# manuelruder/fast-artistic-videos

Hardware: AMD Instinct MI355X
Metric: stylized frames/sec @1280x720, per-frame hot path (mask + warp + assembly + net + deprocess + PNG encode on the GPU) with inputs resident in HBM; file->PNG rate of the product CLI (BASELINE.json's end-to-end) in `end_to_end_fps` / `e2e`, PSNR vs CPU ref in `parity` (higher is better)
Workload: dtype f32

## Files before the change

### fast-artistic-videos_amd/csrc/fav_internal.h

```cpp
#pragma once
#include <hip/hip_runtime.h>
#include <cstdarg>
#include <cstdint>
#include <cstdio>
#include <exception>
#include <new>
#include <string>
#include <vector>

#include "../../include/fav.h"

#include <cstdlib>
inline const char* diag_env(const char* name)
{
#ifdef FAV_DIAG
    return getenv(name);
#else
    (void)name;
    return nullptr;
#endif
}

namespace fav {

// ... 28 lines not shown
        ::fav::set_error(where_ ": unexpected exception"); return FAV_EFORMAT;                                            \
    }

int ensure_device();

struct TraceRange {
    explicit TraceRange(const char* name);
    ~TraceRange();
    static bool enabled();
    bool on;
};

enum LayerType { L_PAD, L_CONV, L_IN, L_RELU, L_RES, L_UP, L_TANH, L_MUL, L_IDENTITY, L_BN };

struct Layer {
    LayerType type = L_IDENTITY;
    int pl = 0, pr = 0, pt = 0, pb = 0, pad_mode = 0;
    int cin = 0, cout = 0, k = 0, stride = 1, pad = 0;
    int transposed = 0, adj = 0;
    std::vector<float> w, b;
    std::vector<float> gamma, beta, mean, var;
    float eps = 1e-5f;
    int scale = 1;
    float mul = 1.f;
    int shave = 0;
    std::vector<Layer> block;
};

int t7_parse_model(const char* path, std::vector<Layer>& out);
int blob_pack(const std::vector<Layer>& layers, std::vector<uint8_t>& blob);
int blob_unpack(const void* blob, size_t bytes, std::vector<Layer>& out);
std::string describe_layers(const std::vector<Layer>& layers, int indent = 0);

struct Affine {
    const float* scale1 = nullptr; const float* shift1 = nullptr; int relu1 = 0;
    const float* scale2 = nullptr; const float* shift2 = nullptr; int relu2 = 0;
    int stages = 0;
    const long long* acc1 = nullptr; long long* acc1_zero = nullptr;
    const float* gamma1 = nullptr; const float* beta1 = nullptr; float eps1 = 0.f; int count1 = 0;
};
constexpr int STAT_COPIES = 8;
inline size_t stat_acc_words(int C) { return (size_t)STAT_COPIES * C * 4; }
constexpr long long STAT_NONFINITE = 1ll << 53;
__host__ __device__ inline bool stat_acc_poisoned(long long hi_sum, long long hi_squares)
{
    return hi_sum >= STAT_NONFINITE / 2 || hi_sum <= -(STAT_NONFINITE / 2) || hi_squares >= STAT_NONFINITE / 2 || hi_squares <= -(STAT_NONFINITE / 2);
}

struct ConvLaunch {
    const float* in = nullptr;
    int IH = 0, IW = 0;
    int IWp = 0;
    int ups = 0;
    int stuff = 0;
    int CIN = 0;
    Affine pre;
    const float* wgt = nullptr;
    const unsigned short* wgt16 = nullptr;
    const float* bias = nullptr;
    int COUT = 0, COUTp = 0;
    int KH = 0, KW = 0, stride = 1, pad = 0;
    int Kpad = 0;
    int OH = 0, OW = 0;
    float* out = nullptr;
    float* partials = nullptr;
    int final_mode = 0;
    float tanh_mul = 1.f;
    float* out_planar = nullptr;
    float* out_raw_nchw = nullptr;
    float* sk_ws = nullptr; unsigned* sk_flags = nullptr; unsigned sk_epoch = 0;
    unsigned* sk_err = nullptr;
    int reserve_cus = 0;
    int no_sk = 0;
    const float* join_skip = nullptr; float* join_out = nullptr; int OWp = 0;
    long long* stat_acc = nullptr;
    float* ks_ws = nullptr; int* ks_cnt = nullptr;
};
inline size_t conv3_wino4_ksplit_bytes() { return (size_t)256 * 2 * 256 * 128 * sizeof(float); }
size_t conv_streamk_workspace_bytes();
int conv_streamk_grid();
constexpr int CONV_BM = 128;
inline int conv_mblocks(int OH, int OW) { return (OH * OW + CONV_BM - 1) / CONV_BM; }
int launch_conv(const ConvLaunch& p, hipStream_t st);
bool conv_c8_eligible(int cin_pitch, int coutp, int k, int stride, int stages, int ups);
int conv_c8_tiles(int OH, int OW);
int launch_conv_c8(const ConvLaunch& p, int* counts, hipStream_t st);
bool conv_c8d_eligible(int cin_pitch, int cin_real, int coutp, int k, int stride, int stages, int ups);
void conv_c8d_pack(const float* w, int cin, int cout, std::vector<float>& out);
int launch_conv_c8d(const ConvLaunch& p, int cin_real, const float* wc8d, int* counts, hipStream_t st);
bool conv3_halo_eligible(int cin_pitch, int coutp, int k, int stride);
int conv3_halo_tiles(int OH, int OW, bool edge_b);
int launch_conv3_halo(const ConvLaunch& p, int* counts, hipStream_t st);
bool conv3s2_eligible(int cin_pitch, int coutp, int k, int stride, int stages, int ups);
int conv3s2_tiles(int OH, int OW);
int launch_conv3s2(const ConvLaunch& p, int* counts, hipStream_t st);
bool conv_fold_eligible(int cin_pitch, int cout, int k, int stride);
bool conv_fold_launchable(int cin_pitch, int k, int pad, int ups, int IH, int IW);
int launch_conv_fold(const ConvLaunch& p, const float* wfold, hipStream_t st);
int conv_first_tiles(int OH, int OW);
int launch_conv_first(const ConvLaunch& p, int cin_real, const float* wpk, int* counts, hipStream_t st);
bool conv_first2d_eligible(int cin_pitch, int cin_real, int coutp, int k, int stride, int stages, int ups);
int conv_first2d_tiles(int OH, int OW);
int launch_conv_first2d(const ConvLaunch& p, int cin_real, const float* wpk, int* counts, hipStream_t st);
bool conv3_wino_eligible(int cin_pitch, int cout, int coutp, int k, int stride, int pad, int stages, int ups);
int conv3_wino_tiles(int OH, int OW);
int launch_conv3_wino(const ConvLaunch& p, const float* wpk, int* counts, hipStream_t st);
bool conv3_wino4_eligible(int cin_pitch, int cout, int coutp, int k, int stride, int pad, int stages, int ups);
int conv3_wino4_tiles(int OH, int OW);
int launch_conv3_wino4(const ConvLaunch& p, const float* wpk, int* counts, hipStream_t st);
bool conv3_up2_eligible(int cin_pitch, int cout, int coutp, int k, int stride, int pad, int stages, int ups);
int conv3_up2_tiles(int OH, int OW);
int launch_conv3_up2(const ConvLaunch& p, const float* wpk, int* counts, hipStream_t st);
bool conv3s2w_eligible(int cin_pitch, int cout, int coutp, int k, int stride, int pad, int stages, int ups);
int conv3s2w_tiles(int OH, int OW, int coutp);
int launch_conv3s2w(const ConvLaunch& p, const float* wpk, int* counts, hipStream_t st);
enum ConvKernel { CK_GENERIC, CK_FOLD, CK_C8, CK_C8D, CK_FIRST1D, CK_FIRST2D, CK_S2W, CK_UP2, CK_WINO, CK_WINO4, CK_HALO3, CK_S2HALO };
constexpr int CONV_KERNELS = CK_S2HALO + 1;
int launch_in_finalize(const float* partials, const int* counts, int mblocks, int M, int block_pixels, int C, int Cpitch,
                       const float* gamma, const float* beta, float eps,
                       float* scale, float* shift, hipStream_t st);
int launch_stats(const float* x, int M, int C, const Affine& t, float* partials, hipStream_t st);
int launch_pad_nhwc(const float* in, int Hp, int Wp, int in_pitch, int C, int ups, float* out, int pl, int pr, int pt, int pb, int mode, hipStream_t st);
int launch_res_add(const float* y, const float* scale, const float* shift,
                   const float* skip, int SH, int SW, int shave, const Affine& skip_t,
                   int C, float* z, float* partials, int* counts, hipStream_t st, int skip_pitch = 0, const Affine* branch_acc = nullptr);
inline int res_add_stat_blocks(int OH, int OW) { return OH * ((OW + 127) / 128); }
int launch_nchw_to_nhwc_pad(const float* in, int C, int H, int W, int pad, int Cp, float* out, hipStream_t st);
int launch_nhwc_to_nchw(const float* in, int M, int C, const Affine& t, float* out, hipStream_t st);

#ifdef __HIPCC__
__device__ __forceinline__ float fill_uniform(unsigned seed, unsigned index, unsigned c, unsigned y, unsigned x)
{
    unsigned k = seed * 0x9E3779B1u + index * 0x85EBCA77u + c * 0xC2B2AE3Du + y * 0x27D4EB2Fu + x * 0x165667B1u;
    k ^= k >> 15; k *= 0x2C1B3C6Du;
    k ^= k >> 12; k *= 0x297A2D39u;
    k ^= k >> 15;
    return (float)(k >> 8) * (1.0f / 16777216.0f);
}
#endif

int launch_warp(const float* img, const float* flow, float* out, int B, int C, int H, int W, int Ho, int Wo,
                int border, hipStream_t st);
int launch_min_filter_f32(const float* cert, float* out, int H, int W, int r, hipStream_t st);
int launch_assemble(const float* frame, const float* warped, const float* cert, float* in7, int H, int W,
                    hipStream_t st);
int launch_cert_prepare(const uint8_t* mask, const float* backward_flo, int invert, int fix_occ, int border,
                        int r, float* cert_tmp, float* cert, int H, int W, hipStream_t st);
int launch_prep_input(const uint8_t* frame_hwc, const float* prev_rgb, int Hs, int Ws, const float* backward_flo,
                      const float* cert, int border, int H, int W, int pad, float* in8, hipStream_t st,
                      int fill_random = 0, unsigned seed = 0, unsigned index = 0, int* q0_out = nullptr);
int launch_quantize_rgb8(const float* rgb_planar, uint8_t* out_hwc, int H, int W, hipStream_t st);
constexpr int PNG_NSYM = 277;
constexpr int PNG_NTABLES = 12;
constexpr int PNG_HDR_WORDS = 40;
struct PngTable {
    uint32_t sym[PNG_NSYM];
    uint32_t hdr[PNG_HDR_WORDS];
    uint32_t hdr_bits, btype, dist_len, dist_code;
// ... 50 lines not shown
```

### fast-artistic-videos_amd/csrc/kernels_elem.hip

```cpp
#include <algorithm>

#include "fav_internal.h"
#include "conv_device.h"

namespace fav {

namespace {

__global__ __launch_bounds__(256) void in_finalize_kernel(const float2* partials, const int* counts, int mblocks, int M, int bp,
                                                          int Cpitch, const float* gamma, const float* beta,
                                                          float eps, float* scale, float* shift)
{
    __shared__ double sh[8];
    const int c = blockIdx.x, t = threadIdx.x;
    double s1 = 0, s2 = 0;
    float gq = 1.f, bq = 0.f;
    if (t == 0) { gq = gamma ? gamma[c] : 1.f; bq = beta ? beta[c] : 0.f; }
    for (int b0 = t; b0 < mblocks; b0 += 1024) {
        float2 pr[4]; int nb[4];
#pragma unroll
        for (int k = 0; k < 4; ++k) {
            const int b = b0 + 256 * k, bc = min(b, mblocks - 1);
            pr[k] = partials[(size_t)bc * Cpitch + c];
            nb[k] = b < mblocks ? (counts ? counts[bc] : min(bp, M - bc * bp)) : 0;
        }
#pragma unroll
        for (int k = 0; k < 4; ++k) {
            const double n = (double)nb[k], mu = (double)pr[k].x;
            s1 += n * mu;
            s2 += (nb[k] ? (double)pr[k].y : 0.0) + n * mu * mu;
        }
    }
    for (int o = 32; o > 0; o >>= 1) { s1 += __shfl_xor(s1, o); s2 += __shfl_xor(s2, o); }
    if ((t & 63) == 0) { sh[2 * (t >> 6)] = s1; sh[2 * (t >> 6) + 1] = s2; }
    __syncthreads();
    if (t == 0) {
        const double a = ((sh[0] + sh[2]) + sh[4]) + sh[6], q = ((sh[1] + sh[3]) + sh[5]) + sh[7];
        const double mean = a / (double)M;
        double var = q / (double)M - mean * mean;
        var = var > 0.0 ? var : 0.0;
        const double g = (double)gq, bt = (double)bq;
        const double sc = g / sqrt(var + (double)eps);
        scale[c] = (float)sc;
        shift[c] = (float)(bt - mean * sc);
    }
}

__device__ __forceinline__ float4 apply_affine_g(float4 v, const Affine& a, int c)
{
    if (a.stages >= 1) {
        v = affine4(v, a.scale1 + c, a.shift1 + c, a.relu1);
        if (a.stages >= 2) v = affine4(v, a.scale2 + c, a.shift2 + c, a.relu2);
    }
    return v;
}

template <int NPT>
__global__ __launch_bounds__(256) void stats_kernel(const float* x, int M, int C, const Affine a, float2* partials)
{
    __shared__ float red[1024];
    __shared__ float mean_s[1024];
    const int t = threadIdx.x;
    const int groups = C >> 2;
    const int nl = 256 / groups;
    const int g = t % groups, pl = t / groups;
    const int m0 = blockIdx.x * 128;
    const int cnt = min(128, M - m0);
    const bool active = pl < nl;
    float4 s = make_float4(0, 0, 0, 0);
    float4 keep[NPT > 0 ? NPT : 1];
    if (NPT > 0) {
#pragma unroll
        for (int i = 0; i < NPT; ++i) {
            const int pix = pl + i * nl;
            float4 v = make_float4(0, 0, 0, 0);
            if (pix < cnt) { v = *reinterpret_cast<const float4*>(x + (size_t)(m0 + pix) * C + 4 * g); v = apply_affine_g(v, a, 4 * g); }
            keep[i] = v;
        }
#pragma unroll
        for (int i = 0; i < NPT; ++i) { s.x += keep[i].x; s.y += keep[i].y; s.z += keep[i].z; s.w += keep[i].w; }
    } else if (active)
        for (int pix = pl; pix < cnt; pix += nl) {
            float4 v = *reinterpret_cast<const float4*>(x + (size_t)(m0 + pix) * C + 4 * g);
            v = apply_affine_g(v, a, 4 * g);
            s.x += v.x; s.y += v.y; s.z += v.z; s.w += v.w;
        }
    if (active) *reinterpret_cast<float4*>(red + pl * C + 4 * g) = s;
    __syncthreads();
    for (int c = t; c < C; c += 256) {
        float r = 0;
        for (int i = 0; i < nl; ++i) r += red[i * C + c];
        mean_s[c] = r / (float)cnt;
    }
    __syncthreads();
    float4 q = make_float4(0, 0, 0, 0);
    if (active) {
        const float4 mu = *reinterpret_cast<const float4*>(mean_s + 4 * g);
        if (NPT > 0) {
#pragma unroll
            for (int i = 0; i < NPT; ++i) {
                const float4 v = keep[i];
                const float dx = v.x - mu.x, dy = v.y - mu.y, dz = v.z - mu.z, dw = v.w - mu.w;
                if (pl + i * nl < cnt) { q.x = fmaf(dx, dx, q.x); q.y = fmaf(dy, dy, q.y); q.z = fmaf(dz, dz, q.z); q.w = fmaf(dw, dw, q.w); }
            }
        } else
            for (int pix = pl; pix < cnt; pix += nl) {
                float4 v = *reinterpret_cast<const float4*>(x + (size_t)(m0 + pix) * C + 4 * g);
                v = apply_affine_g(v, a, 4 * g);
                const float dx = v.x - mu.x, dy = v.y - mu.y, dz = v.z - mu.z, dw = v.w - mu.w;
                q.x = fmaf(dx, dx, q.x); q.y = fmaf(dy, dy, q.y); q.z = fmaf(dz, dz, q.z); q.w = fmaf(dw, dw, q.w);
            }
        *reinterpret_cast<float4*>(red + pl * C + 4 * g) = q;
    }
    __syncthreads();
    for (int c = t; c < C; c += 256) {
        float r = 0;
        for (int i = 0; i < nl; ++i) r += red[i * C + c];
        partials[(size_t)blockIdx.x * C + c] = make_float2(mean_s[c], r);
    }
}

template <bool ACC>
__global__ __launch_bounds__(256) void res_add_kernel(const float* y, const float* scale, const float* shift,
                                                      const float* skip, int SW, int shave, const Affine sa,
                                                      int OH, int OW, int C, float* z, const Affine br)
{
    __shared__ float ss[ACC ? 2048 : 4];
    if (ACC) {
        for (int i = threadIdx.x; i < C; i += 256) {
            long long w0 = 0, w1 = 0, w2 = 0, w3 = 0;
#pragma unroll
            for (int cp = 0; cp < STAT_COPIES; ++cp) {
                const longlong2* a = reinterpret_cast<const longlong2*>(br.acc1 + ((size_t)cp * C + i) * 4);
                const longlong2 lo = a[0], hi = a[1];
                w0 += lo.x; w1 += lo.y; w2 += hi.x; w3 += hi.y;
            }
            const double s1 = ((double)w1 * 4294967296.0 + (double)w0) * (1.0 / 1099511627776.0);
            const double s2 = ((double)w3 * 4294967296.0 + (double)w2) * (1.0 / 1099511627776.0);
            const double mean = s1 / (double)br.count1;
            double var = s2 / (double)br.count1 - mean * mean;
            var = var > 0.0 ? var : 0.0;
            const double sc = stat_acc_poisoned(w1, w3) ? (double)NAN : (double)br.gamma1[i] / sqrt(var + (double)br.eps1);
            ss[i] = (float)sc; ss[C + i] = (float)((double)br.beta1[i] - mean * sc);
            if (blockIdx.x == 0) {
#pragma unroll
                for (int cp = 0; cp < STAT_COPIES; ++cp) {
                    longlong2* zz = reinterpret_cast<longlong2*>(br.acc1_zero + ((size_t)cp * C + i) * 4);
                    zz[0] = longlong2{0, 0}; zz[1] = longlong2{0, 0};
                }
            }
        }
        __syncthreads();
        scale = ss; shift = ss + C;
    }
    const int groups = C >> 2;
    const size_t total = (size_t)OH * OW * groups;
    for (size_t idx = (size_t)blockIdx.x * 256 + threadIdx.x; idx < total; idx += (size_t)gridDim.x * 256) {
        const int g = (int)(idx % groups);
        const size_t pix = idx / groups;
        const int oy = (int)(pix / OW), ox = (int)(pix - (size_t)oy * OW);
        float4 v = *reinterpret_cast<const float4*>(y + pix * C + 4 * g);
        v = affine4(v, scale + 4 * g, shift + 4 * g, 0);
        float4 k = *reinterpret_cast<const float4*>(skip + ((size_t)(oy + shave) * SW + ox + shave) * C + 4 * g);
        k = apply_affine_g(k, sa, 4 * g);
        v.x += k.x; v.y += k.y; v.z += k.z; v.w += k.w;
        *reinterpret_cast<float4*>(z + pix * C + 4 * g) = v;
    }
}

template <int NPT>
__global__ __launch_bounds__(256) void res_add_stats_kernel(const float* y, const float* scale, const float* shift,
                                                            const float* skip, int SW, int shave, const Affine sa,
                                                            int OW, int C, float* z, float2* partials, int* counts)
{
    __shared__ float red[1024];
    __shared__ float mean_s[1024];
    const int t = threadIdx.x;
    const int groups = C >> 2, nl = 256 / groups;
    const int g = t % groups, pl = t / groups;
    const int segs = (OW + 127) / 128;
    const int oy = blockIdx.x / segs, x0 = (blockIdx.x - oy * segs) * 128;
    const int cnt = min(128, OW - x0);
    const bool active = pl < nl;
    const float* yr = y + ((size_t)oy * OW + x0) * C + 4 * g;
    const float* kr = skip + ((size_t)(oy + shave) * SW + x0 + shave) * C + 4 * g;
    float* zr = z + ((size_t)oy * OW + x0) * C + 4 * g;
    float4 sm = make_float4(0, 0, 0, 0);
    float4 keep[NPT > 0 ? NPT : 1];
    if (NPT > 0) {
        float4 kk[NPT > 0 ? NPT : 1];
#pragma unroll
        for (int i = 0; i < NPT; ++i) {
            const int px = pl + i * nl;
            keep[i] = make_float4(0, 0, 0, 0); kk[i] = make_float4(0, 0, 0, 0);
            if (px < cnt) { keep[i] = *reinterpret_cast<const float4*>(yr + (size_t)px * C); kk[i] = *reinterpret_cast<const float4*>(kr + (size_t)px * C); }
        }
#pragma unroll
        for (int i = 0; i < NPT; ++i) {
            const int px = pl + i * nl;
            float4 v = affine4(keep[i], scale + 4 * g, shift + 4 * g, 0);
            const float4 k = apply_affine_g(kk[i], sa, 4 * g);
            v.x += k.x; v.y += k.y; v.z += k.z; v.w += k.w;
            if (px < cnt) { *reinterpret_cast<float4*>(zr + (size_t)px * C) = v; sm.x += v.x; sm.y += v.y; sm.z += v.z; sm.w += v.w; }
            keep[i] = v;
        }
    } else if (active)
        for (int px = pl; px < cnt; px += nl) {
            float4 v = *reinterpret_cast<const float4*>(yr + (size_t)px * C);
            v = affine4(v, scale + 4 * g, shift + 4 * g, 0);
            float4 k = *reinterpret_cast<const float4*>(kr + (size_t)px * C);
            k = apply_affine_g(k, sa, 4 * g);
            v.x += k.x; v.y += k.y; v.z += k.z; v.w += k.w;
            *reinterpret_cast<float4*>(zr + (size_t)px * C) = v;
            sm.x += v.x; sm.y += v.y; sm.z += v.z; sm.w += v.w;
        }
    if (active) *reinterpret_cast<float4*>(red + pl * C + 4 * g) = sm;
    __syncthreads();
    for (int c = t; c < C; c += 256) {
        float r = 0;
        for (int i = 0; i < nl; ++i) r += red[i * C + c];
        mean_s[c] = r / (float)cnt;
    }
    __syncthreads();
    float4 q = make_float4(0, 0, 0, 0);
    if (active) {
        const float4 mu = *reinterpret_cast<const float4*>(mean_s + 4 * g);
        if (NPT > 0) {
#pragma unroll
            for (int i = 0; i < NPT; ++i) {
                const float4 v = keep[i];
                const float dx = v.x - mu.x, dy = v.y - mu.y, dz = v.z - mu.z, dw = v.w - mu.w;
                if (pl + i * nl < cnt) { q.x = fmaf(dx, dx, q.x); q.y = fmaf(dy, dy, q.y); q.z = fmaf(dz, dz, q.z); q.w = fmaf(dw, dw, q.w); }
            }
        } else
        for (int px = pl; px < cnt; px += nl) {
            const float4 v = *reinterpret_cast<const float4*>(zr + (size_t)px * C);
            const float dx = v.x - mu.x, dy = v.y - mu.y, dz = v.z - mu.z, dw = v.w - mu.w;
            q.x = fmaf(dx, dx, q.x); q.y = fmaf(dy, dy, q.y); q.z = fmaf(dz, dz, q.z); q.w = fmaf(dw, dw, q.w);
        }
        *reinterpret_cast<float4*>(red + pl * C + 4 * g) = q;
    }
    __syncthreads();
    for (int c = t; c < C; c += 256) {
        float r = 0;
        for (int i = 0; i < nl; ++i) r += red[i * C + c];
        partials[(size_t)blockIdx.x * C + c] = make_float2(mean_s[c], r);
    }
    if (t == 0) counts[blockIdx.x] = cnt;
}

__device__ __forceinline__ int reflect(int i, int n)
{
    if (i < 0) i = -i;
    if (i >= n) i = 2 * (n - 1) - i;
    return i;
}

__global__ __launch_bounds__(256) void nchw_to_nhwc_pad_kernel(const float* in, int C, int H, int W, int pad, int Cp,
                                                               float* out)
{
    const int Hp = H + 2 * pad, Wp = W + 2 * pad;
    const size_t total = (size_t)Hp * Wp * Cp;
    for (size_t idx = (size_t)blockIdx.x * 256 + threadIdx.x; idx < total; idx += (size_t)gridDim.x * 256) {
        const int c = (int)(idx % Cp);
        const size_t pix = idx / Cp;
        const int y = (int)(pix / Wp), x = (int)(pix - (size_t)y * Wp);
        float v = 0.f;
        if (c < C) v = in[((size_t)c * H + reflect(y - pad, H)) * W + reflect(x - pad, W)];
        out[idx] = v;
    }
}

__global__ __launch_bounds__(256) void nhwc_to_nchw_kernel(const float* in, int M, int C, const Affine a, float* out)
{
    const size_t total = (size_t)M * C;
    for (size_t idx = (size_t)blockIdx.x * 256 + threadIdx.x; idx < total; idx += (size_t)gridDim.x * 256) {
        const int c = (int)(idx / M);
        const size_t m = idx - (size_t)c * M;
        float v = in[m * C + c];
        if (a.stages >= 1) {
            v = fmaf(v, a.scale1[c], a.shift1[c]); if (a.relu1) v = fmaxf(v, 0.f);
            if (a.stages >= 2) { v = fmaf(v, a.scale2[c], a.shift2[c]); if (a.relu2) v = fmaxf(v, 0.f); }
        }
        out[idx] = v;
    }
}

inline int grid_for(size_t total) { size_t b = (total + 255) / 256; return (int)(b > 8192 ? 8192 : (b ? b : 1)); }

}

int launch_in_finalize(const float* partials, const int* counts, int mblocks, int M, int block_pixels, int C, int Cpitch,
                       const float* gamma, const float* beta, float eps, float* scale, float* shift, hipStream_t st)
{
    hipLaunchKernelGGL(in_finalize_kernel, dim3(C), dim3(256), 0, st, reinterpret_cast<const float2*>(partials), counts,
                       mblocks, M, block_pixels, Cpitch, gamma, beta, eps, scale, shift);
    FAV_LAUNCH_CHECK("in_finalize_kernel");
    return FAV_OK;
}

int launch_stats(const float* x, int M, int C, const Affine& t, float* partials, hipStream_t st)
{
    FAV_REQUIRE(C % 4 == 0 && C <= 1024 && 256 % (C / 4) == 0, "stats: unsupported channel count %d", C);
    const dim3 grid((M + 127) / 128);
    float2* pp = reinterpret_cast<float2*>(partials);
    if (C == 64) hipLaunchKernelGGL(stats_kernel<8>, grid, dim3(256), 0, st, x, M, C, t, pp);
    else if (C == 128) hipLaunchKernelGGL(stats_kernel<16>, grid, dim3(256), 0, st, x, M, C, t, pp);
    else hipLaunchKernelGGL(stats_kernel<0>, grid, dim3(256), 0, st, x, M, C, t, pp);
    FAV_LAUNCH_CHECK("stats_kernel");
    return FAV_OK;
}

int launch_res_add(const float* y, const float* scale, const float* shift, const float* skip, int SH, int SW,
                   int shave, const Affine& skip_t, int C, float* z, float* partials, int* counts, hipStream_t st, int skip_pitch, const Affine* branch_acc)
{
    const int OH = SH - 2 * shave, OW = SW - 2 * shave;
    if (skip_pitch > 0) SW = skip_pitch;
    FAV_REQUIRE(C % 4 == 0 && C <= 1024 && 256 % (C / 4) == 0 && OH > 0 && OW > 0, "res_add: bad shape (C=%d)", C);
    FAV_REQUIRE(!(partials && branch_acc && branch_acc->acc1), "res_add: the statistics-taking join does not take an accumulator-form InstanceNorm");
    if (partials) {
        const dim3 grid(res_add_stat_blocks(OH, OW));
        float2* pp = reinterpret_cast<float2*>(partials);
        if (C == 128) hipLaunchKernelGGL(res_add_stats_kernel<16>, grid, dim3(256), 0, st, y, scale, shift, skip, SW, shave, skip_t, OW, C, z, pp, counts);
        else if (C == 64) hipLaunchKernelGGL(res_add_stats_kernel<8>, grid, dim3(256), 0, st, y, scale, shift, skip, SW, shave, skip_t, OW, C, z, pp, counts);
        else hipLaunchKernelGGL(res_add_stats_kernel<0>, grid, dim3(256), 0, st, y, scale, shift, skip, SW, shave, skip_t, OW, C, z, pp, counts);
    }
    else if (branch_acc != nullptr && branch_acc->acc1 != nullptr)
        hipLaunchKernelGGL(res_add_kernel<true>, dim3(std::min(1024, grid_for((size_t)OH * OW * (C / 4)))), dim3(256), 0, st, y, scale, shift, skip, SW, shave, skip_t,
                           OH, OW, C, z, *branch_acc);
    else
        hipLaunchKernelGGL(res_add_kernel<false>, dim3(grid_for((size_t)OH * OW * (C / 4))), dim3(256), 0, st, y, scale, shift, skip, SW, shave, skip_t,
                           OH, OW, C, z, Affine());
    FAV_LAUNCH_CHECK("res_add_kernel");
    return FAV_OK;
}

int launch_nchw_to_nhwc_pad(const float* in, int C, int H, int W, int pad, int Cp, float* out, hipStream_t st)
{
    FAV_REQUIRE(pad < H && pad < W, "reflection pad %d must be smaller than the image (%dx%d)", pad, W, H);
    hipLaunchKernelGGL(nchw_to_nhwc_pad_kernel, dim3(grid_for((size_t)(H + 2 * pad) * (W + 2 * pad) * Cp)), dim3(256), 0,
                       st, in, C, H, W, pad, Cp, out);
    FAV_LAUNCH_CHECK("nchw_to_nhwc_pad_kernel");
    return FAV_OK;
}

int launch_nhwc_to_nchw(const float* in, int M, int C, const Affine& t, float* out, hipStream_t st)
{
    hipLaunchKernelGGL(nhwc_to_nchw_kernel, dim3(grid_for((size_t)M * C)), dim3(256), 0, st, in, M, C, t, out);
    FAV_LAUNCH_CHECK("nhwc_to_nchw_kernel");
    return FAV_OK;
}

}
```

### fast-artistic-videos_amd/csrc/kernels_first.hip

```cpp
#include <algorithm>
#include <cstdlib>
#include <vector>

#include "fav_internal.h"
#include "conv_device.h"
#include "launch_common.h"
#include "first_pack.h"
#include "first2d_pack.h"

namespace fav {

namespace {

constexpr int F_TH = 8, F_TW = 64;
constexpr int F_HR = F_TH + 8, F_HC = F_TW + 8;
constexpr int F_HALF = F_HC / 2;
constexpr int F_RP = F_HC;
constexpr int F_CPL = F_HR * F_RP;
constexpr int F_HP = F_HR * F_HC;
constexpr int F_NH = (F_HP + 511) / 512;

struct FirstArgs {
    const float* in; const float* wpk; const float* bias;
    float* out; float2* partials; int* counts;
    int IH, IW, IWp, COUT, pad, OH, OW, tiles_x, tiles_y;
    int COUTP, groups;
    long long* dbg = nullptr;
};

__device__ __forceinline__ float2 merge_rows(const float2* st, const int* wn, int c, int* n_out)
{
    int n = 0; float s = 0.f;
    for (int w = 0; w < 8; ++w) { n += wn[w]; s += (float)wn[w] * st[w * 32 + c].x; }
    const float mean = n ? s / (float)n : 0.f;
    float m2 = 0.f;
    for (int w = 0; w < 8; ++w) { const float d = st[w * 32 + c].x - mean; m2 += st[w * 32 + c].y + (float)wn[w] * d * d; }
    *n_out = n;
    return make_float2(mean, m2);
}

constexpr int f_off(int e) { return (e & 1) * F_HALF + (e >> 1); }

template <int CR>
__global__ __launch_bounds__(512, 2) void conv_first_kernel(const FirstArgs p)
{
    constexpr int NCC = (CR / 2) * 27, NJ = NCC + 14, LAST = CR - 1;
    extern __shared__ __attribute__((aligned(16))) float smem[];
    float* const Ws = smem;
    float* const Hs = Ws + 4 * NJ * 64;
    float* const red = Hs + CR * F_CPL;
    const int t = threadIdx.x, lane = t & 63, wave = t >> 6;

    for (int e = t; e < 4 * NJ * 16; e += 512) *reinterpret_cast<v4f*>(Ws + e * 4) = *reinterpret_cast<const v4f*>(p.wpk + e * 4);

    const int ntiles = p.tiles_x * p.tiles_y;
    float4 hlo[F_NH], hhi[F_NH];
#define FL_LOAD_HALO(tile_)                                                                         \
// ... 206 lines not shown
        _Pragma("unroll") for (int i = 0; i < G_NH; ++i) {                                          \
            float* d_ = Hs + min(t + 512 * i, G_HP - 1);                                            \
            const float c_[8] = {hlo[i].x, hlo[i].y, hlo[i].z, hlo[i].w, hhi[i].x, hhi[i].y, hhi[i].z, hhi[i].w}; \
            _Pragma("unroll") for (int c = 0; c < CR; ++c) d_[c * G_CPL] = c_[c];                   \
        }                                                                                           \
    }

    int tile = WIDE ? blockIdx.x / p.groups : blockIdx.x;
    G_LOAD_HALO(tile);
    G_STORE_HALO();

    const int txl = lane & 15, g = lane >> 4;
    int qoff[NQ];
#pragma unroll
    for (int q = 0; q < NQ; ++q) {
        const int idx = 4 * q + g;
        const int c = idx / 9, a = (idx - 9 * c) / 3, b = idx - 9 * c - 3 * a;
        qoff[q] = idx < 9 * CR ? c * G_CPL + 3 * a * G_HC + 3 * b : 0;
    }
    const float* const a_lane = Hs + 2 * wave * G_HC + 2 * txl;
    const float* const b_lo = Ws + lane;
    int hi_words = 8 * NQ * 128;
    asm volatile("" : "+v"(hi_words));
    const float* const b_hi = b_lo + hi_words;
    __syncthreads();

#ifdef FAV_DIAG
    long long dt_[5] = {0, 0, 0, 0, 0}, tq_ = 0; int ntl_ = 0;
#define G_DBG(i_) { if (p.dbg && t == 0) { const long long n_ = wall_clock64(); dt_[i_] += n_ - tq_; tq_ = n_; } }
    if (p.dbg && t == 0) tq_ = wall_clock64();
#else
#define G_DBG(i_)
#endif
    for (; tile < ntiles; tile += tstep) {
        const int nxt = tile + tstep;
        G_LOAD_HALO(nxt);
        G_DBG(0);
        v4f acc[16][2];
#pragma unroll
        for (int ps = 0; ps < 16; ++ps)
#pragma unroll
            for (int nt = 0; nt < 2; ++nt) acc[ps][nt] = v4f{0.f, 0.f, 0.f, 0.f};

        float R[2][16], B[2][8];
#define G_READ_R(set_, q_)                                                                          \
        { const float* rb_ = a_lane + qoff[q_];                                                     \
          _Pragma("unroll") for (int r = 0; r < 4; ++r) _Pragma("unroll") for (int d = 0; d < 4; ++d) R[set_][4 * r + d] = rb_[r * G_HC + d]; }
#define G_READ_B(set_, q_, i_)                                                                      \
        { _Pragma("unroll") for (int j = 0; j < 4; ++j) _Pragma("unroll") for (int nt = 0; nt < 2; ++nt) \
              B[set_][2 * j + nt] = ((i_) < 2 ? b_lo : b_hi)[(((4 * ((i_) & 1) + j) * NQ + (q_)) * 2 + nt) * 64]; }
#define G_FENCE() __builtin_amdgcn_sched_barrier(0)
        G_READ_R(0, 0);
        G_READ_B(0, 0, 0);
#pragma unroll
        for (int q = 0; q < NQ; ++q) {
            if (q + 1 < NQ) { G_READ_R((q + 1) & 1, q + 1); }
#pragma unroll
            for (int i = 0; i < 4; ++i) {
                float L[4], V[4];
                const float* Rq = R[q & 1];
#pragma unroll
                for (int d = 0; d < 4; ++d)
                    L[d] = i == 0 ? Rq[d] - Rq[8 + d] : i == 1 ? Rq[4 + d] + Rq[8 + d] : i == 2 ? Rq[8 + d] - Rq[4 + d] : Rq[4 + d] - Rq[12 + d];
                V[0] = L[0] - L[2]; V[1] = L[1] + L[2]; V[2] = L[2] - L[1]; V[3] = L[1] - L[3];
                const int nset = (4 * q + i + 1) & 1;
                if (i < 3) { G_READ_B(nset, q, i + 1); } else if (q + 1 < NQ) { G_READ_B(nset, q + 1, 0); }
// ... 83 lines not shown
            const int nw = nrows * ncols;
#pragma unroll
            for (int nt = 0; nt < 2; ++nt) {
                float s = sm[nt];
                s += __shfl_xor(s, 16); s += __shfl_xor(s, 32);
                const float mu = nw ? s / (float)nw : 0.f;
                float qv = 0.f;
                if (inside) {
#pragma unroll
                    for (int r = 0; r < 4; ++r)
#pragma unroll
                        for (int a = 0; a < 2; ++a)
#pragma unroll
                            for (int b = 0; b < 2; ++b) { const float d = y[nt][r][a][b] - mu; qv = fmaf(d, d, qv); }
                } else {
#pragma unroll
                    for (int r = 0; r < 4; ++r)
#pragma unroll
                        for (int a = 0; a < 2; ++a)
#pragma unroll
                            for (int b = 0; b < 2; ++b) {
                                const int oy = oy0 + a, ox = ox0 + 2 * (4 * g + r) + b;
                                const float d = y[nt][r][a][b] - mu;
                                if (oy < p.OH && ox < p.OW) qv = fmaf(d, d, qv);
                            }
                }
                qv += __shfl_xor(qv, 16); qv += __shfl_xor(qv, 32);
                if (lane < 16) st[wave * 32 + nt * 16 + lane] = make_float2(mu, qv);
            }
            if (lane == 0) wn[wave] = nw;
            __syncthreads();
            if (t < 32) {
                int n;
                p.partials[(size_t)tile * PITCH + grp * 32 + t] = merge_rows(st, wn, t, &n);
                if (t == 0 && grp == 0) p.counts[tile] = n;
            }
        }
        __syncthreads();
        G_DBG(4);
#ifdef FAV_DIAG
        ++ntl_;
#endif
    }
#ifdef FAV_DIAG
    if (p.dbg && t == 0) { for (int i = 0; i < 5; ++i) p.dbg[blockIdx.x * 8 + i] = dt_[i]; p.dbg[blockIdx.x * 8 + 5] = ntl_; }
#endif
#undef G_DBG
#undef G_LOAD_HALO
#undef G_STORE_HALO
}

template <int CR, bool WIDE = false>
int launch_first2d_t(const FirstArgs& a, int reserve_cus, hipStream_t st)
{
    const size_t lds = (size_t)(16 * conv_first2d_quads(CR) * 128 + CR * G_CPL + 8 * 64 + 8) * sizeof(float);
    static PerDevice cache; int cus;
    FAV_HIP(launch_cus(cache, &cus, conv_first2d_kernel<CR, WIDE>));
    const int tiles = a.tiles_x * a.tiles_y;
    const int ngrp = WIDE ? a.groups : 1;
    int grid = persistent_slots(cus, reserve_cus);
    grid = std::min(grid, tiles * ngrp);
    if (WIDE) grid = std::max(ngrp, grid / ngrp * ngrp);
#ifdef FAV_DIAG
    static int dbg_n = diag_env("FAV_FIRST_DBG") ? atoi(diag_env("FAV_FIRST_DBG")) : 0;
    static long long* dbuf = nullptr;
    const bool dbg = dbg_n > 0 && --dbg_n == 0;
    FirstArgs ad = a;
    if (dbg) { FAV_HIP(hipMalloc(reinterpret_cast<void**>(&dbuf), 1024 * 8 * 8)); FAV_HIP(hipMemsetAsync(dbuf, 0, 1024 * 8 * 8, st)); ad.dbg = dbuf; }
    hipLaunchKernelGGL((conv_first2d_kernel<CR, WIDE>), dim3(grid), dim3(512), lds, st, ad);
    FAV_LAUNCH_CHECK("conv_first2d_kernel");
    if (dbg) {
        std::vector<long long> hb((size_t)1024 * 8);
        FAV_HIP(hipStreamSynchronize(st)); FAV_HIP(hipMemcpy(hb.data(), dbuf, hb.size() * 8, hipMemcpyDeviceToHost));
        double sum[5] = {0, 0, 0, 0, 0}, nt = 0;
        for (int b = 0; b < grid; ++b) { for (int i = 0; i < 5; ++i) sum[i] += hb[b * 8 + i] * 0.01; nt += hb[b * 8 + 5]; }
        fprintf(stderr, "FIRSTDBG grid=%d tiles=%.0f  per tile (us): halo request %.2f  quads %.2f  barrier + halo to LDS %.2f  transform + stores %.2f  statistics %.2f\n",
                grid, nt, sum[0] / nt, sum[1] / nt, sum[2] / nt, sum[3] / nt, sum[4] / nt);
    }
    return FAV_OK;
#else
    hipLaunchKernelGGL((conv_first2d_kernel<CR, WIDE>), dim3(grid), dim3(512), lds, st, a);
    FAV_LAUNCH_CHECK("conv_first2d_kernel");
    return FAV_OK;
#endif
}

}

int conv_first_tiles(int OH, int OW) { return ((OH + F_TH - 1) / F_TH) * ((OW + F_TW - 1) / F_TW); }

int launch_conv_first(const ConvLaunch& c, int cin_real, const float* wpk, int* counts, hipStream_t st)
{
    FAV_REQUIRE(c.CIN == 8 && (cin_real == 7 || cin_real == 3) && c.COUTp == 32 && c.KH == 9 && c.KW == 9 && c.stride == 1 && c.pre.stages == 0 &&
                c.ups == 0 && !c.final_mode && wpk, "first-layer conv (F(2,3) along x): not eligible");
    FAV_REQUIRE((long long)c.IH * c.IWp * 8 < (1ll << 31), "first-layer conv: bad shape");
    FirstArgs a;
    a.in = c.in; a.wpk = wpk; a.bias = c.bias; a.out = c.out; a.partials = reinterpret_cast<float2*>(c.partials); a.counts = counts;
    a.IH = c.IH; a.IW = c.IW; a.IWp = c.IWp; a.COUT = c.COUT; a.pad = c.pad; a.OH = c.OH; a.OW = c.OW;
    a.tiles_x = (c.OW + F_TW - 1) / F_TW; a.tiles_y = (c.OH + F_TH - 1) / F_TH;
    return cin_real == 7 ? launch_first_t<7>(a, c.reserve_cus, st) : launch_first_t<3>(a, c.reserve_cus, st);
}

bool conv_first2d_eligible(int cin_pitch, int cin_real, int coutp, int k, int stride, int stages, int ups)
{
    return cin_pitch == 8 && (cin_real == 7 || cin_real == 3) && k == 9 && stride == 1 && stages == 0 && ups == 0 && coutp % 32 == 0 && coutp >= 32 && coutp <= 256;
}
int conv_first2d_tiles(int OH, int OW) { return ((OH + G_TH - 1) / G_TH) * ((OW + G_TW - 1) / G_TW); }

int launch_conv_first2d(const ConvLaunch& c, int cin_real, const float* wpk, int* counts, hipStream_t st)
{
    FAV_REQUIRE(conv_first2d_eligible(c.CIN, cin_real, c.COUTp, c.KH, c.stride, c.pre.stages, c.ups) && c.KW == 9 && !c.final_mode && wpk,
                "first-layer conv (F(2x2,3x3) over the nine 3x3 blocks): not eligible");
    FAV_REQUIRE((long long)c.IH * c.IWp * 32 < (1ll << 31) - 512, "first-layer conv: input too large for 32-bit byte offsets");
    FirstArgs a;
    a.in = c.in; a.wpk = wpk; a.bias = c.bias; a.out = c.out; a.partials = reinterpret_cast<float2*>(c.partials); a.counts = counts;
    a.IH = c.IH; a.IW = c.IW; a.IWp = c.IWp; a.COUT = c.COUT; a.pad = c.pad; a.OH = c.OH; a.OW = c.OW;
    a.tiles_x = (c.OW + G_TW - 1) / G_TW; a.tiles_y = (c.OH + G_TH - 1) / G_TH;
    a.COUTP = c.COUTp; a.groups = c.COUTp / 32; a.dbg = nullptr;
    if (a.groups > 1) return cin_real == 7 ? launch_first2d_t<7, true>(a, c.reserve_cus, st) : launch_first2d_t<3, true>(a, c.reserve_cus, st);
    return cin_real == 7 ? launch_first2d_t<7>(a, c.reserve_cus, st) : launch_first2d_t<3>(a, c.reserve_cus, st);
}

}
```

### fast-artistic-videos_amd/csrc/kernels_fold.hip

```cpp
#include <algorithm>
#include <cstdlib>
#include <vector>

#include "fav_internal.h"
#include "conv_device.h"
#include "launch_common.h"

namespace fav {

namespace {

constexpr int FOLD_R = 16;
constexpr int FOLD_M = 128;

struct FoldArgs {
    const float* in; const float* wfold; const float* bias;
    const float* scale1; const float* shift1; const float* scale2; const float* shift2;
    float* out_planar; float* out_raw;
    int IH, IW, IWp, ups, COUT, KH, KW, pad, OH, OW;
    int stages, relu1, relu2;
    float tanh_mul;
    int tiles_x, tiles_y;
    long long* dbg;
};

template <int CIN>
__global__ __launch_bounds__(512, 2) void conv_rowfold_kernel(const FoldArgs p)
{
    constexpr int NT = 512;
    constexpr int RW = FOLD_R / 2;
    constexpr int S = CIN + 4;
    constexpr int NV = CIN / 16;
    constexpr int KK = CIN / 8;
    extern __shared__ __attribute__((aligned(16))) float smem[];
    float* Bs = smem;
    float* aff = Bs + p.KH * 32 * S;
    float* As = aff + 4 * CIN;

    const int t = threadIdx.x, lane = t & 63, wave = t >> 6;
    const int wcol = wave & 3, wrow = wave >> 2;
    const int XO = FOLD_M - (p.KW - 1);

    for (int i = t; i < CIN; i += NT) {
        aff[i] = p.stages >= 1 ? p.scale1[i] : 1.f; aff[CIN + i] = p.stages >= 1 ? p.shift1[i] : 0.f;
        aff[2 * CIN + i] = p.stages >= 2 ? p.scale2[i] : 1.f; aff[3 * CIN + i] = p.stages >= 2 ? p.shift2[i] : 0.f;
    }
    const float lo1 = (p.stages >= 1 && p.relu1) ? 0.f : -INFINITY;
    const float lo2 = (p.stages >= 2 && p.relu2) ? 0.f : -INFINITY;
    for (int e = t; e < p.KH * 32 * (CIN / 4); e += NT) {
        const int row = e / (CIN / 4), c4 = e - row * (CIN / 4);
        *reinterpret_cast<v4f*>(Bs + row * S + c4 * 4) = *reinterpret_cast<const v4f*>(p.wfold + (size_t)row * CIN + c4 * 4);
    }
    const int xl = t >> 2, ch0 = (t & 3) * (CIN / 4);
// ... 106 lines not shown
            __syncthreads();
        }
    }
}

constexpr int FOLD2_M = 64;

template <int CIN, int NH = 1>
__global__ __launch_bounds__(512, 2) void conv_rowfold_up2_kernel(const FoldArgs p)
{
    constexpr int NT = 512;
    constexpr int CT = CIN * NH;
    constexpr int RW = FOLD_R / 4;
    constexpr int S = CIN + 4;
    constexpr int NV = CIN / 32;
    constexpr int KK = CIN / 8;
    extern __shared__ __attribute__((aligned(16))) float smem[];
    float* Bs = smem;
    float* aff = Bs + (p.KH + 1) * 32 * S;
    float* As = aff + 4 * CIN;

    const int t = threadIdx.x, lane = t & 63, wave = t >> 6;
    const int wcol = wave & 1, wrow = wave >> 1;
    const int XO = 2 * FOLD2_M - (p.KW - 1);
    const int PH = p.IH >> 1, PW = p.IW >> 1;

    const float lo1 = (p.stages >= 1 && p.relu1) ? 0.f : -INFINITY;
    const float lo2 = (p.stages >= 2 && p.relu2) ? 0.f : -INFINITY;
    const float* wm = p.wfold + (size_t)p.KH * 32 * CT;
#define FOLD_RESIDENT(hoff_)                                                                        \
    {                                                                                               \
        for (int i = t; i < CIN; i += NT) {                                                         \
            aff[i] = p.stages >= 1 ? p.scale1[(hoff_) + i] : 1.f; aff[CIN + i] = p.stages >= 1 ? p.shift1[(hoff_) + i] : 0.f; \
            aff[2 * CIN + i] = p.stages >= 2 ? p.scale2[(hoff_) + i] : 1.f; aff[3 * CIN + i] = p.stages >= 2 ? p.shift2[(hoff_) + i] : 0.f; \
        }                                                                                           \
        for (int e = t; e < (p.KH + 1) * 32 * (CIN / 4); e += NT) {                                 \
            const int row = e / (CIN / 4), c4 = e - row * (CIN / 4);                                \
            *reinterpret_cast<v4f*>(Bs + row * S + c4 * 4) = *reinterpret_cast<const v4f*>(wm + (size_t)row * CT + (hoff_) + c4 * 4); \
        }                                                                                           \
    }
    if (NH == 1) FOLD_RESIDENT(0);
    const int xl = t >> 3, ch0 = (t & 7) * (CIN / 8);
    const int frag = (lane & 31) * S + (lane >> 5) * 4;
    const int col = lane & 31, rbase = 4 * (lane >> 5);
    float4 ra[NV];

    for (int tile = blockIdx.x; tile < p.tiles_x * p.tiles_y; tile += gridDim.x) {
        const int by = tile / p.tiles_x, bx = tile - by * p.tiles_x;
        const int ox0 = bx * XO, oy0 = by * FOLD_R;
        const int pxs = (ox0 - p.pad) >> 1;
        const int iy_lo = max(0, oy0 - p.pad), iy_hi = min(p.IH - 1, oy0 + FOLD_R - 1 + p.KH - 1 - p.pad);
        const int pr_lo = iy_lo >> 1, pr_hi = min(iy_hi >> 1, PH - 1);
        const int pc = pxs + xl;
        const bool colv = pc >= 0 && pc < PW;
        const float colm = colv ? 1.f : 0.f;
        const int coloff = colv ? pc * CT + ch0 : 0;
        int hoff = 0;

#define FOLD_LOAD(pr_)                                                                              \
        {                                                                                           \
            const float* src_ = p.in + (size_t)(pr_) * p.IWp * CT + coloff + hoff;                  \
            _Pragma("unroll") for (int i = 0; i < NV; ++i) ra[i] = *reinterpret_cast<const float4*>(src_ + 4 * i); \
        }
#define FOLD_STORE(buf_)                                                                            \
        {                                                                                           \
            float* dst_ = As + (buf_) * FOLD2_M * S + xl * S + ch0;                                 \
            _Pragma("unroll") for (int i = 0; i < NV; ++i) {                                        \
// ... 145 lines not shown
        for (int b = 0; b < 512; ++b) { n += hb[b * 8]; a0 += hb[b * 8 + 1]; a1 += hb[b * 8 + 2]; a2 += hb[b * 8 + 3]; rows += hb[b * 8 + 4]; }
        if (n > 0) fprintf(stderr, "FOLDDBG tiles=%.0f  per tile: first row %.2f  loop %.2f (%.1f staged rows)  epilogue %.2f us\n", n, a0 / n * 0.01, a1 / n * 0.01, rows / n, a2 / n * 0.01);
    }
    return FAV_OK;
}

template <int CIN>
int launch_fold_t(FoldArgs a, int reserve_cus, hipStream_t st)
{
    const int S = CIN + 4;
    const size_t wbytes = (size_t)(a.KH * 32 * S + 4 * CIN) * sizeof(float);
    size_t stage = (size_t)(2 * FOLD_M * S) * sizeof(float);
    const size_t epi = (size_t)4 * FOLD_M * 33 * sizeof(float);
    if (epi > stage) stage = epi;
    const size_t lds = wbytes + stage;
    if (lds > 160 * 1024) { set_error("row-folded conv: %zu bytes of LDS needed", lds); return FAV_EUNSUPPORTED; }
    static PerDevice cache; int cus;
    FAV_HIP(launch_cus(cache, &cus, conv_rowfold_kernel<CIN>));
    const int XO = FOLD_M - (a.KW - 1);
    a.tiles_x = (a.OW + XO - 1) / XO; a.tiles_y = (a.OH + FOLD_R - 1) / FOLD_R;
    const int tiles = a.tiles_x * a.tiles_y;
    const int nres = persistent_slots(cus, reserve_cus);
    hipLaunchKernelGGL((conv_rowfold_kernel<CIN>), dim3(tiles < nres ? tiles : nres), dim3(512), lds, st, a);
    FAV_LAUNCH_CHECK("conv_rowfold_kernel");
    return FAV_OK;
}

}

bool conv_fold_eligible(int cin_pitch, int cout, int k, int stride)
{
    return stride == 1 && cout * k <= 32 && k <= 9 && (cin_pitch == 16 || cin_pitch == 32 || cin_pitch == 64 || cin_pitch == 128 || cin_pitch == 256);
}
bool conv_fold_launchable(int cin_pitch, int k, int pad, int ups, int IH, int IW)
{
    static const bool no_up2 = diag_env("FAV_NO_FOLD_UP2") != nullptr;
    if (cin_pitch <= 64) return true;
    return ups == 1 && !no_up2 && (pad & 1) == 0 && (k & 1) == 1 && (IH & 1) == 0 && (IW & 1) == 0 && k + 1 <= 10;
}

int launch_conv_fold(const ConvLaunch& c, const float* wfold, hipStream_t st)
{
    FAV_REQUIRE(conv_fold_eligible(c.CIN, c.COUT, c.KW, c.stride) && c.KH == c.KW && c.final_mode, "row-folded conv: not eligible");
    FoldArgs a;
    a.dbg = nullptr;
    a.in = c.in; a.wfold = wfold; a.bias = c.bias;
    a.scale1 = c.pre.scale1; a.shift1 = c.pre.shift1; a.scale2 = c.pre.scale2; a.shift2 = c.pre.shift2;
    a.stages = c.pre.stages; a.relu1 = c.pre.relu1; a.relu2 = c.pre.relu2;
    a.out_planar = c.out_planar; a.out_raw = c.out_raw_nchw;
    a.IH = c.IH; a.IW = c.IW; a.IWp = c.IWp; a.ups = c.ups; a.COUT = c.COUT; a.KH = c.KH; a.KW = c.KW; a.pad = c.pad;
    a.OH = c.OH; a.OW = c.OW; a.tanh_mul = c.tanh_mul;
    static const bool no_up2 = diag_env("FAV_NO_FOLD_UP2") != nullptr;
    if (c.ups == 1 && !no_up2 && (c.pad & 1) == 0 && (c.KW & 1) == 1 && (c.IH & 1) == 0 && (c.IW & 1) == 0 && c.KH + 1 <= 10) {
        if (c.CIN == 256) return launch_fold_up2_t<64, 4>(a, c.reserve_cus, st);
        if (c.CIN == 128) return launch_fold_up2_t<64, 2>(a, c.reserve_cus, st);
        if (c.CIN == 64) return launch_fold_up2_t<64>(a, c.reserve_cus, st);
        if (c.CIN == 32) return launch_fold_up2_t<32>(a, c.reserve_cus, st);
    }
    FAV_REQUIRE(c.CIN <= 64, "row-folded conv: %d input channels are supported on a x2-upsampled input only", c.CIN);
    if (c.CIN == 64) return launch_fold_t<64>(a, c.reserve_cus, st);
    if (c.CIN == 32) return launch_fold_t<32>(a, c.reserve_cus, st);
    return launch_fold_t<16>(a, c.reserve_cus, st);
}

}
```

### fast-artistic-videos_amd/csrc/kernels_s2.hip

```cpp
#include <algorithm>
#include <cstdlib>

#include "fav_internal.h"
#include "conv_device.h"
#include "launch_common.h"
#include "s2_pack.h"

namespace fav {

namespace {

constexpr int SW_P = 20;
constexpr int SW_EW = 33, SW_OW = 32;

struct S2wArgs {
    const float* in; const float* wpk; const float* bias; const float* scale1; const float* shift1;
    float* out; float2* partials; int* counts;
    int IH, IW, IWp, CIN, OH, OW, pad, tiles_x, tiles_y, stages, relu1;
    int COUTP, groups;
};

template <int NTC, int TR> struct SwGeo {
    static constexpr int NW = NTC * TR;
    static constexpr int NTH = 64 * NW;
    static constexpr int HR = 2 * TR + 1;
    static constexpr int EP = HR * SW_EW;
    static constexpr int HP = EP + HR * SW_OW;
    static constexpr int PS = NTH / 4;
    static constexpr int NPC = (HP + PS - 1) / PS;
    static constexpr int HB = NPC * PS * SW_P;
};

template <int NTC, int TR, bool WIDE = false>
__global__ __launch_bounds__(64 * NTC * TR, NTC * TR / 4) void conv3s2w_kernel(const S2wArgs p)
{
    using G = SwGeo<NTC, TR>;
    static_assert(G::NW % 4 == 0 && G::NW >= 8 && G::NW <= 16, "whole waves per SIMD");
    constexpr int COUT = NTC * 32;
    constexpr int EP = G::EP, HP = G::HP, NPC = G::NPC, HB = G::HB, PS = G::PS, NTH = G::NTH;
    extern __shared__ __attribute__((aligned(16))) float smem[];
    float* const Hs = smem;
    float* const aff = smem + 2 * HB;
    float2* const stt = reinterpret_cast<float2*>(aff + 2 * p.CIN);
    int* const wn = reinterpret_cast<int*>(stt + TR * COUT);

    const int t = threadIdx.x, lane = t & 63;
    const int wave = __builtin_amdgcn_readfirstlane(t >> 6);
    const int nt = wave % NTC, row = wave / NTC;
    const int m = lane & 31, h = lane >> 5;
    const int CIN = p.CIN, nch = CIN >> 4;
    const int lb = xcd_linear_block();
    const int ngrp = WIDE ? p.groups : 1, grp = WIDE ? lb % p.groups : 0;
    const int PITCH = WIDE ? p.COUTP : COUT;
    const __amdgpu_buffer_rsrc_t wrs = __builtin_amdgcn_make_buffer_rsrc(const_cast<float*>(p.wpk) + (size_t)grp * (nch * 18 * NTC * 256), 0, nch * 18 * NTC * 1024, 0x00020000);
    const __amdgpu_buffer_rsrc_t irs = __builtin_amdgcn_make_buffer_rsrc(const_cast<float*>(p.in), 0, p.IH * p.IWp * CIN * 4, 0x00020000);
    const int wlo = lane * 16, wnt = nt * 1024;

    const float* const aE = Hs + ((2 * row) * SW_EW + m) * SW_P + 4 * h;
    const float* const aO = Hs + (EP + (2 * row) * SW_OW + m) * SW_P + 4 * h;
#define SW_AOFF(T_) (((T_) % 3 == 1) ? ((T_) / 3) * SW_OW * SW_P : (((T_) / 3) * SW_EW + ((T_) % 3 == 2 ? 1 : 0)) * SW_P)
#define SW_ABASE(T_) (((T_) % 3 == 1) ? aO : aE)

    const int c4 = t & 3, p0 = t >> 2;
    float* const hst = Hs + p0 * SW_P + c4 * 4;
    int hyx[NPC], hbase[NPC];
#pragma unroll
    for (int i = 0; i < NPC; ++i) {
        const int pe = p0 + PS * i;
        int hy = 0x7000, hx = 0;
        if (pe < EP) { hy = pe / SW_EW; hx = 2 * (pe - hy * SW_EW); }
        else if (pe < HP) { const int q = pe - EP; hy = q / SW_OW; hx = 2 * (q - hy * SW_OW) + 1; }
        hyx[i] = hy << 16 | hx;
        hbase[i] = ((pe < HP ? (hy * p.IWp + hx) * p.CIN : 0) + c4 * 4) * 4;
    }
    for (int i = t; i < CIN; i += NTH) { aff[i] = p.stages >= 1 ? p.scale1[i] : 1.f; aff[CIN + i] = p.stages >= 1 ? p.shift1[i] : 0.f; }
    const float lo1 = (p.stages >= 1 && p.relu1) ? 0.f : -INFINITY;
    const float* const affr = aff + c4 * 4;

    const int ntiles = p.tiles_x * p.tiles_y * ngrp;
    int tile = lb;
    if (tile >= ntiles) return;

    int ho[NPC]; float hm[NPC];
    v4f hq[NPC];
    bool hmask = false;
#define SW_TILE_SETUP(tile_)                                                                        \
    {   const int pt_ = WIDE ? (tile_) / ngrp : (tile_);                                            \
        const int ty_ = pt_ / p.tiles_x, tx_ = pt_ - ty_ * p.tiles_x;                               \
        const int iy0_ = 2 * ty_ * TR - p.pad, ix0_ = 2 * tx_ * 32 - p.pad;                         \
        hmask = iy0_ < 0 || ix0_ < 0 || iy0_ + 2 * TR >= p.IH || ix0_ + 64 >= p.IW;                  \
        if (!hmask) {                                                                               \
            const int org_ = (iy0_ * p.IWp + ix0_) * CIN * 4;                                       \
            _Pragma("unroll") for (int i = 0; i < NPC; ++i) ho[i] = hbase[i] + org_;                \
        } else {                                                                                    \
            _Pragma("unroll") for (int i = 0; i < NPC; ++i) {                                       \
                const int iy = iy0_ + (hyx[i] >> 16), ix = ix0_ + (hyx[i] & 0xffff);                \
                const bool v = ((unsigned)iy < (unsigned)p.IH) & ((unsigned)ix < (unsigned)p.IW);   \
                ho[i] = ((v ? (iy * p.IWp + ix) * CIN : 0) + c4 * 4) * 4;                           \
                hm[i] = v ? 1.f : 0.f;                                                              \
            } } }
#define SW_LOAD_H(chunk_)                                                                           \
    { _Pragma("unroll") for (int i = 0; i < NPC; ++i) hq[i] = __builtin_bit_cast(v4f, __builtin_amdgcn_raw_buffer_load_b128(irs, ho[i], (chunk_) * 64, 0)); }
#define SW_COMMIT(chunk_, par_)                                                                     \
    {   const v4f sc_ = *reinterpret_cast<const v4f*>(affr + (chunk_) * 16), sh_ = *reinterpret_cast<const v4f*>(affr + CIN + (chunk_) * 16); \
        _Pragma("unroll") for (int i = 0; i < NPC; ++i) {                                           \
            hq[i].x = fmaxf(fmaf(hq[i].x, sc_.x, sh_.x), lo1); hq[i].y = fmaxf(fmaf(hq[i].y, sc_.y, sh_.y), lo1); \
            hq[i].z = fmaxf(fmaf(hq[i].z, sc_.z, sh_.z), lo1); hq[i].w = fmaxf(fmaf(hq[i].w, sc_.w, sh_.w), lo1); } \
        if (hmask) { _Pragma("unroll") for (int i = 0; i < NPC; ++i) hq[i] *= hm[i]; }               \
// ... 47 lines not shown
            if (last && ntile < ntiles) SW_TILE_SETUP(ntile);
            const int so1 = ((chunk * 2 + 1) * 9) * NTC * 1024 + wnt, so0 = ((nchunk * 2) * 9) * NTC * 1024 + wnt;
#pragma unroll
            for (int tp = 0; tp < 9; ++tp) {
                fb[1][tp] = __builtin_bit_cast(v4f, __builtin_amdgcn_raw_buffer_load_b128(wrs, wlo, so1 + tp * NTC * 1024, 0));
                if (tp < NPC) hq[tp] = __builtin_bit_cast(v4f, __builtin_amdgcn_raw_buffer_load_b128(irs, ho[tp], nchunk * 64, 0));
                if (tp + 2 < 9) { SW_READ_A_DYN((tp + 2) % 3, tp + 2, 0, par); } else { SW_READ_A_DYN((tp + 2) % 3, tp + 2 - 9, 1, par); }
                SW_FENCE(); SW_MFMA4(fa[tp % 3], fb[0][tp]); SW_FENCE();
            }
#pragma unroll
            for (int tp = 0; tp < 7; ++tp) {
                fb[0][tp] = __builtin_bit_cast(v4f, __builtin_amdgcn_raw_buffer_load_b128(wrs, wlo, so0 + tp * NTC * 1024, 0));
                if (tp + 2 < 9) { SW_READ_A_DYN((tp + 2) % 3, tp + 2, 1, par); }
                SW_FENCE(); SW_MFMA4(fa[tp % 3], fb[1][tp]); SW_FENCE();
                if (tp == 2) { __builtin_amdgcn_sched_barrier(0); SW_COMMIT(nchunk, par ^ 1); __builtin_amdgcn_sched_barrier(0); }
            }
            asm volatile("s_waitcnt lgkmcnt(0)" ::: "memory");
            __syncthreads();
            __builtin_amdgcn_sched_barrier(0);
            {
                const v4f a7_ = fa[7 % 3], a8_ = fa[8 % 3];
                fb[0][7] = __builtin_bit_cast(v4f, __builtin_amdgcn_raw_buffer_load_b128(wrs, wlo, so0 + 7 * NTC * 1024, 0));
                fb[0][8] = __builtin_bit_cast(v4f, __builtin_amdgcn_raw_buffer_load_b128(wrs, wlo, so0 + 8 * NTC * 1024, 0));
                SW_READ_A_DYN(0, 0, 0, par ^ 1); SW_READ_A_DYN(1, 1, 0, par ^ 1);
                SW_FENCE(); SW_MFMA4(a7_, fb[1][7]); SW_MFMA4(a8_, fb[1][8]); SW_FENCE();
            }
            if (pend >= 0) {
                if (t < COUT) {
                    int cnt = 0; float s1 = 0.f;
                    for (int w = 0; w < TR; ++w) { cnt += wn[w]; s1 += (float)wn[w] * stt[w * COUT + t].x; }
                    const float mean = cnt ? s1 / (float)cnt : 0.f;
                    float m2 = 0.f;
                    for (int w = 0; w < TR; ++w) { const float d = stt[w * COUT + t].x - mean; m2 += stt[w * COUT + t].y + (float)wn[w] * d * d; }
                    p.partials[(size_t)pend * PITCH + grp * COUT + t] = make_float2(mean, m2);
                    if (t == 0 && grp == 0) p.counts[pend] = cnt;
                }
                pend = -1;
            }
            par ^= 1;
        }
        {
            const int oy = oy0 + row;
            float sm = 0.f; int nv = 0;
            float* const ob = p.out + ((size_t)oy * p.OW + ox0 + 4 * h) * PITCH + grp * COUT + co;
            const bool full = oy0 + TR <= p.OH && ox0 + 32 <= p.OW;
            if (full) {
#pragma unroll
                for (int r = 0; r < 16; ++r) {
                    const float v = acc[r] + bv;
                    acc[r] = v;
                    ob[(size_t)((r & 3) + 8 * (r >> 2)) * PITCH] = v;
                    sm += v;
                }
                nv = 16;
            } else {
#pragma unroll
                for (int r = 0; r < 16; ++r) {
                    const int mi = (r & 3) + 8 * (r >> 2);
                    const float v = acc[r] + bv;
                    acc[r] = v;
                    if (oy < p.OH && ox0 + 4 * h + mi < p.OW) { ob[(size_t)mi * PITCH] = v; sm += v; ++nv; }
                }
            }
            if (p.partials != nullptr) {
                const int nw = nv + __shfl_xor(nv, 32);
                const float ssum = sm + __shfl_xor(sm, 32);
                const float mu = nw ? ssum / (float)nw : 0.f;
                float q = 0.f;
                if (full) {
#pragma unroll
                    for (int r = 0; r < 16; ++r) { const float d = acc[r] - mu; q = fmaf(d, d, q); }
                } else {
#pragma unroll
                    for (int r = 0; r < 16; ++r) {
                        const int mi = (r & 3) + 8 * (r >> 2);
                        const float d = acc[r] - mu;
                        if (oy < p.OH && ox0 + 4 * h + mi < p.OW) q = fmaf(d, d, q);
                    }
                }
                q += __shfl_xor(q, 32);
                if (lane < 32) stt[row * COUT + co] = make_float2(mu, q);
                if (lane == 0 && nt == 0) wn[row] = nw;
                pend = ptile;
            }
#pragma unroll
            for (int r = 0; r < 16; ++r) acc[r] = 0.f;
        }
        tile = ntile;
        if (tile >= ntiles) break;
        ptile = WIDE ? tile / ngrp : tile;
        oy0 = (ptile / p.tiles_x) * TR; ox0 = (ptile - (ptile / p.tiles_x) * p.tiles_x) * 32;
    }
    if (pend >= 0) {
        __syncthreads();
        if (t < COUT) {
            int cnt = 0; float s1 = 0.f;
            for (int w = 0; w < TR; ++w) { cnt += wn[w]; s1 += (float)wn[w] * stt[w * COUT + t].x; }
            const float mean = cnt ? s1 / (float)cnt : 0.f;
            float m2 = 0.f;
            for (int w = 0; w < TR; ++w) { const float d = stt[w * COUT + t].x - mean; m2 += stt[w * COUT + t].y + (float)wn[w] * d * d; }
            p.partials[(size_t)pend * PITCH + grp * COUT + t] = make_float2(mean, m2);
            if (t == 0 && grp == 0) p.counts[pend] = cnt;
        }
    }
#undef SW_AOFF
#undef SW_ABASE
#undef SW_TILE_SETUP
#undef SW_LOAD_H
#undef SW_COMMIT
#undef SW_LOAD_B
#undef SW_READ_A
#undef SW_GROUP
#undef SW_TAPS
#undef SW_MFMA4
#undef SW_FENCE
#undef SW_READ_A_DYN
}

template <int NTC, int TR, bool WIDE = false>
int launch_s2w_t(const S2wArgs& a, int reserve_cus, hipStream_t st)
{
    const auto kern = conv3s2w_kernel<NTC, TR, WIDE>;
    const size_t lds = (size_t)(2 * SwGeo<NTC, TR>::HB + 2 * a.CIN) * sizeof(float) + (size_t)TR * NTC * 32 * sizeof(float2) + 16 * sizeof(int);
    static PerDevice cache; int cus;
    FAV_HIP(launch_cus(cache, &cus, kern));
    const int ngrp = WIDE ? a.groups : 1;
    const int tiles = a.tiles_x * a.tiles_y * ngrp;
    const int slots = persistent_slots(cus, reserve_cus);
    static const bool tile_grid = diag_env("FAV_S2W_TILE_GRID") != nullptr;
    int grid = (tile_grid && reserve_cus > 0 && tiles > 4 * slots) ? tiles : std::min(tiles, slots);
    if (WIDE) grid = std::max(ngrp, grid / ngrp * ngrp);
    hipLaunchKernelGGL(kern, dim3(grid), dim3(SwGeo<NTC, TR>::NTH), lds, st, a);
    FAV_LAUNCH_CHECK("conv3s2w_kernel");
    return FAV_OK;
}

}

bool conv3s2w_eligible(int cin_pitch, int cout, int coutp, int k, int stride, int pad, int stages, int ups)
{
    return k == 3 && stride == 2 && pad <= 1 && ups == 0 && stages <= 1 && cin_pitch % 16 == 0 && cin_pitch >= 32 && cin_pitch <= 512 &&
           cout == coutp && (coutp == 64 || (coutp % 128 == 0 && coutp <= 1024));
}
static int s2w_rows(int coutp) { static const int r128 = diag_env("FAV_S2W_ROWS128") ? atoi(diag_env("FAV_S2W_ROWS128")) : 3; return coutp == 64 ? 4 : (r128 == 2 && coutp == 128 ? 2 : 3); }
int conv3s2w_tiles(int OH, int OW, int coutp) { const int tr = s2w_rows(coutp); return ((OH + tr - 1) / tr) * ((OW + 31) / 32); }

int launch_conv3s2w(const ConvLaunch& c, const float* wpk, int* counts, hipStream_t st)
{
    FAV_REQUIRE(conv3s2w_eligible(c.CIN, c.COUT, c.COUTp, c.KH, c.stride, c.pad, c.pre.stages, c.ups) && c.KH == c.KW && !c.final_mode && !c.stuff && wpk,
                "stride-2 conv: not eligible");
    FAV_REQUIRE((long long)(c.IH + 1) * c.IWp * c.CIN < (1ll << 29), "stride-2 conv: tensor too large for 32-bit byte offsets");
    S2wArgs a;
    a.in = c.in; a.wpk = wpk; a.bias = c.bias; a.scale1 = c.pre.scale1; a.shift1 = c.pre.shift1; a.stages = c.pre.stages; a.relu1 = c.pre.relu1;
    a.out = c.out; a.partials = reinterpret_cast<float2*>(c.partials); a.counts = counts;
    a.IH = c.IH; a.IW = c.IW; a.IWp = c.IWp; a.CIN = c.CIN; a.OH = c.OH; a.OW = c.OW; a.pad = c.pad;
    const int tr = s2w_rows(c.COUTp);
    a.tiles_x = (c.OW + 31) / 32; a.tiles_y = (c.OH + tr - 1) / tr;
    a.COUTP = c.COUTp; a.groups = c.COUTp > 128 ? c.COUTp / 128 : 1;
    FAV_REQUIRE((long long)(c.OH + 1) * c.OW * c.COUTp < (1ll << 31), "stride-2 conv: output too large");
    if (a.groups > 1) return launch_s2w_t<4, 3, true>(a, c.reserve_cus, st);
    return c.COUTp == 64 ? launch_s2w_t<2, 4>(a, c.reserve_cus, st) : tr == 2 ? launch_s2w_t<4, 2>(a, c.reserve_cus, st) : launch_s2w_t<4, 3>(a, c.reserve_cus, st);
}

}
```

### fast-artistic-videos_amd/csrc/kernels_up2.hip

```cpp
#include <algorithm>
#include <cstdlib>

#include "fav_internal.h"
#include "conv_device.h"
#include "launch_common.h"
#include "up2_pack.h"

namespace fav {

namespace {

constexpr int U2_HW = 34, U2_HP = 10 * 34;
constexpr int U2_HPP = 384;
constexpr int U2_HB = U2_HPP * LDSS;

struct Up2Args {
    const float* in; const float* wpk; const float* bias; const float* scale1; const float* shift1;
    float* out; float2* partials; int* counts;
    int PH, PW, IWp, CIN, tiles_x, tiles_y, relu1;
    int COUTP, groups;
};

template <bool AFF>
__global__ __launch_bounds__(512, 2) void conv3_up2_kernel(const Up2Args p)
{
    extern __shared__ __attribute__((aligned(16))) float smem[];
    float* const Hs = smem;
    float* const aff = smem + 2 * U2_HB;

    const int t = threadIdx.x, lane = t & 63;
    const int wave = __builtin_amdgcn_readfirstlane(t >> 6);
    const int py = wave >> 2, px = (wave >> 1) & 1, nt = wave & 1;
    const int CIN = p.CIN, nslices = CIN >> 5, nsteps = nslices * 16;
    const int m = lane & 31, h = lane >> 5;

    const __amdgpu_buffer_rsrc_t wrs = __builtin_amdgcn_make_buffer_rsrc(const_cast<float*>(p.wpk), 0, nsteps * 8192, 0x00020000);
    const __amdgpu_buffer_rsrc_t irs = __builtin_amdgcn_make_buffer_rsrc(const_cast<float*>(p.in), 0, p.PH * p.IWp * CIN * 4, 0x00020000);
    const int wlo = lane * 16, wso = wave * 1024;

    const float* const ab = Hs + ((py * U2_HW) + px + m) * LDSS + 4 * h;
    const int c4 = t & 7;
    float* const hst = Hs + (t >> 3) * LDSS + c4 * 4;

    if (AFF) { for (int i = t; i < CIN; i += 512) { aff[i] = p.scale1[i]; aff[CIN + i] = p.shift1[i]; } __syncthreads(); }
    const float lo1 = (AFF && p.relu1) ? 0.f : -INFINITY;
    const float* const affr = aff + c4 * 4;

    const int ntiles = p.tiles_x * p.tiles_y;
    for (int tile = blockIdx.x; tile < ntiles; tile += gridDim.x) {
        const int ty = tile / p.tiles_x, tx = tile - ty * p.tiles_x;
        const int sy0 = ty * 8, sx0 = tx * 32;
// ... 131 lines not shown
                if (t == 0) p.counts[tile] = cnt;
            }
            __syncthreads();
        }
    }
}

constexpr int UW_HW = 34, UW_HP = 6 * 34;
constexpr int UW_HPP = 288;
constexpr int UW_HB = UW_HPP * LDSS;
static_assert(2 * 288 * LDSS <= 8 * 64 * 2 * LDSS, "halo buffers inside the exchange area");
constexpr int UW_ZS = 8 * 64 * 2 * LDSS;

template <bool WIDE>
__global__ __launch_bounds__(768) void conv3_up2w_kernel(const Up2Args p)
{
    extern __shared__ __attribute__((aligned(16))) float smem[];
    float* const Hs = smem;
    float* const aff = smem + UW_ZS;
    const int t = threadIdx.x, lane = t & 63;
    const int wave = __builtin_amdgcn_readfirstlane(t >> 6);
    const int kind = wave >> 2, row = wave & 3;
    const int CIN = p.CIN, nslices = CIN >> 5, nkg = CIN >> 3;
    const int m = lane & 31, h = lane >> 5;
    const int ngrp = WIDE ? p.groups : 1, PITCH = WIDE ? p.COUTP : 64;
    const __amdgpu_buffer_rsrc_t wrs = __builtin_amdgcn_make_buffer_rsrc(const_cast<float*>(p.wpk), 0, nkg * 18 * 1024 * ngrp, 0x00020000);
    const __amdgpu_buffer_rsrc_t irs = __builtin_amdgcn_make_buffer_rsrc(const_cast<float*>(p.in), 0, p.PH * p.IWp * CIN * 4, 0x00020000);
    const int wlo = lane * 16, wso0 = kind * 3 * 2048;
    const float kap = kind == 1 ? 0.f : 1.f;
    const float* const ra = Hs + ((row + (kind == 0 ? 0 : 1)) * UW_HW + m) * LDSS + 4 * h;
    const float* const rb = Hs + ((row + (kind == 0 ? 1 : kind == 1 ? 1 : 2)) * UW_HW + m) * LDSS + 4 * h;
    const int c4 = t & 7;
    float* const hst = Hs + (t >> 3) * LDSS + c4 * 4;
    for (int i = t; i < CIN; i += 768) { aff[i] = p.scale1[i]; aff[CIN + i] = p.shift1[i]; }
    __syncthreads();
    const float lo1 = p.relu1 ? 0.f : -INFINITY;
    const float* const affr = aff + c4 * 4;

    const int ntiles = p.tiles_x * p.tiles_y * ngrp;
    for (int item = blockIdx.x; item < ntiles; item += gridDim.x) {
        const int tile = WIDE ? item / ngrp : item, grp = WIDE ? item - tile * ngrp : 0;
        const int wso = wso0 + grp * nkg * 18432;
        const int ty = tile / p.tiles_x, tx = tile - ty * p.tiles_x;
        const int sy0 = ty * 4, sx0 = tx * 32;
        int ho[3];
#pragma unroll
        for (int i = 0; i < 3; ++i) {
            const int pix = (t >> 3) + 96 * i, hy = (pix * 1928) >> 16, hx = pix - hy * UW_HW;
            const int sy = sy0 - 1 + hy, sx = sx0 - 1 + hx;
            const bool v = pix < UW_HP && (unsigned)sy < (unsigned)p.PH && (unsigned)sx < (unsigned)p.PW;
            ho[i] = v ? ((sy * p.IWp + sx) * CIN + c4 * 4) * 4 : -16;
        }
#define UW_XF(v_, i_, slice_)                                                                       \
        { const v4f sc_ = *reinterpret_cast<const v4f*>(affr + (slice_) * 32), sh_ = *reinterpret_cast<const v4f*>(affr + CIN + (slice_) * 32); \
          const float mk_ = ho[i_] >= 0 ? 1.f : 0.f;                                                \
          v_.x = fmaxf(fmaf(v_.x, sc_.x, sh_.x), lo1) * mk_; v_.y = fmaxf(fmaf(v_.y, sc_.y, sh_.y), lo1) * mk_; \
          v_.z = fmaxf(fmaf(v_.z, sc_.z, sh_.z), lo1) * mk_; v_.w = fmaxf(fmaf(v_.w, sc_.w, sh_.w), lo1) * mk_; }
#define UW_LOAD_B(jj_, kg_)                                                                         \
        { const int so_ = wso + (kg_) * 18432 + (jj_) * 2048;                                       \
          fb[jj_][0] = __builtin_bit_cast(v4f, __builtin_amdgcn_raw_buffer_load_b128(wrs, wlo, so_, 0)); \
          fb[jj_][1] = __builtin_bit_cast(v4f, __builtin_amdgcn_raw_buffer_load_b128(wrs, wlo + 1024, so_, 0)); }
#define UW_READ_R(par_, kg_)                                                                        \
        { _Pragma("unroll") for (int dx = 0; dx < 3; ++dx) {                                        \
              Ra[dx] = *reinterpret_cast<const v4f*>(ra + (par_) * UW_HB + dx * LDSS + (kg_) * 8);  \
              Rb[dx] = *reinterpret_cast<const v4f*>(rb + (par_) * UW_HB + dx * LDSS + (kg_) * 8); } }

        v4f fb[3][2], Ra[3], Rb[3], V[3];
// ... 104 lines not shown
                            if (nt == 0) nv += 4;
                        }
                    }
                }
            }
            if (p.partials != nullptr) {
                const int nw = nv + __shfl_xor(nv, 32);
#pragma unroll
                for (int nt = 0; nt < 2; ++nt) {
                    const float ssum = sm[nt] + __shfl_xor(sm[nt], 32);
                    const float mu = nw ? ssum / (float)nw : 0.f;
                    float q = 0.f;
#pragma unroll
                    for (int r = 0; r < 16; ++r) {
                        const int sx = sx0 + (r & 3) + 8 * (r >> 2) + 4 * h;
                        if (sy < p.PH && sx < p.PW) {
                            const float d0 = acc[0][nt][r] - mu, d1 = acc[1][nt][r] - mu, d2 = acc[2][nt][r] - mu, d3 = y3[nt][r] - mu;
                            q = fmaf(d0, d0, q); q = fmaf(d1, d1, q); q = fmaf(d2, d2, q); q = fmaf(d3, d3, q);
                        }
                    }
                    q += __shfl_xor(q, 32);
                    if (lane < 32) stt[row * 64 + nt * 32 + lane] = make_float2(mu, q);
                }
                if (lane == 0) wn[row] = nw;
            }
        }
        __syncthreads();
        if (p.partials != nullptr && t < 64) {
            int cnt = 0; float s1 = 0.f;
            for (int w = 0; w < 4; ++w) { cnt += wn[w]; s1 += (float)wn[w] * stt[w * 64 + t].x; }
            const float mean = cnt ? s1 / (float)cnt : 0.f;
            float m2 = 0.f;
            for (int w = 0; w < 4; ++w) { const float d = stt[w * 64 + t].x - mean; m2 += stt[w * 64 + t].y + (float)wn[w] * d * d; }
            p.partials[(size_t)tile * PITCH + grp * 64 + t] = make_float2(mean, m2);
            if (t == 0 && grp == 0) p.counts[tile] = cnt;
        }
        __syncthreads();
    }
}

}

static bool up2_winograd() { static const bool w = diag_env("FAV_UP2_PHASES") == nullptr; return w; }
bool conv3_up2_eligible(int cin_pitch, int cout, int coutp, int k, int stride, int pad, int stages, int ups)
{
    return k == 3 && stride == 1 && pad == 1 && ups == 1 && stages == 1 && cin_pitch % 32 == 0 && cin_pitch >= 32 && cin_pitch <= 256 &&
           cout == coutp && (cout == 64 || (up2_winograd() && cout % 64 == 0 && cout <= 512));
}
int conv3_up2_tiles(int OH, int OW) { return ((OH / 2 + (up2_winograd() ? 3 : 7)) / (up2_winograd() ? 4 : 8)) * ((OW / 2 + 31) / 32); }

int launch_conv3_up2(const ConvLaunch& c, const float* wpk, int* counts, hipStream_t st)
{
    FAV_REQUIRE(conv3_up2_eligible(c.CIN, c.COUT, c.COUTp, c.KH, c.stride, c.pad, c.pre.stages, c.ups) && c.KH == c.KW && !c.final_mode && !c.stuff && wpk,
                "upsampled 3x3 conv: not eligible");
    FAV_REQUIRE((c.IH & 1) == 0 && (c.IW & 1) == 0 && c.OH == c.IH && c.OW == c.IW, "upsampled 3x3 conv: bad geometry");
    FAV_REQUIRE((long long)(c.IH / 2 + 1) * c.IWp * c.CIN < (1ll << 29), "upsampled 3x3 conv: tensor too large for 32-bit byte offsets");
    Up2Args a;
    a.in = c.in; a.wpk = wpk; a.bias = c.bias; a.scale1 = c.pre.scale1; a.shift1 = c.pre.shift1; a.relu1 = c.pre.relu1; a.out = c.out; a.partials = reinterpret_cast<float2*>(c.partials); a.counts = counts;
    a.PH = c.IH / 2; a.PW = c.IW / 2; a.IWp = c.IWp; a.CIN = c.CIN;
    const bool wg = up2_winograd();
    a.tiles_x = (a.PW + 31) / 32; a.tiles_y = wg ? (a.PH + 3) / 4 : (a.PH + 7) / 8;
    const size_t lds = wg ? (size_t)(UW_ZS + 2 * c.CIN + 2 * 4 * 64 + 8) * sizeof(float)
                          : (size_t)(2 * U2_HB + 2 * c.CIN) * sizeof(float);
    static PerDevice cache; int cus;
    FAV_HIP(launch_cus(cache, &cus, conv3_up2_kernel<true>, conv3_up2w_kernel<false>, conv3_up2w_kernel<true>));
    a.COUTP = c.COUTp; a.groups = c.COUTp / 64;
    FAV_REQUIRE((long long)(c.OH + 1) * c.OW * c.COUTp < (1ll << 31), "upsampled 3x3 conv: output too large");
    const int tiles = a.tiles_x * a.tiles_y * a.groups;
    const int grid = std::min(tiles, persistent_slots(cus, c.reserve_cus));
    if (wg && a.groups > 1) { hipLaunchKernelGGL(conv3_up2w_kernel<true>, dim3(grid), dim3(768), lds, st, a); }
    else if (wg) { a.wpk = wpk + conv_up2_packed_floats(c.CIN); hipLaunchKernelGGL(conv3_up2w_kernel<false>, dim3(grid), dim3(768), lds, st, a); }
    else hipLaunchKernelGGL(conv3_up2_kernel<true>, dim3(grid), dim3(512), lds, st, a);
    FAV_LAUNCH_CHECK("conv3_up2_kernel");
    return FAV_OK;
}

}
```

### fast-artistic-videos_amd/csrc/kernels_wino4.hip

```cpp
#include <algorithm>
#include <cstdlib>
#include <type_traits>
#include <vector>

#include "fav_internal.h"
#include "wino4_pack.h"

namespace fav {

typedef float v4f __attribute__((ext_vector_type(4)));
typedef int v4i __attribute__((ext_vector_type(4)));

namespace {

constexpr int MAX_DEVICES = 64;
constexpr int W4_MEET_MAX = 256;
constexpr int W4_SHARES = 252;
inline int cur_dev() { int d = 0; (void)hipGetDevice(&d); return (d >= 0 && d < MAX_DEVICES) ? d : 0; }

constexpr int W4_VPOS = 256;
constexpr int W4_VBUF = 36 * W4_VPOS;
constexpr int W4_LLINE = 18 * 4;
constexpr int W4_LTY = 113 * 4;
constexpr int W4_LKQ = 464 * 4;
constexpr int W4_LBUF = 4 * W4_LKQ;
constexpr int W4_RBUF = 6 * 288 * 4;
constexpr int W4_SMEM = 2 * W4_VBUF + W4_LBUF + W4_RBUF;
static_assert((W4_LTY / 4) % 16 == 1 && (W4_LKQ / 4) % 16 == 0 && W4_LTY >= 6 * W4_LLINE && W4_LKQ >= 4 * W4_LTY, "pitches of L");

struct Wino4Args {
    const float* in; const float* wpk; const float* bias; const float* scale1; const float* shift1;
    float* out; float2* partials; int* counts;
    const float* skip; float* zout;
    int OWp;
    int IH, IW, IWp, CIN, OH, OW, units_x, units_y, relu1;
    int stream, shares; float* ks_ws; int* ks_cnt;
    long long* dbg;
    long long* stat_acc; const long long* acc1; long long* acc1_zero; const float* gamma1; const float* beta1; float eps1; int count1;
    int COUT, groups;
};

__device__ __forceinline__ void w4_store16_wt(void* ptr, v4f v)
{
    asm volatile("global_store_dwordx4 %0, %1, off sc1" ::"v"(ptr), "v"(v) : "memory");
}

typedef float v2f __attribute__((ext_vector_type(2)));
__device__ __forceinline__ v2f w4_fma(float a, v2f b, v2f c) { return __builtin_elementwise_fma(v2f{a, a}, b, c); }
__device__ __forceinline__ void w4_bt2(const v2f d[6], v2f v[6])
{
    const v2f e1 = w4_fma(-2.25f, d[2], d[4]), o1 = w4_fma(-1.6875f, d[1], 0.75f * d[3]);
    const v2f e2 = w4_fma(-0.5625f, d[2], d[4]), o2 = w4_fma(-0.84375f, d[1], 1.5f * d[3]);
    v[0] = w4_fma(1.265625f, d[0], w4_fma(-2.8125f, d[2], d[4]));
    v[1] = e1 + o1; v[2] = e1 - o1; v[3] = e2 + o2; v[4] = e2 - o2;
    v[5] = w4_fma(1.265625f, d[1], w4_fma(-2.8125f, d[3], d[5]));
}
__device__ __forceinline__ void w4_bt(const v4f d[6], v4f v[6])
{
    v2f dl[6], dh[6], vl[6], vh[6];
#pragma unroll
    for (int i = 0; i < 6; ++i) { dl[i] = d[i].xy; dh[i] = d[i].zw; }
    w4_bt2(dl, vl); w4_bt2(dh, vh);
#pragma unroll
    for (int i = 0; i < 6; ++i) v[i] = v4f{vl[i].x, vl[i].y, vh[i].x, vh[i].y};
}
__device__ __forceinline__ void w4_at(const v2f m[6], v2f y[4])
{
    const v2f s1 = m[1] + m[2], d1 = m[1] - m[2], s2 = m[3] + m[4], d2 = m[3] - m[4];
    y[0] = (m[0] + s1) + s2;
    y[1] = w4_fma(1.5f, d2, 0.75f * d1);
    y[2] = w4_fma(2.25f, s2, 0.5625f * s1);
    y[3] = w4_fma(3.375f, d2, w4_fma(0.421875f, d1, m[5]));
}

template <int MODE, int VAR = 0, bool WIDE = false>
__global__ __launch_bounds__(512) __attribute__((amdgpu_waves_per_eu(2, 2))) void conv3_wino4_kernel(const Wino4Args p)
{
    constexpr bool AFF = MODE != 0, JOIN = MODE == 2;
    constexpr bool PAIR = (VAR & 8) == 0 && MODE != 2;
    constexpr int NT = 512;
    extern __shared__ __attribute__((aligned(16))) float smem[];
    float* const Vs = smem;
    float* const Ls = smem + 2 * W4_VBUF;
    float* const Rs = Ls + W4_LBUF;
    float* const Ss = Rs + W4_RBUF;
    float* const aff = Ss + ((MODE == 2 || PAIR) ? W4_RBUF : 0);
    typedef __attribute__((address_space(3))) void* lds_ptr_t;

    const int t = threadIdx.x, lane = t & 63;
    const int wave = __builtin_amdgcn_readfirstlane(t >> 6);
    const int CIN = p.CIN, nslices = CIN >> 4;

    int dbi = 0;
#define DBG_T() { if (p.dbg && t == 0 && dbi < 21) p.dbg[blockIdx.x * 24 + dbi++] = wall_clock64(); }
    DBG_T();
    int lb;
    {
        const int nwg = gridDim.x, q = nwg >> 3, r = nwg & 7, xcd = blockIdx.x & 7, idx = blockIdx.x >> 3;
        lb = (xcd < r ? xcd * (q + 1) : r * (q + 1) + (xcd - r) * q) + idx;
    }
    if (MODE == 1 && p.acc1 != nullptr) {
        for (int i = t; i < CIN; i += NT) {
            long long w0 = 0, w1 = 0, w2 = 0, w3 = 0;
#pragma unroll
            for (int cp = 0; cp < STAT_COPIES; ++cp) {
                const longlong2* a = reinterpret_cast<const longlong2*>(p.acc1 + ((size_t)cp * CIN + i) * 4);
                const longlong2 lo = a[0], hi = a[1];
                w0 += lo.x; w1 += lo.y; w2 += hi.x; w3 += hi.y;
            }
            const double s1 = ((double)w1 * 4294967296.0 + (double)w0) * (1.0 / 1099511627776.0);
            const double s2 = ((double)w3 * 4294967296.0 + (double)w2) * (1.0 / 1099511627776.0);
            const double mean = s1 / (double)p.count1;
            double var = s2 / (double)p.count1 - mean * mean;
            var = var > 0.0 ? var : 0.0;
            const double sc = stat_acc_poisoned(w1, w3) ? (double)NAN : (double)p.gamma1[i] / sqrt(var + (double)p.eps1);
            aff[i] = (float)sc; aff[CIN + i] = (float)((double)p.beta1[i] - mean * sc);
            if (blockIdx.x == 0) {
#pragma unroll
                for (int cp = 0; cp < STAT_COPIES; ++cp) {
                    longlong2* z = reinterpret_cast<longlong2*>(p.acc1_zero + ((size_t)cp * CIN + i) * 4);
                    z[0] = longlong2{0, 0}; z[1] = longlong2{0, 0};
                }
            }
        }
    } else if (AFF) for (int i = t; i < CIN; i += NT) { aff[i] = p.scale1[i]; aff[CIN + i] = p.shift1[i]; }
    const float lo1 = (MODE == 1 && p.relu1) ? 0.f : -INFINITY;

    const bool has1 = t < 288;
    const int cq = (t >> 3) & 3;
    const int pix1 = min((t >> 5) * 8 + (t & 7), 71), ty1 = (pix1 * 3641) >> 16, x1 = pix1 - ty1 * 18;
    float* const l1 = Ls + cq * W4_LKQ + ty1 * W4_LTY + x1 * 4;
    const float* const affr = aff + cq * 4;
    const bool has2 = wave >= 2;
    const int i2 = max(wave - 2, 0);
    const int m2 = lane & 15, kq2 = lane >> 4;
    const float* const l2 = Ls + kq2 * W4_LKQ + (m2 >> 2) * W4_LTY + 4 * (m2 & 3) * 4 + i2 * W4_LLINE;
    float* const v2 = Vs + lane * 4 + 6 * i2 * W4_VPOS;
    const float* const aA = Vs + lane * 4;
    const int wlo = lane * 16, wso = wave * 1024;

    v4f fb[6];
    bool ring_primed = false;
    int ring_grp = 0;
    const int upix = p.units_x * p.units_y;
    if (AFF) __syncthreads();
    auto work = [&](const int ug, const int s0, const int s1, const int meet, const int part) {
        const int nsl = s1 - s0;
        const bool whole = meet < 0;
        if (s0 != 0) ring_primed = false;
        int u = ug, grp = 0;
        if (WIDE) {
            if (p.stream) { grp = ug / upix; u = ug - grp * upix; } else { u = ug / p.groups; grp = ug - u * p.groups; }
            if (grp != ring_grp) { ring_primed = false; ring_grp = grp; }
        }
        const int wgb = (p.CIN >> 4) * 36 * 8192;
        const __amdgpu_buffer_rsrc_t wrs = __builtin_amdgcn_make_buffer_rsrc(const_cast<float*>(p.wpk) + (WIDE ? (size_t)grp * (wgb >> 2) : 0), 0, wgb, 0x00020000);
        const __amdgpu_buffer_rsrc_t irs = __builtin_amdgcn_make_buffer_rsrc(const_cast<float*>(p.in), 0, p.IH * p.IWp * p.CIN * 4, 0x00020000);
// ... 256 lines not shown
        } else {
#pragma unroll
            for (int a = 0; a < 4; ++a) {
                const bool rv = oyb + a < p.OH;
                const int ro = rv ? ((oyb + a) * p.OWp + ox0) * cpb + cb * 4 : (int)0xFFFF0000;
#pragma unroll
                for (int c = 0; c < 16; ++c) {
                    if (c < ncols) {
                        const float v = y[a][c & 3][c >> 2];
                        __builtin_amdgcn_raw_buffer_store_b32(__builtin_bit_cast(int, v), ors, ro + c * cpb, 0, 0);
                        sm += rv ? v : 0.f;
                    }
                }
            }
            if (p.partials != nullptr) {
                sm += __shfl_xor(sm, 16); sm += __shfl_xor(sm, 32);
                mu = nv ? sm / (float)nv : 0.f;
#pragma unroll
                for (int a = 0; a < 4; ++a) {
                    const bool rv = oyb + a < p.OH;
#pragma unroll
                    for (int c = 0; c < 16; ++c) {
                        if (c < ncols) {
                            const float d = y[a][c & 3][c >> 2] - mu;
                            m2 = rv ? fmaf(d, d, m2) : m2;
                        }
                    }
                }
            }
        }
        if (p.partials != nullptr) {
            m2 += __shfl_xor(m2, 16); m2 += __shfl_xor(m2, 32);
            if (p.stat_acc != nullptr) {
                const double nd = (double)nv, mud = (double)mu;
                const double v = (g & 2) ? (double)m2 + nd * mud * mud : nd * mud;
                const double tt = v * 1099511627776.0;
                const double hi = floor(tt * (1.0 / 4294967296.0));
                const bool fin = fabs(tt) < 9.0e18;
                const long long word = !fin ? ((g & 1) ? STAT_NONFINITE : 0ll) : (g & 1) ? (long long)hi : (long long)(tt - hi * 4294967296.0);
                long long* const dst = p.stat_acc + ((size_t)(blockIdx.x & (STAT_COPIES - 1)) * (WIDE ? p.COUT : 128) + cb) * 4 + g;
                __hip_atomic_fetch_add(dst, word, __ATOMIC_RELAXED, __HIP_MEMORY_SCOPE_AGENT);
            } else if (g == 0) p.partials[(size_t)u * (WIDE ? p.COUT : 128) + cb] = make_float2(mu, m2);
        }
        if (p.partials != nullptr && p.stat_acc == nullptr && t == 0 && grp == 0) p.counts[u] = nv;
        DBG_T();
    };
    const int units = WIDE ? upix * p.groups : upix;
    if (!p.stream) {
        for (int u = lb; u < units; u += gridDim.x) work(u, 0, nslices, -1, 0);
    } else {
        const long long tot = (long long)units * nslices;
        for (int sh = lb; sh < p.shares; sh += gridDim.x) {
            int g = (int)(tot * sh / p.shares);
            const int g1 = (int)(tot * (sh + 1) / p.shares);
            while (g < g1) {
                const int u = g / nslices, s0 = g - u * nslices, s1 = min(nslices, s0 + (g1 - g));
                const bool whole = s0 == 0 && s1 == nslices;
                work(u, s0, s1, whole ? -1 : (s0 == 0 ? sh : sh - 1), s0 == 0 ? 0 : 1);
                g += s1 - s0;
            }
        }
    }
    if (p.dbg && t == 0) p.dbg[blockIdx.x * 24 + 23] = dbi;
#undef DBG_T
}

void wino4_debug_report(const long long* hbuf, int grid, int mode)
{
    long long t0 = hbuf[0];
    for (int b = 0; b < grid; ++b) t0 = std::min(t0, hbuf[b * 24]);
    double sum[4] = {0, 0, 0, 0}, tend = 0, ck = 0, wk = 0; int items = 0;
    for (int b = 0; b < grid; ++b) {
        const long long* r = &hbuf[b * 24]; const int n = (int)r[23];
        for (int i = 1; i + 4 < n + 1 && i + 4 <= 20; i += 5) {
// ... 51 lines not shown
    if (dbg) {
        std::vector<long long> hb((size_t)512 * 24);
        FAV_HIP(hipStreamSynchronize(st)); FAV_HIP(hipMemcpy(hb.data(), dbuf, hb.size() * 8, hipMemcpyDeviceToHost));
        wino4_debug_report(hb.data(), grid, MODE);
    }
    return FAV_OK;
}

}

bool conv3_wino4_eligible(int cin_pitch, int cout, int coutp, int k, int stride, int pad, int stages, int ups)
{
    return k == 3 && stride == 1 && pad == 0 && ups == 0 && stages <= 1 && cin_pitch % 16 == 0 && cin_pitch >= 16 && cin_pitch <= 512 &&
           cout == coutp && cout % 128 == 0 && cout >= 128 && cout <= 1024;
}
int conv3_wino4_tiles(int OH, int OW) { return ((OH + 15) / 16) * ((OW + 15) / 16); }

int launch_conv3_wino4(const ConvLaunch& c, const float* wpk, int* counts, hipStream_t st)
{
    FAV_REQUIRE(conv3_wino4_eligible(c.CIN, c.COUT, c.COUTp, c.KH, c.stride, c.pad, c.pre.stages, c.ups) && c.KH == c.KW && !c.final_mode && !c.stuff && wpk,
                "winograd F(4x4) conv: not eligible");
    FAV_REQUIRE((long long)(c.IH + 1) * c.IWp * c.CIN < (1ll << 29), "winograd F(4x4) conv: tensor too large for 32-bit byte offsets");
    FAV_REQUIRE(c.OH == c.IH - 2 && c.OW == c.IW - 2, "winograd F(4x4) conv: bad geometry");
    FAV_REQUIRE((long long)(c.OH + 1) * (c.OWp > 0 ? c.OWp : c.OW) * c.COUT < (1ll << 29), "winograd F(4x4) conv: output too large for 32-bit byte offsets");
    Wino4Args a;
    a.in = c.in; a.wpk = wpk; a.bias = c.bias; a.scale1 = c.pre.scale1; a.shift1 = c.pre.shift1; a.relu1 = c.pre.relu1;
    a.out = c.out; a.partials = reinterpret_cast<float2*>(c.partials); a.counts = counts;
    a.IH = c.IH; a.IW = c.IW; a.IWp = c.IWp; a.CIN = c.CIN; a.OH = c.OH; a.OW = c.OW;
    a.units_x = (c.OW + 15) / 16; a.units_y = (c.OH + 15) / 16;
    a.dbg = nullptr;
    a.skip = c.join_skip; a.zout = c.join_out; a.OWp = c.OWp > 0 ? c.OWp : c.OW;
    a.ks_ws = c.ks_ws; a.ks_cnt = c.ks_cnt; a.stream = 0; a.shares = 1;
    a.COUT = c.COUT; a.groups = c.COUT / 128;
    a.stat_acc = c.stat_acc; a.acc1 = c.pre.acc1; a.acc1_zero = c.pre.acc1_zero; a.gamma1 = c.pre.gamma1; a.beta1 = c.pre.beta1; a.eps1 = c.pre.eps1; a.count1 = c.pre.count1;
    if (c.stat_acc != nullptr && a.partials == nullptr) a.partials = reinterpret_cast<float2*>(c.stat_acc);
    FAV_REQUIRE(c.pre.acc1 == nullptr || (c.join_skip == nullptr && c.pre.stages == 1 && c.pre.count1 > 0), "winograd F(4x4) conv: accumulator-form InstanceNorm on an unsupported input");
    if (c.join_skip != nullptr) {
        FAV_REQUIRE(c.join_out != nullptr && c.pre.stages == 1 && c.pre.relu1 == 0, "winograd F(4x4) conv: a pending residual join needs its output tensor and exactly one pending normalisation");
        FAV_REQUIRE(a.groups == 1, "winograd F(4x4) conv: a pending residual join is formed by 128-filter layers only");
        return launch_wino4_t<2, false>(a, c.reserve_cus, st);
    }
    if (a.groups > 1) return c.pre.stages >= 1 ? launch_wino4_t<1, true>(a, c.reserve_cus, st) : launch_wino4_t<0, true>(a, c.reserve_cus, st);
    return c.pre.stages >= 1 ? launch_wino4_t<1, false>(a, c.reserve_cus, st) : launch_wino4_t<0, false>(a, c.reserve_cus, st);
}

}
```

### fast-artistic-videos_amd/csrc/net.cpp

```cpp
#include <algorithm>
#include <cmath>
#include <cstdlib>
#include <cstring>
#include <functional>
#include <memory>

#include <mutex>
#include <unistd.h>

#include "fav_internal.h"
#include "wino_pack.h"
#include "wino4_pack.h"
#include "up2_pack.h"
#include "s2_pack.h"
#include "first_pack.h"
#include "first2d_pack.h"

using namespace fav;

namespace {

struct DevBuf { void* p = nullptr; size_t bytes = 0; };
struct DevConvW {
    float* wgt = nullptr; float* bias = nullptr; unsigned short* wgt16 = nullptr;
    float* packed[CONV_KERNELS] = {};
    int cinp = 0, coutp = 0, kpad = 0;
};
struct DevIN { float* gamma = nullptr; float* beta = nullptr; float* scale = nullptr; float* shift = nullptr;
               long long* acc = nullptr; size_t acc_bytes = 0; };

struct Act {
    float* data = nullptr;
    int Hp = 0, Wp = 0;
    int C = 0;
    int ups = 0;
    Affine pre;
    float* partials = nullptr;
    int mblocks = 0, ppitch = 0;
    int* counts = nullptr;
    int pitch = 0;
    const float* join_skip = nullptr; float* join_out = nullptr;
    long long* acc = nullptr; long long* acc_other = nullptr;
    int H() const { return Hp << ups; }
    int W() const { return Wp << ups; }
    int P() const { return pitch ? pitch : Wp; }
};

int dev_upload(const std::vector<float>& h, size_t pad_to, float** out)
{
    const size_t n = std::max(pad_to, h.size());
    std::vector<float> tmp(n, 0.f);
    std::copy(h.begin(), h.end(), tmp.begin());
    FAV_HIP(hipMalloc(reinterpret_cast<void**>(out), (n ? n : 1) * sizeof(float)));
    if (n) FAV_HIP(hipMemcpy(*out, tmp.data(), n * sizeof(float), hipMemcpyHostToDevice));
    return FAV_OK;
}

void repack_weights(const Layer& L, int cinp, int coutp, int kpad, std::vector<float>& out)
{
    out.assign((size_t)coutp * kpad, 0.f);
    const int taps = L.k * L.k;
    for (int co = 0; co < L.cout; ++co)
// ... 58 lines not shown
    case CK_FOLD:    return {0, false, 1};
    case CK_C8:      return {conv_c8_tiles(OH, OW), true, 8};
    case CK_C8D:     return {conv_c8_tiles(OH, OW), true, 7};
    case CK_FIRST1D: return {conv_first_tiles(OH, OW), true, 6};
    case CK_FIRST2D: return {conv_first2d_tiles(OH, OW), true, 16};
    case CK_S2W:     return {conv3s2w_tiles(OH, OW, coutp), true, 700 + coutp};
    case CK_UP2:     return {conv3_up2_tiles(OH, OW), true, 500 + coutp};
    case CK_WINO:    return {conv3_wino_tiles(OH, OW), true, 400 + coutp + (join ? 1 : 0)};
    case CK_WINO4:   return {conv3_wino4_tiles(OH, OW), true, 600 + coutp + (join ? 1 : 0)};
    case CK_HALO3:   return {conv3_halo_tiles(OH, OW, precision == 0), true, 300 + coutp};
    case CK_S2HALO:  return {conv3s2_tiles(OH, OW), true, 200 + coutp};
    }
    return {0, false, 0};
}

int launch_selected(ConvKernel k, const ConvLaunch& cs, const ConvLaunch& cg, const DevConvW& d, int cin_real, int* counts, hipStream_t st)
{
    const float* w = d.packed[k];
    switch (k) {
    case CK_GENERIC: return launch_conv(cg, st);
    case CK_FOLD:    return launch_conv_fold(cs, w, st);
    case CK_C8:      return launch_conv_c8(cs, counts, st);
    case CK_C8D:     return launch_conv_c8d(cs, cin_real, w, counts, st);
    case CK_FIRST1D: return launch_conv_first(cs, cin_real, w, counts, st);
    case CK_FIRST2D: return launch_conv_first2d(cs, cin_real, w, counts, st);
    case CK_S2W:     return launch_conv3s2w(cs, w, counts, st);
    case CK_UP2:     return launch_conv3_up2(cs, w, counts, st);
    case CK_WINO:    return launch_conv3_wino(cs, w, counts, st);
    case CK_WINO4:   return launch_conv3_wino4(cs, w, counts, st);
    case CK_HALO3:   return launch_conv3_halo(cg, counts, st);
    case CK_S2HALO:  return launch_conv3s2(tuning().side_sk == 2 ? cs : cg, counts, st);
    }
    set_error("internal: unknown convolution kernel %d", (int)k); return FAV_EINVAL;
}

int append_stage(Affine& a, const float* scale, const float* shift, int relu)
{
    if (a.stages >= 2) { set_error("network: more than two stacked normalisations on one tensor are unsupported"); return FAV_EUNSUPPORTED; }
    if (a.stages == 0) { a.scale1 = scale; a.shift1 = shift; a.relu1 = relu; }
    else { a.scale2 = scale; a.shift2 = shift; a.relu2 = relu; }
    ++a.stages;
    return FAV_OK;
}

bool only_tail(const std::vector<Layer>& ls, size_t from, bool& has_tanh, float& mul);
int pow2_ceil(int c) { int p = 4; while (p < c) p <<= 1; return p; }

int pad_channel_counts(std::vector<Layer>& ls, int& chan, int& real, bool& seen_conv, bool top)
{
    for (size_t li = 0; li < ls.size(); ++li) {
        Layer& L = ls[li];
        if (L.type == L_CONV) {
            const bool first_input = !seen_conv && L.cin <= 8;
            seen_conv = true;
            const int cin_new = first_input ? L.cin : chan;
            bool has_tanh = false; float mul = 1.f;
            const bool is_final = top && L.cout == 3 && only_tail(ls, li + 1, has_tanh, mul) && has_tanh;
            const int cout_new = is_final ? L.cout : pow2_ceil(L.cout);
            if (!first_input && L.cin != real) { set_error("network: conv expects %d input channels, its producer has %d", L.cin, real); return FAV_EFORMAT; }
            const int cout_real = L.cout;
            if (cin_new != L.cin || cout_new != L.cout) {
                std::vector<float> w((size_t)cout_new * cin_new * L.k * L.k, 0.f);
                const size_t kk = (size_t)L.k * L.k;
                for (int co = 0; co < L.cout; ++co)
                    for (int ci = 0; ci < L.cin; ++ci) {
                        const float* src = L.transposed ? &L.w[((size_t)ci * L.cout + co) * kk] : &L.w[((size_t)co * L.cin + ci) * kk];
// ... 32 lines not shown
    return n;
}

bool only_tail(const std::vector<Layer>& ls, size_t from, bool& has_tanh, float& mul)
{
    has_tanh = false; mul = 1.f;
    for (size_t i = from; i < ls.size(); ++i) {
        if (ls[i].type == L_TANH) { if (has_tanh) return false; has_tanh = true; }
        else if (ls[i].type == L_MUL) { if (!has_tanh) return false; mul *= ls[i].mul; }
        else if (ls[i].type != L_IDENTITY) return false;
    }
    return true;
}

}

struct fav_net {
    int device = 0;
    std::vector<Layer> layers;
    std::vector<Layer> exec;
    int pad = 0;
    bool pad_folded = false;
    int in_channels = 0;
    long long params = 0;
    std::vector<DevConvW> convs;
    std::vector<DevIN> ins;
    float* ones = nullptr; float* zeros = nullptr;
    float* sk_ws = nullptr; unsigned* sk_flags = nullptr; unsigned sk_epoch = 0;
    float* ks_ws = nullptr; int* ks_cnt = nullptr;
    struct LazyOut { bool active = false; int pitch = 0, rows = 0, shave = 0, conv_index = -1; } lazy;
    unsigned* sk_err_host = nullptr; unsigned* sk_err_dev = nullptr;
    bool shared_device = false;
    int precision = 0;
    int acc_parity = 0;
    bool acc_dirty = false;
    bool branch_tail_acc_ok = false;
    int reserve_cus = 0;
    int curH = 0, curW = 0;
    std::vector<DevBuf> bufs;
    std::vector<void*> slabs; char* slab_cur = nullptr; size_t slab_left = 0;
    size_t cursor = 0, conv_cursor = 0, in_cursor = 0;
    hipStream_t st = nullptr;
    float* stage = nullptr; size_t stage_bytes = 0;
    bool profiling = false;
    struct ProfRec { hipEvent_t a, b; int conv; };
    std::vector<ProfRec> prof_pending;
    std::vector<double> prof_ms, prof_macs; std::vector<int> prof_n, prof_tile;

    ~fav_net()
    {
        (void)hipSetDevice(device);
        (void)hipFree(stage);
        for (auto& c : convs) { (void)hipFree(c.wgt); (void)hipFree(c.bias); (void)hipFree(c.wgt16); for (float* p : c.packed) (void)hipFree(p); }
        for (auto& i : ins) { (void)hipFree(i.gamma); (void)hipFree(i.beta); (void)hipFree(i.scale); (void)hipFree(i.shift); (void)hipFree(i.acc); }
        for (void* sp : slabs) (void)hipFree(sp);
        (void)hipFree(ones); (void)hipFree(zeros); (void)hipFree(sk_ws); (void)hipFree(sk_flags); (void)hipFree(ks_ws); (void)hipFree(ks_cnt); if (sk_err_host) (void)hipHostFree(sk_err_host);
    }
    int upload_layers(std::vector<Layer>& ls, int& chan_pitch, int& maxc);
    int upload();
    int alloc(size_t bytes, float** out);
    int timed_conv(const ConvLaunch& c, int conv_index, const Layer& L, ConvKernel kernel, int* counts);
    int run(std::vector<Layer>& ls, Act& cur, bool top, float* out_planar, float* out_raw);
    bool res_block_is_winograd(const Layer& R, size_t first_conv) const;
    bool acc_stats_ok(const std::vector<Layer>& ls, size_t li) const;
    int forward_padded(const float* in8, int H, int W, float* out_planar, float* out_raw, hipStream_t stream);
    int forward_padded_unordered(const float* in8, int H, int W, float* out_planar, float* out_raw, hipStream_t stream);
    void out_size(int H, int W, int* Ho, int* Wo) const;
};

int fav_net::upload_layers(std::vector<Layer>& ls, int& chan_pitch, int& maxc)
{
    for (Layer& L : ls) {
        if (L.type == L_CONV) {
            convs.emplace_back();
            DevConvW& d = convs.back();
            d.cinp = chan_pitch;
            if (L.cin > chan_pitch || (chan_pitch != 8 && L.cin != chan_pitch)) {
                set_error("network: conv expects %d input channels, producer has %d", L.cin, chan_pitch); return FAV_EFORMAT; }
            if (L.k < 1 || L.stride < 1 || L.pad < 0) { set_error("network: bad convolution geometry"); return FAV_EFORMAT; }
            if ((d.cinp & (d.cinp - 1)) != 0) {
                set_error("network: a convolution with %d input channels is unsupported (channel counts must be powers of two)", d.cinp);
                return FAV_EUNSUPPORTED; }
            d.coutp = (L.cout + 31) / 32 * 32;
            d.kpad = (L.k * L.k * d.cinp + 31) / 32 * 32;
            std::vector<float> w;
            repack_weights(L, d.cinp, d.coutp, d.kpad, w);
            int rc = dev_upload(w, 0, &d.wgt); if (rc) return rc;
            rc = dev_upload(L.b, (size_t)d.coutp, &d.bias); if (rc) return rc;
            if (!L.transposed && conv3_halo_eligible(d.cinp, d.coutp, L.k, L.stride)) {
                std::vector<unsigned short> w16(w.size());
                for (size_t i = 0; i < w.size(); ++i) { unsigned b; memcpy(&b, &w[i], 4); w16[i] = (unsigned short)((b + 0x7FFFu + ((b >> 16) & 1u)) >> 16); }
                FAV_HIP(hipMalloc(reinterpret_cast<void**>(&d.wgt16), w16.size() * 2));
                FAV_HIP(hipMemcpy(d.wgt16, w16.data(), w16.size() * 2, hipMemcpyHostToDevice));
            }
            if (L.transposed && (L.stride != 2 || L.adj != 1 || L.pad > L.k - 1)) {
                set_error("network: SpatialFullConvolution is supported for stride 2, adj 1 (models_video.lua:99-102), got s=%d adj=%d", L.stride, L.adj);
                return FAV_EUNSUPPORTED; }
// ... 115 lines not shown
    FAV_HIP(hipMemset(sk_flags, 0, conv_streamk_grid() * sizeof(unsigned)));
    FAV_HIP(hipMalloc(reinterpret_cast<void**>(&ks_ws), conv3_wino4_ksplit_bytes()));
    FAV_HIP(hipMalloc(reinterpret_cast<void**>(&ks_cnt), 256 * sizeof(int)));
    FAV_HIP(hipMemset(ks_cnt, 0, 256 * sizeof(int)));
    FAV_HIP(hipHostMalloc(reinterpret_cast<void**>(&sk_err_host), sizeof(unsigned), hipHostMallocMapped));
    *sk_err_host = 0;
    FAV_HIP(hipHostGetDevicePointer(reinterpret_cast<void**>(&sk_err_dev), sk_err_host, 0));
    return FAV_OK;
}

int fav_net::alloc(size_t bytes, float** out)
{
    bytes = (bytes + 255) / 256 * 256;
    if (cursor < bufs.size()) {
        if (bufs[cursor].bytes < bytes) { set_error("internal: activation arena mismatch"); return FAV_EINVAL; }
        *out = static_cast<float*>(bufs[cursor++].p);
        return FAV_OK;
    }
    if (slab_left < bytes) {
        const size_t sz = std::max(bytes, (size_t)256 << 20);
        void* sp = nullptr;
        FAV_HIP(hipMalloc(&sp, sz));
        slabs.push_back(sp); slab_cur = static_cast<char*>(sp); slab_left = sz;
    }
    DevBuf b; b.bytes = bytes; b.p = slab_cur;
    slab_cur += bytes; slab_left -= bytes;
    bufs.push_back(b); ++cursor;
    *out = static_cast<float*>(b.p);
    return FAV_OK;
}

int fav_net::timed_conv(const ConvLaunch& c, int conv_index, const Layer& L, ConvKernel kernel, int* counts)
{
    if (c.pre.acc1 != nullptr && kernel != CK_WINO4) { set_error("internal: accumulator-form InstanceNorm in front of a kernel that cannot take it"); return FAV_EINVAL; }
    ConvLaunch cs = c;
    cs.reserve_cus = reserve_cus;
    cs.no_sk = shared_device ? 1 : 0;
    cs.sk_ws = sk_ws; cs.sk_flags = sk_flags; cs.sk_epoch = ++sk_epoch;
    cs.sk_err = sk_err_dev;
    cs.ks_ws = ks_ws; cs.ks_cnt = ks_cnt;
    if (sk_epoch == 0xffffffffu) sk_epoch = 0;
    ConvLaunch cg = cs;
    if (reserve_cus > 0 && tuning().side_sk != 1) cg.no_sk = 1;
    auto go = [&]() { return launch_selected(kernel, cs, cg, convs[conv_index], L.cin, counts, st); };
    char tag[96] = "";
    if (TraceRange::enabled()) snprintf(tag, sizeof tag, "fav:conv%d k%d s%d %d->%d %dx%d", conv_index, L.k, L.stride, L.cin, L.cout, c.OW, c.OH);
    TraceRange tr(tag);
    if (!profiling) return go();
    ProfRec r; r.conv = conv_index;
    FAV_HIP(hipEventCreateWithFlags(&r.a, hipEventDisableSystemFence)); FAV_HIP(hipEventCreateWithFlags(&r.b, hipEventDisableSystemFence));
    FAV_HIP(hipEventRecord(r.a, st));
    int rc = go();
    FAV_HIP(hipEventRecord(r.b, st));
    prof_pending.push_back(r);
    if ((int)prof_ms.size() <= conv_index) { prof_ms.resize(conv_index + 1, 0.0); prof_macs.resize(conv_index + 1, 0.0); prof_n.resize(conv_index + 1, 0); prof_tile.resize(conv_index + 1, 0); }
    prof_macs[conv_index] = (double)c.OH * c.OW * L.cout * L.cin * L.k * L.k;
    prof_tile[conv_index] = conv_facts(kernel, c.OH, c.OW, c.COUTp, precision, c.join_skip != nullptr).id;
    return rc;
}

static int count_convs(const std::vector<Layer>& ls)
{
    int n = 0;
    for (const Layer& l : ls) { if (l.type == L_CONV) ++n; else if (l.type == L_RES) n += count_convs(l.block); }
    return n;
}

bool fav_net::acc_stats_ok(const std::vector<Layer>& ls, size_t li) const
{
    if (tuning().no_acc_stats) return false;
    if (li + 3 >= ls.size() || ls[li + 1].type != L_IN || ls[li + 2].type != L_RELU || ls[li + 3].type != L_CONV) return false;
    if (conv_cursor >= convs.size()) return false;
    const Layer& c2 = ls[li + 3]; const DevConvW& d2 = convs[conv_cursor];
    return select_conv(c2, d2, 1, 0, precision, false, 0, 0, tuning()) == CK_WINO4;
}

bool fav_net::res_block_is_winograd(const Layer& R, size_t first_conv) const
{
    const std::vector<Layer>& b = R.block;
    if (b.size() != 5 || b[0].type != L_CONV || b[1].type != L_IN || b[2].type != L_RELU || b[3].type != L_CONV || b[4].type != L_IN) return false;
    if (first_conv + 1 >= convs.size()) return false;
    for (int k = 0; k < 2; ++k) {
        const Layer& c = b[k ? 3 : 0]; const DevConvW& d = convs[first_conv + (size_t)k];
        const ConvKernel kernel = select_conv(c, d, 1, 0, precision, false, 0, 0, tuning());
        if ((kernel != CK_WINO && kernel != CK_WINO4) || d.packed[CK_WINO] == nullptr) return false;
    }
    return true;
}

int fav_net::run(std::vector<Layer>& ls, Act& cur, bool top, float* out_planar, float* out_raw)
{
    for (size_t li = 0; li < ls.size(); ++li) {
        Layer& L = ls[li];
        switch (L.type) {
        case L_PAD: {
            if (top && li == 0 && pad_folded) break;
            if (cur.data == nullptr || cur.join_skip != nullptr) { set_error("network: misplaced padding layer"); return FAV_EUNSUPPORTED; }
            if (L.pad_mode == 0 && (std::max(L.pl, L.pr) >= cur.W() || std::max(L.pt, L.pb) >= cur.H())) { set_error("network: reflection padding %d %d %d %d of a %dx%d tensor", L.pl, L.pr, L.pt, L.pb, cur.W(), cur.H()); return FAV_EINVAL; }
            Act nxt;
            nxt.Hp = cur.H() + L.pt + L.pb; nxt.Wp = cur.W() + L.pl + L.pr; nxt.C = cur.C; nxt.pre = cur.pre;
            if (nxt.pre.acc1 != nullptr) { set_error("internal: accumulator-form InstanceNorm in front of a padding layer"); return FAV_EINVAL; }
            int rc = alloc((size_t)nxt.Hp * nxt.Wp * nxt.C * sizeof(float), &nxt.data); if (rc) return rc;
            rc = launch_pad_nhwc(cur.data, cur.Hp, cur.Wp, cur.P(), cur.C, cur.ups, nxt.data, L.pl, L.pr, L.pt, L.pb, L.pad_mode, st); if (rc) return rc;
            cur = nxt;
            break;
        }
        case L_CONV: {
            const DevConvW& d = convs[conv_cursor++];
            if (cur.C != d.cinp) { set_error("internal: channel pitch mismatch (%d vs %d)", cur.C, d.cinp); return FAV_EINVAL; }
            ConvLaunch c;
            c.in = cur.data; c.IH = cur.H(); c.IW = cur.W(); c.IWp = cur.P(); c.ups = cur.ups; c.CIN = d.cinp;
            c.pre = cur.pre;
            c.wgt = d.wgt; c.bias = d.bias; c.COUT = L.cout; c.COUTp = d.coutp; c.KH = c.KW = L.k; c.stride = L.stride;
            c.pad = L.pad; c.Kpad = d.kpad;
            if (L.transposed) {
                if (cur.ups != 0) { set_error("network: SpatialFullConvolution directly after an upsampling is unsupported"); return FAV_EUNSUPPORTED; }
                c.ups = 1; c.stuff = 1; c.IH = 2 * cur.Hp; c.IW = 2 * cur.Wp; c.stride = 1; c.pad = L.k - 1 - L.pad;
                c.OH = c.IH + 2 * c.pad - L.k + 1; c.OW = c.IW + 2 * c.pad - L.k + 1;
            } else {
                c.OH = (c.IH + 2 * L.pad - L.k) / L.stride + 1;
                c.OW = (c.IW + 2 * L.pad - L.k) / L.stride + 1;
            }
            if (c.IH + 2 * c.pad < L.k || c.IW + 2 * c.pad < L.k) { set_error("network: input too small for the architecture"); return FAV_EINVAL; }
            bool has_tanh = false; float mul = 1.f;
            const bool is_final = top && only_tail(ls, li + 1, has_tanh, mul) && has_tanh && L.cout == 3;
            const ConvKernel kernel = select_conv(L, d, cur.pre.stages, cur.ups, precision, is_final, c.IH, c.IW, tuning());
            Act nxt;
            nxt.Hp = c.OH; nxt.Wp = c.OW; nxt.C = L.cout;
            if (is_final && L.transposed) { set_error("network: a transposed convolution as the last layer is unsupported"); return FAV_EUNSUPPORTED; }
            if (is_final) {
                c.final_mode = 1; c.tanh_mul = mul; c.out_planar = out_planar; c.out_raw_nchw = out_raw;
                int rc = timed_conv(c, (int)conv_cursor - 1, L, kernel, nullptr); if (rc) return rc;
                cur = nxt;
                return FAV_OK;
            }
            if (L.cout % 4 != 0) { set_error("network: %d output channels (must be a multiple of 4 except for the last layer)", L.cout); return FAV_EUNSUPPORTED; }
            const bool pitched_out = lazy.active && (int)conv_cursor - 1 == lazy.conv_index;
            int rc;
            if (pitched_out) {
                if (c.OH != lazy.rows - 2 * lazy.shave || c.OW > lazy.pitch - 2 * lazy.shave) { set_error("internal: pending residual join of mismatching shapes"); return FAV_EINVAL; }
                float* base = nullptr;
                rc = alloc((size_t)lazy.rows * lazy.pitch * L.cout * sizeof(float), &base); if (rc) return rc;
                nxt.data = base + ((size_t)lazy.shave * lazy.pitch + lazy.shave) * L.cout; nxt.pitch = lazy.pitch; c.OWp = lazy.pitch;
            } else { rc = alloc((size_t)c.OH * c.OW * L.cout * sizeof(float), &nxt.data); if (rc) return rc; }
            const bool want_stats = li + 1 < ls.size() && ls[li + 1].type == L_IN;
            const ConvFacts facts = conv_facts(kernel, c.OH, c.OW, d.coutp, precision, cur.join_skip != nullptr);
            nxt.mblocks = facts.tiles; nxt.ppitch = d.coutp;
            const bool acc = kernel == CK_WINO4 && want_stats && !pitched_out && cur.join_skip == nullptr &&
                             (acc_stats_ok(ls, li) || (branch_tail_acc_ok && !top && li + 2 == ls.size() && !tuning().no_acc_stats && precision == 0));
            if (acc) {
                DevIN& din = ins[in_cursor];
                nxt.acc = din.acc + (size_t)acc_parity * stat_acc_words(L.cout); nxt.acc_other = din.acc + (size_t)(acc_parity ^ 1) * stat_acc_words(L.cout);
                c.stat_acc = nxt.acc;
            }
            if (want_stats && !acc) { rc = alloc((size_t)nxt.mblocks * d.coutp * 2 * sizeof(float), &nxt.partials); if (rc) return rc; }
            if (want_stats && !acc && facts.counts) { float* cp = nullptr; rc = alloc((size_t)nxt.mblocks * sizeof(int), &cp); if (rc) return rc; nxt.counts = reinterpret_cast<int*>(cp); }
            c.out = nxt.data; c.partials = nxt.partials;
            if (cur.join_skip != nullptr || pitched_out) {
                if (kernel != CK_WINO && kernel != CK_WINO4) { set_error("internal: a pending residual join next to a convolution that is not the Winograd kernel's"); return FAV_EINVAL; }
                c.join_skip = cur.join_skip; c.join_out = cur.join_out;
            }
            if (kernel == CK_HALO3 && precision == 1) c.wgt16 = d.wgt16;
            int* counts = facts.counts ? (nxt.counts ? nxt.counts : reinterpret_cast<int*>(zeros)) : nullptr;
            rc = timed_conv(c, (int)conv_cursor - 1, L, kernel, counts); if (rc) return rc;
            cur = nxt;
            break;
        }
        case L_IN: {
            const DevIN& d = ins[in_cursor++];
            const int C = (int)L.gamma.size();
            const int M = cur.Hp * cur.Wp;
            if (cur.data == nullptr || C != cur.C) { set_error("network: misplaced InstanceNormalization"); return FAV_EUNSUPPORTED; }
            if (cur.acc != nullptr && cur.pre.stages == 0) {
                cur.pre = Affine();
                cur.pre.acc1 = cur.acc; cur.pre.acc1_zero = cur.acc_other; cur.pre.gamma1 = d.gamma; cur.pre.beta1 = d.beta; cur.pre.eps1 = L.eps; cur.pre.count1 = M;
                cur.pre.relu1 = 0; cur.pre.stages = 1;
            } else if (cur.partials != nullptr && cur.pre.stages == 0) {
                int rc = launch_in_finalize(cur.partials, cur.counts, cur.mblocks, M, CONV_BM, C, cur.ppitch, d.gamma, d.beta, L.eps,
                                            d.scale, d.shift, st);
                if (rc) return rc;
                rc = append_stage(cur.pre, d.scale, d.shift, 0); if (rc) return rc;
            } else {
                Affine normalised = cur.pre;
                int rc = append_stage(normalised, d.scale, d.shift, 0); if (rc) return rc;
                float* part = nullptr;
                const int mb = (M + 127) / 128;
                rc = alloc((size_t)mb * C * 2 * sizeof(float), &part); if (rc) return rc;
                rc = launch_stats(cur.data, M, C, cur.pre, part, st); if (rc) return rc;
                rc = launch_in_finalize(part, nullptr, mb, M, 128, C, C, d.gamma, d.beta, L.eps, d.scale, d.shift, st); if (rc) return rc;
                cur.pre = normalised;
            }
            cur.partials = nullptr; cur.counts = nullptr; cur.acc = nullptr; cur.acc_other = nullptr;
            break;
        }
        case L_BN: {
            const DevIN& d = ins[in_cursor++];
            if (cur.data == nullptr || (int)L.mean.size() != cur.C) { set_error("network: misplaced SpatialBatchNormalization"); return FAV_EUNSUPPORTED; }
            int rc = append_stage(cur.pre, d.scale, d.shift, 0); if (rc) return rc;
            cur.partials = nullptr; cur.counts = nullptr;
            break;
        }
        case L_RELU:
            if (cur.pre.stages == 0) (void)append_stage(cur.pre, ones, zeros, 1);
            else if (cur.pre.stages == 1) cur.pre.relu1 = 1;
            else cur.pre.relu2 = 1;
            cur.partials = nullptr;
            break;
        case L_UP:
            if (L.scale != 2 || cur.ups != 0) { set_error("network: only a single x2 nearest upsampling per convolution is supported"); return FAV_EUNSUPPORTED; }
            cur.ups = 1;
            break;
        case L_RES: {
            if (cur.ups != 0) { set_error("network: residual block directly after an upsampling is unsupported"); return FAV_EUNSUPPORTED; }
            Act skip = cur;
            Act br = cur;
            br.partials = nullptr;
            int rc;
            if (cur.join_skip != nullptr) {
                float* zb = nullptr;
                rc = alloc((size_t)cur.Hp * cur.P() * cur.C * sizeof(float), &zb); if (rc) return rc;
                br.join_out = zb;
                skip = Act(); skip.data = zb; skip.Hp = cur.Hp; skip.Wp = cur.Wp; skip.C = cur.C; skip.pitch = cur.P();
            }
            const int nconv = count_convs(L.block);
            const bool lazy_out = !tuning().no_lazy_join && (tuning().wino_f2 || tuning().lazy_join) && precision == 0 &&
                                  li + 1 < ls.size() && ls[li + 1].type == L_RES && skip.pre.stages == 0 && skip.ups == 0 &&
                                  res_block_is_winograd(L, conv_cursor) && res_block_is_winograd(ls[li + 1], conv_cursor + (size_t)nconv);
            if (lazy_out) { lazy.active = true; lazy.pitch = skip.P(); lazy.rows = skip.Hp; lazy.shave = L.shave; lazy.conv_index = (int)conv_cursor + nconv - 1; }
            size_t nx = li + 1;
            if (nx < ls.size() && ls[nx].type == L_UP && ls[nx].scale == 2) ++nx;
            const bool join_stats = nx < ls.size() && ls[nx].type == L_IN;
            branch_tail_acc_ok = !lazy_out && !join_stats;
            rc = run(L.block, br, false, nullptr, nullptr);
            lazy.active = false; branch_tail_acc_ok = false;
            if (rc) return rc;
            if (br.pre.stages != 1 || br.pre.relu1 || br.ups != 0) { set_error("network: residual branch must end in conv + InstanceNormalization"); return FAV_EUNSUPPORTED; }
            if (br.Hp != skip.Hp - 2 * L.shave || br.Wp != skip.Wp - 2 * L.shave || br.C != skip.C) {
                set_error("network: residual branch output %dx%d does not match the shaved skip %dx%d", br.Wp, br.Hp,
                          skip.Wp - 2 * L.shave, skip.Hp - 2 * L.shave);
                return FAV_EUNSUPPORTED; }
            if (lazy_out) {
                cur = br;
                cur.partials = nullptr; cur.counts = nullptr;
                cur.join_skip = skip.data + ((size_t)L.shave * skip.P() + L.shave) * skip.C; cur.join_out = nullptr;
                break;
            }
            Act z; z.Hp = br.Hp; z.Wp = br.Wp; z.C = br.C;
            rc = alloc((size_t)z.Hp * z.Wp * z.C * sizeof(float), &z.data); if (rc) return rc;
            if (join_stats) {
                z.mblocks = res_add_stat_blocks(z.Hp, z.Wp); z.ppitch = z.C;
                rc = alloc((size_t)z.mblocks * z.C * 2 * sizeof(float), &z.partials); if (rc) return rc;
                float* cp = nullptr; rc = alloc((size_t)z.mblocks * sizeof(int), &cp); if (rc) return rc; z.counts = reinterpret_cast<int*>(cp);
            }
            rc = launch_res_add(br.data, br.pre.scale1, br.pre.shift1, skip.data, skip.Hp, skip.Wp, L.shave, skip.pre, z.C,
                                z.data, z.partials, z.counts, st, skip.P(), &br.pre);
            if (rc) return rc;
            cur = z;
            break;
        }
        case L_TANH: case L_MUL:
            set_error("network: Tanh/MulConstant are only supported after the last convolution"); return FAV_EUNSUPPORTED;
        case L_IDENTITY: break;
        }
    }
    if (top) { set_error("network: the model does not end in a 3-channel convolution followed by Tanh"); return FAV_EUNSUPPORTED; }
    return FAV_OK;
}

void fav_net::out_size(int H, int W, int* Ho, int* Wo) const
{
    int h = H + 2 * pad, w = W + 2 * pad;
    std::function<void(const std::vector<Layer>&)> walk = [&](const std::vector<Layer>& ls) {
        for (const Layer& L : ls) {
            if (L.type == L_PAD) { if (&L == &layers[0] && pad_folded) continue; h += L.pt + L.pb; w += L.pl + L.pr; }
            else if (L.type == L_CONV && L.transposed) { h = (h - 1) * L.stride - 2 * L.pad + L.k + L.adj; w = (w - 1) * L.stride - 2 * L.pad + L.k + L.adj; }
            else if (L.type == L_CONV) { h = (h + 2 * L.pad - L.k) / L.stride + 1; w = (w + 2 * L.pad - L.k) / L.stride + 1; }
            else if (L.type == L_UP) { h *= L.scale; w *= L.scale; }
            else if (L.type == L_RES) walk(L.block);
        }
    };
    walk(layers);
    *Ho = h; *Wo = w;
}

namespace {
struct DeviceOrder { std::mutex mu; hipStream_t last = nullptr; bool valid = false; };
DeviceOrder& device_order(int device)
{
// ... 21 lines not shown
{
    FAV_HIP(hipSetDevice(device));
    DeviceOrder& ord = device_order(device);
    std::lock_guard<std::mutex> order_lock(ord.mu);
    if (ord.valid && ord.last != stream && hipStreamSynchronize(ord.last) != hipSuccess)
        (void)hipGetLastError();
    ord.valid = true; ord.last = stream;
    return forward_padded_unordered(in8, H, W, out_planar, out_raw, stream);
}

int fav_net::forward_padded_unordered(const float* in8, int H, int W, float* out_planar, float* out_raw, hipStream_t stream)
{
    if (sk_err_host && *reinterpret_cast<volatile unsigned*>(sk_err_host)) {
        *sk_err_host = 0;
        shared_device = true;
        set_error("a stream-K hand-off between convolution blocks timed out in an earlier launch of this network: its result was "
                  "wrong (two networks running concurrently on one device? see the concurrency note in fav.h)");
        return FAV_EHIP;
    }
    if (H != curH || W != curW) {
        if (!bufs.empty()) {
            FAV_HIP(hipDeviceSynchronize());
            for (void* sp : slabs) (void)hipFree(sp);
            slabs.clear(); slab_cur = nullptr; slab_left = 0;
            bufs.clear();
        }
        curH = H; curW = W;
    }
    st = stream; cursor = 0; conv_cursor = 0; in_cursor = 0;
    if (acc_dirty) {
        for (DevIN& i : ins) if (i.acc) FAV_HIP(hipMemsetAsync(i.acc, 0, i.acc_bytes, stream));
        acc_dirty = false;
    }
    if (precision == 0 && !tuning().no_acc_stats && !tuning().no_wino) acc_parity ^= 1;
    Act cur;
    cur.data = const_cast<float*>(in8); cur.Hp = H + 2 * pad; cur.Wp = W + 2 * pad; cur.C = 8;
    const int rc = run(exec, cur, true, out_planar, out_raw);
    if (rc) acc_dirty = true;
    return rc;
}

static int finish_create(fav_net* net, fav_net** out)
{
    int rc = net->upload();
    if (rc) { delete net; return rc; }
    *out = net;
    return FAV_OK;
}

extern "C" int fav_net_create(const char* t7_path_host, int device, fav_net** out)
{
    FAV_REQUIRE(t7_path_host && out, "fav_net_create: null argument");
    int rc = ensure_device(); if (rc) return rc;
    FAV_ABI_TRY
    std::unique_ptr<fav_net> net(new fav_net());
    net->device = device;
    rc = t7_parse_model(t7_path_host, net->layers);
    if (rc) return rc;
    return finish_create(net.release(), out);
    FAV_ABI_CATCH("fav_net_create")
}

extern "C" int fav_net_pack_host(const char* t7_path_host, void* blob_host, size_t capacity, size_t* bytes)
{
    FAV_REQUIRE(t7_path_host && bytes, "fav_net_pack_host: null argument");
    FAV_ABI_TRY
    std::vector<Layer> layers;
// ... 564 lines not shown
```

Baseline: 658.9.

## Extend fixed-point atomic InstanceNorm statistics to stats, res-add and first-layer kernels

Generalizes the accumulator-form InstanceNorm statistics (fixed-point atomics into striped copies) to the standalone stats kernel, the statistics-taking residual join, and the first-layer conv. Each block accumulates its tiles locally and flushes once with atomics, and consumers rebuild scale and shift from the accumulator in-kernel. This removes the separate in_finalize launches and the partials round-trips. It adds a grid-stride loop with a capped grid, per-block recomputation of the affine table, and wider overflow limits, which risk precision or parity edge cases.

Measured after the change: 660.1, median of 5. Within noise of the previous version (+0.2%).

```diff
diff --git a/fast-artistic-videos_amd/csrc/fav_internal.h b/fast-artistic-videos_amd/csrc/fav_internal.h
--- a/fast-artistic-videos_amd/csrc/fav_internal.h
+++ b/fast-artistic-videos_amd/csrc/fav_internal.h
@@ -84,16 +84,22 @@
 int blob_unpack(const void* blob, size_t bytes, std::vector<Layer>& out);
 std::string describe_layers(const std::vector<Layer>& layers, int indent = 0);
 
+struct StatAcc {
+    const long long* acc = nullptr; long long* zero = nullptr;
+    const float* gamma = nullptr; const float* beta = nullptr; float eps = 0.f; int count = 0;
+    float* scale_out = nullptr; float* shift_out = nullptr;
+};
 struct Affine {
     const float* scale1 = nullptr; const float* shift1 = nullptr; int relu1 = 0;
     const float* scale2 = nullptr; const float* shift2 = nullptr; int relu2 = 0;
     int stages = 0;
-    const long long* acc1 = nullptr; long long* acc1_zero = nullptr;
-    const float* gamma1 = nullptr; const float* beta1 = nullptr; float eps1 = 0.f; int count1 = 0;
+    StatAcc acc;
 };
 constexpr int STAT_COPIES = 8;
 inline size_t stat_acc_words(int C) { return (size_t)STAT_COPIES * C * 4; }
-constexpr long long STAT_NONFINITE = 1ll << 53;
+constexpr long long STAT_NONFINITE = 1ll << 61;
+constexpr double STAT_TILE_LIMIT = 0x1p76;
+constexpr long long STAT_RUN_LIMIT = 1ll << 50;
 __host__ __device__ inline bool stat_acc_poisoned(long long hi_sum, long long hi_squares)
 {
     return hi_sum >= STAT_NONFINITE / 2 || hi_sum <= -(STAT_NONFINITE / 2) || hi_squares >= STAT_NONFINITE / 2 || hi_squares <= -(STAT_NONFINITE / 2);
@@ -148,6 +154,7 @@
 int launch_conv3s2(const ConvLaunch& p, int* counts, hipStream_t st);
 bool conv_fold_eligible(int cin_pitch, int cout, int k, int stride);
 bool conv_fold_launchable(int cin_pitch, int k, int pad, int ups, int IH, int IW);
+bool conv_fold_takes_acc(int cin_pitch, int k, int pad, int ups, int IH, int IW);
 int launch_conv_fold(const ConvLaunch& p, const float* wfold, hipStream_t st);
 int conv_first_tiles(int OH, int OW);
 int launch_conv_first(const ConvLaunch& p, int cin_real, const float* wpk, int* counts, hipStream_t st);
@@ -162,6 +169,7 @@
 int launch_conv3_wino4(const ConvLaunch& p, const float* wpk, int* counts, hipStream_t st);
 bool conv3_up2_eligible(int cin_pitch, int cout, int coutp, int k, int stride, int pad, int stages, int ups);
 int conv3_up2_tiles(int OH, int OW);
+bool conv3_up2_takes_acc(int coutp);
 int launch_conv3_up2(const ConvLaunch& p, const float* wpk, int* counts, hipStream_t st);
 bool conv3s2w_eligible(int cin_pitch, int cout, int coutp, int k, int stride, int pad, int stages, int ups);
 int conv3s2w_tiles(int OH, int OW, int coutp);
@@ -171,11 +179,12 @@
 int launch_in_finalize(const float* partials, const int* counts, int mblocks, int M, int block_pixels, int C, int Cpitch,
                        const float* gamma, const float* beta, float eps,
                        float* scale, float* shift, hipStream_t st);
-int launch_stats(const float* x, int M, int C, const Affine& t, float* partials, hipStream_t st);
+int launch_stats(const float* x, int M, int C, const Affine& t, float* partials, hipStream_t st, long long* stat_acc = nullptr);
 int launch_pad_nhwc(const float* in, int Hp, int Wp, int in_pitch, int C, int ups, float* out, int pl, int pr, int pt, int pb, int mode, hipStream_t st);
 int launch_res_add(const float* y, const float* scale, const float* shift,
                    const float* skip, int SH, int SW, int shave, const Affine& skip_t,
-                   int C, float* z, float* partials, int* counts, hipStream_t st, int skip_pitch = 0, const Affine* branch_acc = nullptr);
+                   int C, float* z, float* partials, int* counts, hipStream_t st, int skip_pitch = 0, const Affine* branch_acc = nullptr,
+                   long long* stat_acc = nullptr);
 inline int res_add_stat_blocks(int OH, int OW) { return OH * ((OW + 127) / 128); }
 int launch_nchw_to_nhwc_pad(const float* in, int C, int H, int W, int pad, int Cp, float* out, hipStream_t st);
 int launch_nhwc_to_nchw(const float* in, int M, int C, const Affine& t, float* out, hipStream_t st);
diff --git a/fast-artistic-videos_amd/csrc/kernels_elem.hip b/fast-artistic-videos_amd/csrc/kernels_elem.hip
--- a/fast-artistic-videos_amd/csrc/kernels_elem.hip
+++ b/fast-artistic-videos_amd/csrc/kernels_elem.hip
@@ -2,6 +2,7 @@
 
 #include "fav_internal.h"
 #include "conv_device.h"
+#include "stat_acc.h"
 
 namespace fav {
 
@@ -56,17 +57,27 @@
 }
 
 template <int NPT>
-__global__ __launch_bounds__(256) void stats_kernel(const float* x, int M, int C, const Affine a, float2* partials)
+__global__ __launch_bounds__(256) void stats_kernel(const float* x, int M, int C, const Affine a_in, float2* partials, long long* stat_acc)
 {
     __shared__ float red[1024];
     __shared__ float mean_s[1024];
+    __shared__ float ss[2048];
     const int t = threadIdx.x;
+    Affine a = a_in;
+    if (a.acc.acc != nullptr) {
+        stat_acc_table<256>(a.acc, C, ss, ss + C);
+        __syncthreads();
+        if (a.stages >= 2) { a.scale2 = ss; a.shift2 = ss + C; } else { a.scale1 = ss; a.shift1 = ss + C; }
+    }
     const int groups = C >> 2;
     const int nl = 256 / groups;
     const int g = t % groups, pl = t / groups;
-    const int m0 = blockIdx.x * 128;
+    const bool active = pl < nl;
+    StatAccRun run;
+    const int nblk = (M + 127) / 128;
+    for (int blk = blockIdx.x; blk < nblk; blk += gridDim.x) {
+    const int m0 = blk * 128;
     const int cnt = min(128, M - m0);
-    const bool active = pl < nl;
     float4 s = make_float4(0, 0, 0, 0);
     float4 keep[NPT > 0 ? NPT : 1];
     if (NPT > 0) {
@@ -116,40 +127,22 @@
     for (int c = t; c < C; c += 256) {
         float r = 0;
         for (int i = 0; i < nl; ++i) r += red[i * C + c];
-        partials[(size_t)blockIdx.x * C + c] = make_float2(mean_s[c], r);
-    }
+        if (stat_acc != nullptr) run.add(cnt, mean_s[c], r);
+        else partials[(size_t)blk * C + c] = make_float2(mean_s[c], r);
+    }
+    __syncthreads();
+    }
+    if (stat_acc != nullptr && t < C) run.flush(stat_acc, C, t);
 }
 
 template <bool ACC>
 __global__ __launch_bounds__(256) void res_add_kernel(const float* y, const float* scale, const float* shift,
                                                       const float* skip, int SW, int shave, const Affine sa,
-                                                      int OH, int OW, int C, float* z, const Affine br)
+                                                      int OH, int OW, int C, float* z, const StatAcc br)
 {
     __shared__ float ss[ACC ? 2048 : 4];
     if (ACC) {
-        for (int i = threadIdx.x; i < C; i += 256) {
-            long long w0 = 0, w1 = 0, w2 = 0, w3 = 0;
-#pragma unroll
-            for (int cp = 0; cp < STAT_COPIES; ++cp) {
-                const longlong2* a = reinterpret_cast<const longlong2*>(br.acc1 + ((size_t)cp * C + i) * 4);
-                const longlong2 lo = a[0], hi = a[1];
-                w0 += lo.x; w1 += lo.y; w2 += hi.x; w3 += hi.y;
-            }
-            const double s1 = ((double)w1 * 4294967296.0 + (double)w0) * (1.0 / 1099511627776.0);
-            const double s2 = ((double)w3 * 4294967296.0 + (double)w2) * (1.0 / 1099511627776.0);
-            const double mean = s1 / (double)br.count1;
-            double var = s2 / (double)br.count1 - mean * mean;
-            var = var > 0.0 ? var : 0.0;
-            const double sc = stat_acc_poisoned(w1, w3) ? (double)NAN : (double)br.gamma1[i] / sqrt(var + (double)br.eps1);
-            ss[i] = (float)sc; ss[C + i] = (float)((double)br.beta1[i] - mean * sc);
-            if (blockIdx.x == 0) {
-#pragma unroll
-                for (int cp = 0; cp < STAT_COPIES; ++cp) {
-                    longlong2* zz = reinterpret_cast<longlong2*>(br.acc1_zero + ((size_t)cp * C + i) * 4);
-                    zz[0] = longlong2{0, 0}; zz[1] = longlong2{0, 0};
-                }
-            }
-        }
+        stat_acc_table<256>(br, C, ss, ss + C);
         __syncthreads();
         scale = ss; shift = ss + C;
     }
@@ -171,17 +164,25 @@
 template <int NPT>
 __global__ __launch_bounds__(256) void res_add_stats_kernel(const float* y, const float* scale, const float* shift,
                                                             const float* skip, int SW, int shave, const Affine sa,
-                                                            int OW, int C, float* z, float2* partials, int* counts)
+                                                            int OH, int OW, int C, float* z, float2* partials, int* counts, const StatAcc br, long long* stat_acc)
 {
     __shared__ float red[1024];
     __shared__ float mean_s[1024];
+    __shared__ float ss[2048];
     const int t = threadIdx.x;
+    if (br.acc != nullptr) {
+        stat_acc_table<256>(br, C, ss, ss + C);
+        __syncthreads();
+        scale = ss; shift = ss + C;
+    }
     const int groups = C >> 2, nl = 256 / groups;
     const int g = t % groups, pl = t / groups;
     const int segs = (OW + 127) / 128;
-    const int oy = blockIdx.x / segs, x0 = (blockIdx.x - oy * segs) * 128;
+    const bool active = pl < nl;
+    StatAccRun run;
+    for (int blk = blockIdx.x; blk < OH * segs; blk += gridDim.x) {
+    const int oy = blk / segs, x0 = (blk - oy * segs) * 128;
     const int cnt = min(128, OW - x0);
-    const bool active = pl < nl;
     const float* yr = y + ((size_t)oy * OW + x0) * C + 4 * g;
     const float* kr = skip + ((size_t)(oy + shave) * SW + x0 + shave) * C + 4 * g;
     float* zr = z + ((size_t)oy * OW + x0) * C + 4 * g;
@@ -244,9 +245,13 @@
     for (int c = t; c < C; c += 256) {
         float r = 0;
         for (int i = 0; i < nl; ++i) r += red[i * C + c];
-        partials[(size_t)blockIdx.x * C + c] = make_float2(mean_s[c], r);
-    }
-    if (t == 0) counts[blockIdx.x] = cnt;
+        if (stat_acc != nullptr) run.add(cnt, mean_s[c], r);
+        else partials[(size_t)blk * C + c] = make_float2(mean_s[c], r);
+    }
+    if (t == 0 && stat_acc == nullptr) counts[blk] = cnt;
+    __syncthreads();
+    }
+    if (stat_acc != nullptr && t < C) run.flush(stat_acc, C, t);
 }
 
 __device__ __forceinline__ int reflect(int i, int n)
@@ -299,38 +304,49 @@
     return FAV_OK;
 }
 
-int launch_stats(const float* x, int M, int C, const Affine& t, float* partials, hipStream_t st)
+inline int capped_grid(int nblk) { const int rounds = (nblk + 1023) / 1024; return rounds ? (nblk + rounds - 1) / rounds : 1; }
+
+int launch_stats(const float* x, int M, int C, const Affine& t, float* partials, hipStream_t st, long long* stat_acc)
 {
     FAV_REQUIRE(C % 4 == 0 && C <= 1024 && 256 % (C / 4) == 0, "stats: unsupported channel count %d", C);
-    const dim3 grid((M + 127) / 128);
+    FAV_REQUIRE(stat_acc == nullptr || C <= 256, "stats: accumulator-form statistics take at most 256 channels (%d)", C);
+    FAV_REQUIRE(t.acc.acc == nullptr || (t.stages >= 1 && t.acc.count > 0), "stats: accumulator-form InstanceNorm without a stage");
+    const int nblk = (M + 127) / 128;
+    const dim3 grid(stat_acc != nullptr || t.acc.acc != nullptr ? capped_grid(nblk) : nblk);
     float2* pp = reinterpret_cast<float2*>(partials);
-    if (C == 64) hipLaunchKernelGGL(stats_kernel<8>, grid, dim3(256), 0, st, x, M, C, t, pp);
-    else if (C == 128) hipLaunchKernelGGL(stats_kernel<16>, grid, dim3(256), 0, st, x, M, C, t, pp);
-    else hipLaunchKernelGGL(stats_kernel<0>, grid, dim3(256), 0, st, x, M, C, t, pp);
+    if (C == 64) hipLaunchKernelGGL(stats_kernel<8>, grid, dim3(256), 0, st, x, M, C, t, pp, stat_acc);
+    else if (C == 128) hipLaunchKernelGGL(stats_kernel<16>, grid, dim3(256), 0, st, x, M, C, t, pp, stat_acc);
+    else hipLaunchKernelGGL(stats_kernel<0>, grid, dim3(256), 0, st, x, M, C, t, pp, stat_acc);
     FAV_LAUNCH_CHECK("stats_kernel");
     return FAV_OK;
 }
 
 int launch_res_add(const float* y, const float* scale, const float* shift, const float* skip, int SH, int SW,
-                   int shave, const Affine& skip_t, int C, float* z, float* partials, int* counts, hipStream_t st, int skip_pitch, const Affine* branch_acc)
+                   int shave, const Affine& skip_t, int C, float* z, float* partials, int* counts, hipStream_t st, int skip_pitch, const Affine* branch_acc,
+                   long long* stat_acc)
 {
     const int OH = SH - 2 * shave, OW = SW - 2 * shave;
     if (skip_pitch > 0) SW = skip_pitch;
     FAV_REQUIRE(C % 4 == 0 && C <= 1024 && 256 % (C / 4) == 0 && OH > 0 && OW > 0, "res_add: bad shape (C=%d)", C);
-    FAV_REQUIRE(!(partials && branch_acc && branch_acc->acc1), "res_add: the statistics-taking join does not take an accumulator-form InstanceNorm");
-    if (partials) {
-        const dim3 grid(res_add_stat_blocks(OH, OW));
+    const bool bacc = branch_acc != nullptr && branch_acc->acc.acc != nullptr;
+    FAV_REQUIRE(skip_t.acc.acc == nullptr, "res_add: the skip side does not take an accumulator-form InstanceNorm");
+    FAV_REQUIRE(!bacc || (branch_acc->stages == 1 && branch_acc->acc.count > 0), "res_add: accumulator-form InstanceNorm of a branch that does not end in one");
+    FAV_REQUIRE(stat_acc == nullptr || C <= 256, "res_add: accumulator-form statistics take at most 256 channels (%d)", C);
+    if (partials || stat_acc) {
+        const int nblk = res_add_stat_blocks(OH, OW);
+        const dim3 grid(bacc || stat_acc ? capped_grid(nblk) : nblk);
         float2* pp = reinterpret_cast<float2*>(partials);
-        if (C == 128) hipLaunchKernelGGL(res_add_stats_kernel<16>, grid, dim3(256), 0, st, y, scale, shift, skip, SW, shave, skip_t, OW, C, z, pp, counts);
-        else if (C == 64) hipLaunchKernelGGL(res_add_stats_kernel<8>, grid, dim3(256), 0, st, y, scale, shift, skip, SW, shave, skip_t, OW, C, z, pp, counts);
-        else hipLaunchKernelGGL(res_add_stats_kernel<0>, grid, dim3(256), 0, st, y, scale, shift, skip, SW, shave, skip_t, OW, C, z, pp, counts);
-    }
-    else if (branch_acc != nullptr && branch_acc->acc1 != nullptr)
+        const StatAcc br = bacc ? branch_acc->acc : StatAcc();
+        if (C == 128) hipLaunchKernelGGL(res_add_stats_kernel<16>, grid, dim3(256), 0, st, y, scale, shift, skip, SW, shave, skip_t, OH, OW, C, z, pp, counts, br, stat_acc);
+        else if (C == 64) hipLaunchKernelGGL(res_add_stats_kernel<8>, grid, dim3(256), 0, st, y, scale, shift, skip, SW, shave, skip_t, OH, OW, C, z, pp, counts, br, stat_acc);
+        else hipLaunchKernelGGL(res_add_stats_kernel<0>, grid, dim3(256), 0, st, y, scale, shift, skip, SW, shave, skip_t, OH, OW, C, z, pp, counts, br, stat_acc);
+    }
+    else if (bacc)
         hipLaunchKernelGGL(res_add_kernel<true>, dim3(std::min(1024, grid_for((size_t)OH * OW * (C / 4)))), dim3(256), 0, st, y, scale, shift, skip, SW, shave, skip_t,
-                           OH, OW, C, z, *branch_acc);
+                           OH, OW, C, z, branch_acc->acc);
     else
         hipLaunchKernelGGL(res_add_kernel<false>, dim3(grid_for((size_t)OH * OW * (C / 4))), dim3(256), 0, st, y, scale, shift, skip, SW, shave, skip_t,
-                           OH, OW, C, z, Affine());
+                           OH, OW, C, z, StatAcc());
     FAV_LAUNCH_CHECK("res_add_kernel");
     return FAV_OK;
 }
diff --git a/fast-artistic-videos_amd/csrc/kernels_first.hip b/fast-artistic-videos_amd/csrc/kernels_first.hip
--- a/fast-artistic-videos_amd/csrc/kernels_first.hip
+++ b/fast-artistic-videos_amd/csrc/kernels_first.hip
@@ -4,6 +4,7 @@
 
 #include "fav_internal.h"
 #include "conv_device.h"
+#include "stat_acc.h"
 #include "launch_common.h"
 #include "first_pack.h"
 #include "first2d_pack.h"
@@ -23,6 +24,7 @@
 struct FirstArgs {
     const float* in; const float* wpk; const float* bias;
     float* out; float2* partials; int* counts;
+    long long* stat_acc;
     int IH, IW, IWp, COUT, pad, OH, OW, tiles_x, tiles_y;
     int COUTP, groups;
     long long* dbg = nullptr;
@@ -295,6 +297,7 @@
 #else
 #define G_DBG(i_)
 #endif
+    StatAccRun run;
     for (; tile < ntiles; tile += tstep) {
         const int nxt = tile + tstep;
         G_LOAD_HALO(nxt);
@@ -444,8 +447,12 @@
             __syncthreads();
             if (t < 32) {
                 int n;
-                p.partials[(size_t)tile * PITCH + grp * 32 + t] = merge_rows(st, wn, t, &n);
-                if (t == 0 && grp == 0) p.counts[tile] = n;
+                const float2 ms = merge_rows(st, wn, t, &n);
+                if (!WIDE && p.stat_acc != nullptr) run.add(n, ms.x, ms.y);
+                else {
+                    p.partials[(size_t)tile * PITCH + grp * 32 + t] = ms;
+                    if (t == 0 && grp == 0) p.counts[tile] = n;
+                }
             }
         }
         __syncthreads();
@@ -454,6 +461,7 @@
         ++ntl_;
 #endif
     }
+    if (!WIDE && p.stat_acc != nullptr && t < 32) run.flush(p.stat_acc, 32, t);
 #ifdef FAV_DIAG
     if (p.dbg && t == 0) { for (int i = 0; i < 5; ++i) p.dbg[blockIdx.x * 8 + i] = dt_[i]; p.dbg[blockIdx.x * 8 + 5] = ntl_; }
 #endif
@@ -508,6 +516,7 @@
     FAV_REQUIRE((long long)c.IH * c.IWp * 8 < (1ll << 31), "first-layer conv: bad shape");
     FirstArgs a;
     a.in = c.in; a.wpk = wpk; a.bias = c.bias; a.out = c.out; a.partials = reinterpret_cast<float2*>(c.partials); a.counts = counts;
+    a.stat_acc = nullptr;
     a.IH = c.IH; a.IW = c.IW; a.IWp = c.IWp; a.COUT = c.COUT; a.pad = c.pad; a.OH = c.OH; a.OW = c.OW;
     a.tiles_x = (c.OW + F_TW - 1) / F_TW; a.tiles_y = (c.OH + F_TH - 1) / F_TH;
     return cin_real == 7 ? launch_first_t<7>(a, c.reserve_cus, st) : launch_first_t<3>(a, c.reserve_cus, st);
@@ -529,6 +538,9 @@
     a.IH = c.IH; a.IW = c.IW; a.IWp = c.IWp; a.COUT = c.COUT; a.pad = c.pad; a.OH = c.OH; a.OW = c.OW;
     a.tiles_x = (c.OW + G_TW - 1) / G_TW; a.tiles_y = (c.OH + G_TH - 1) / G_TH;
     a.COUTP = c.COUTp; a.groups = c.COUTp / 32; a.dbg = nullptr;
+    a.stat_acc = c.stat_acc;
+    FAV_REQUIRE(c.stat_acc == nullptr || c.COUTp == 32, "first-layer conv: accumulator-form statistics take one group of 32 filters");
+    if (c.stat_acc != nullptr && a.partials == nullptr) a.partials = reinterpret_cast<float2*>(c.stat_acc);
     if (a.groups > 1) return cin_real == 7 ? launch_first2d_t<7, true>(a, c.reserve_cus, st) : launch_first2d_t<3, true>(a, c.reserve_cus, st);
     return cin_real == 7 ? launch_first2d_t<7>(a, c.reserve_cus, st) : launch_first2d_t<3>(a, c.reserve_cus, st);
 }
diff --git a/fast-artistic-videos_amd/csrc/kernels_fold.hip b/fast-artistic-videos_amd/csrc/kernels_fold.hip
--- a/fast-artistic-videos_amd/csrc/kernels_fold.hip
+++ b/fast-artistic-videos_amd/csrc/kernels_fold.hip
@@ -4,6 +4,7 @@
 
 #include "fav_internal.h"
 #include "conv_device.h"
+#include "stat_acc.h"
 #include "launch_common.h"
 
 namespace fav {
@@ -19,6 +20,7 @@
     float* out_planar; float* out_raw;
     int IH, IW, IWp, ups, COUT, KH, KW, pad, OH, OW;
     int stages, relu1, relu2;
+    StatAcc acc2;
     float tanh_mul;
     int tiles_x, tiles_y;
     long long* dbg;
@@ -191,7 +193,8 @@
     {                                                                                               \
         for (int i = t; i < CIN; i += NT) {                                                         \
             aff[i] = p.stages >= 1 ? p.scale1[(hoff_) + i] : 1.f; aff[CIN + i] = p.stages >= 1 ? p.shift1[(hoff_) + i] : 0.f; \
-            aff[2 * CIN + i] = p.stages >= 2 ? p.scale2[(hoff_) + i] : 1.f; aff[3 * CIN + i] = p.stages >= 2 ? p.shift2[(hoff_) + i] : 0.f; \
+            if (NH == 1 && p.acc2.acc != nullptr) stat_acc_affine(p.acc2, CT, i, blockIdx.x == 0, aff + 2 * CIN + i, aff + 3 * CIN + i); \
+            else { aff[2 * CIN + i] = p.stages >= 2 ? p.scale2[(hoff_) + i] : 1.f; aff[3 * CIN + i] = p.stages >= 2 ? p.shift2[(hoff_) + i] : 0.f; } \
         }                                                                                           \
         for (int e = t; e < (p.KH + 1) * 32 * (CIN / 4); e += NT) {                                 \
             const int row = e / (CIN / 4), c4 = e - row * (CIN / 4);                                \
@@ -403,6 +406,15 @@
 {
     return stride == 1 && cout * k <= 32 && k <= 9 && (cin_pitch == 16 || cin_pitch == 32 || cin_pitch == 64 || cin_pitch == 128 || cin_pitch == 256);
 }
+static bool fold_up2_form(int k, int pad, int ups, int IH, int IW)
+{
+    static const bool no_up2 = diag_env("FAV_NO_FOLD_UP2") != nullptr;
+    return ups == 1 && !no_up2 && (pad & 1) == 0 && (k & 1) == 1 && (IH & 1) == 0 && (IW & 1) == 0 && k + 1 <= 10;
+}
+bool conv_fold_takes_acc(int cin_pitch, int k, int pad, int ups, int IH, int IW)
+{
+    return (cin_pitch == 64 || cin_pitch == 32) && fold_up2_form(k, pad, ups, IH, IW);
+}
 bool conv_fold_launchable(int cin_pitch, int k, int pad, int ups, int IH, int IW)
 {
     static const bool no_up2 = diag_env("FAV_NO_FOLD_UP2") != nullptr;
@@ -418,6 +430,9 @@
     a.in = c.in; a.wfold = wfold; a.bias = c.bias;
     a.scale1 = c.pre.scale1; a.shift1 = c.pre.shift1; a.scale2 = c.pre.scale2; a.shift2 = c.pre.shift2;
     a.stages = c.pre.stages; a.relu1 = c.pre.relu1; a.relu2 = c.pre.relu2;
+    a.acc2 = c.pre.acc;
+    FAV_REQUIRE(a.acc2.acc == nullptr || (c.pre.stages == 2 && a.acc2.count > 0 && conv_fold_takes_acc(c.CIN, c.KH, c.pad, c.ups, c.IH, c.IW)),
+                "row-folded conv: accumulator-form InstanceNorm on an unsupported input");
     a.out_planar = c.out_planar; a.out_raw = c.out_raw_nchw;
     a.IH = c.IH; a.IW = c.IW; a.IWp = c.IWp; a.ups = c.ups; a.COUT = c.COUT; a.KH = c.KH; a.KW = c.KW; a.pad = c.pad;
     a.OH = c.OH; a.OW = c.OW; a.tanh_mul = c.tanh_mul;
diff --git a/fast-artistic-videos_amd/csrc/kernels_s2.hip b/fast-artistic-videos_amd/csrc/kernels_s2.hip
--- a/fast-artistic-videos_amd/csrc/kernels_s2.hip
+++ b/fast-artistic-videos_amd/csrc/kernels_s2.hip
@@ -3,6 +3,7 @@
 
 #include "fav_internal.h"
 #include "conv_device.h"
+#include "stat_acc.h"
 #include "launch_common.h"
 #include "s2_pack.h"
 
@@ -18,6 +19,7 @@
     float* out; float2* partials; int* counts;
     int IH, IW, IWp, CIN, OH, OW, pad, tiles_x, tiles_y, stages, relu1;
     int COUTP, groups;
+    StatAcc acc1; long long* stat_acc;
 };
 
 template <int NTC, int TR> struct SwGeo {
@@ -73,7 +75,9 @@
         hyx[i] = hy << 16 | hx;
         hbase[i] = ((pe < HP ? (hy * p.IWp + hx) * p.CIN : 0) + c4 * 4) * 4;
     }
-    for (int i = t; i < CIN; i += NTH) { aff[i] = p.stages >= 1 ? p.scale1[i] : 1.f; aff[CIN + i] = p.stages >= 1 ? p.shift1[i] : 0.f; }
+    if (p.acc1.acc != nullptr) stat_acc_table<NTH>(p.acc1, CIN, aff, aff + CIN);
+    else for (int i = t; i < CIN; i += NTH) { aff[i] = p.stages >= 1 ? p.scale1[i] : 1.f; aff[CIN + i] = p.stages >= 1 ? p.shift1[i] : 0.f; }
+    StatAccRun run;
     const float lo1 = (p.stages >= 1 && p.relu1) ? 0.f : -INFINITY;
     const float* const affr = aff + c4 * 4;
 
@@ -187,8 +191,11 @@
                     const float mean = cnt ? s1 / (float)cnt : 0.f;
                     float m2 = 0.f;
                     for (int w = 0; w < TR; ++w) { const float d = stt[w * COUT + t].x - mean; m2 += stt[w * COUT + t].y + (float)wn[w] * d * d; }
-                    p.partials[(size_t)pend * PITCH + grp * COUT + t] = make_float2(mean, m2);
-                    if (t == 0 && grp == 0) p.counts[pend] = cnt;
+                    if (!WIDE && p.stat_acc != nullptr) run.add(cnt, mean, m2);
+                    else {
+                        p.partials[(size_t)pend * PITCH + grp * COUT + t] = make_float2(mean, m2);
+                        if (t == 0 && grp == 0) p.counts[pend] = cnt;
+                    }
                 }
                 pend = -1;
             }
@@ -254,10 +261,14 @@
             const float mean = cnt ? s1 / (float)cnt : 0.f;
             float m2 = 0.f;
             for (int w = 0; w < TR; ++w) { const float d = stt[w * COUT + t].x - mean; m2 += stt[w * COUT + t].y + (float)wn[w] * d * d; }
-            p.partials[(size_t)pend * PITCH + grp * COUT + t] = make_float2(mean, m2);
-            if (t == 0 && grp == 0) p.counts[pend] = cnt;
+            if (!WIDE && p.stat_acc != nullptr) run.add(cnt, mean, m2);
+            else {
+                p.partials[(size_t)pend * PITCH + grp * COUT + t] = make_float2(mean, m2);
+                if (t == 0 && grp == 0) p.counts[pend] = cnt;
+            }
         }
     }
+    if (!WIDE && p.stat_acc != nullptr && t < COUT) run.flush(p.stat_acc, COUT, t);
 #undef SW_AOFF
 #undef SW_ABASE
 #undef SW_TILE_SETUP
@@ -308,6 +319,10 @@
     S2wArgs a;
     a.in = c.in; a.wpk = wpk; a.bias = c.bias; a.scale1 = c.pre.scale1; a.shift1 = c.pre.shift1; a.stages = c.pre.stages; a.relu1 = c.pre.relu1;
     a.out = c.out; a.partials = reinterpret_cast<float2*>(c.partials); a.counts = counts;
+    a.acc1 = c.pre.acc; a.stat_acc = c.stat_acc;
+    FAV_REQUIRE(a.acc1.acc == nullptr || (c.pre.stages == 1 && a.acc1.count > 0), "stride-2 conv: accumulator-form InstanceNorm without a stage");
+    FAV_REQUIRE(c.stat_acc == nullptr || c.COUTp <= 128, "stride-2 conv: accumulator-form statistics take one group of filters");
+    if (c.stat_acc != nullptr && a.partials == nullptr) a.partials = reinterpret_cast<float2*>(c.stat_acc);
     a.IH = c.IH; a.IW = c.IW; a.IWp = c.IWp; a.CIN = c.CIN; a.OH = c.OH; a.OW = c.OW; a.pad = c.pad;
     const int tr = s2w_rows(c.COUTp);
     a.tiles_x = (c.OW + 31) / 32; a.tiles_y = (c.OH + tr - 1) / tr;
diff --git a/fast-artistic-videos_amd/csrc/kernels_up2.hip b/fast-artistic-videos_amd/csrc/kernels_up2.hip
--- a/fast-artistic-videos_amd/csrc/kernels_up2.hip
+++ b/fast-artistic-videos_amd/csrc/kernels_up2.hip
@@ -3,6 +3,7 @@
 
 #include "fav_internal.h"
 #include "conv_device.h"
+#include "stat_acc.h"
 #include "launch_common.h"
 #include "up2_pack.h"
 
@@ -17,6 +18,7 @@
 struct Up2Args {
     const float* in; const float* wpk; const float* bias; const float* scale1; const float* shift1;
     float* out; float2* partials; int* counts;
+    StatAcc acc1; long long* stat_acc;
     int PH, PW, IWp, CIN, tiles_x, tiles_y, relu1;
     int COUTP, groups;
 };
@@ -214,7 +216,10 @@
     const float* const rb = Hs + ((row + (kind == 0 ? 1 : kind == 1 ? 1 : 2)) * UW_HW + m) * LDSS + 4 * h;
     const int c4 = t & 7;
     float* const hst = Hs + (t >> 3) * LDSS + c4 * 4;
-    for (int i = t; i < CIN; i += 768) { aff[i] = p.scale1[i]; aff[CIN + i] = p.shift1[i]; }
+    if (!WIDE && p.acc1.acc != nullptr) stat_acc_table<768>(p.acc1, CIN, aff, aff + CIN);
+    else for (int i = t; i < CIN; i += 768) { aff[i] = p.scale1[i]; aff[CIN + i] = p.shift1[i]; }
+    long long* const runl = reinterpret_cast<long long*>(smem + UW_ZS + 2 * CIN + 2 * 4 * 64 + 8) + 5 * (t & 63);
+    if (t < 64) { runl[0] = 0; runl[1] = 0; runl[2] = 0; runl[3] = 0; runl[4] = 0; }
     __syncthreads();
     const float lo1 = p.relu1 ? 0.f : -INFINITY;
     const float* const affr = aff + c4 * 4;
@@ -385,10 +390,20 @@
             const float mean = cnt ? s1 / (float)cnt : 0.f;
             float m2 = 0.f;
             for (int w = 0; w < 4; ++w) { const float d = stt[w * 64 + t].x - mean; m2 += stt[w * 64 + t].y + (float)wn[w] * d * d; }
-            p.partials[(size_t)tile * PITCH + grp * 64 + t] = make_float2(mean, m2);
-            if (t == 0 && grp == 0) p.counts[tile] = cnt;
-        }
-        __syncthreads();
+            if (!WIDE && p.stat_acc != nullptr) {
+#pragma unroll
+                for (int k = 0; k < 4; ++k) { bool f; runl[k] += stat_acc_word(k, cnt, mean, m2, &f); if (!f) runl[4] = 1; }
+            } else {
+                p.partials[(size_t)tile * PITCH + grp * 64 + t] = make_float2(mean, m2);
+                if (t == 0 && grp == 0) p.counts[tile] = cnt;
+            }
+        }
+        __syncthreads();
+    }
+    if (!WIDE && p.stat_acc != nullptr && t < 64) {
+        StatAccRun run;
+        run.w[0] = runl[0]; run.w[1] = runl[1]; run.w[2] = runl[2]; run.w[3] = runl[3]; run.fin = runl[4] == 0;
+        run.flush(p.stat_acc, 64, t);
     }
 }
 
@@ -400,6 +415,7 @@
     return k == 3 && stride == 1 && pad == 1 && ups == 1 && stages == 1 && cin_pitch % 32 == 0 && cin_pitch >= 32 && cin_pitch <= 256 &&
            cout == coutp && (cout == 64 || (up2_winograd() && cout % 64 == 0 && cout <= 512));
 }
+bool conv3_up2_takes_acc(int coutp) { return up2_winograd() && coutp == 64; }
 int conv3_up2_tiles(int OH, int OW) { return ((OH / 2 + (up2_winograd() ? 3 : 7)) / (up2_winograd() ? 4 : 8)) * ((OW / 2 + 31) / 32); }
 
 int launch_conv3_up2(const ConvLaunch& c, const float* wpk, int* counts, hipStream_t st)
@@ -412,8 +428,12 @@
     a.in = c.in; a.wpk = wpk; a.bias = c.bias; a.scale1 = c.pre.scale1; a.shift1 = c.pre.shift1; a.relu1 = c.pre.relu1; a.out = c.out; a.partials = reinterpret_cast<float2*>(c.partials); a.counts = counts;
     a.PH = c.IH / 2; a.PW = c.IW / 2; a.IWp = c.IWp; a.CIN = c.CIN;
     const bool wg = up2_winograd();
+    a.acc1 = c.pre.acc; a.stat_acc = c.stat_acc;
+    FAV_REQUIRE((a.acc1.acc == nullptr && c.stat_acc == nullptr) || conv3_up2_takes_acc(c.COUTp), "upsampled 3x3 conv: accumulator forms on a kernel that does not take them");
+    FAV_REQUIRE(a.acc1.acc == nullptr || a.acc1.count > 0, "upsampled 3x3 conv: accumulator-form InstanceNorm without a count");
+    if (c.stat_acc != nullptr && a.partials == nullptr) a.partials = reinterpret_cast<float2*>(c.stat_acc);
     a.tiles_x = (a.PW + 31) / 32; a.tiles_y = wg ? (a.PH + 3) / 4 : (a.PH + 7) / 8;
-    const size_t lds = wg ? (size_t)(UW_ZS + 2 * c.CIN + 2 * 4 * 64 + 8) * sizeof(float)
+    const size_t lds = wg ? (size_t)(UW_ZS + 2 * c.CIN + 2 * 4 * 64 + 8 + 64 * 5 * 2) * sizeof(float)
                           : (size_t)(2 * U2_HB + 2 * c.CIN) * sizeof(float);
     static PerDevice cache; int cus;
     FAV_HIP(launch_cus(cache, &cus, conv3_up2_kernel<true>, conv3_up2w_kernel<false>, conv3_up2w_kernel<true>));
diff --git a/fast-artistic-videos_amd/csrc/kernels_wino4.hip b/fast-artistic-videos_amd/csrc/kernels_wino4.hip
--- a/fast-artistic-videos_amd/csrc/kernels_wino4.hip
+++ b/fast-artistic-videos_amd/csrc/kernels_wino4.hip
@@ -4,6 +4,7 @@
 #include <vector>
 
 #include "fav_internal.h"
+#include "stat_acc.h"
 #include "wino4_pack.h"
 
 namespace fav {
@@ -36,7 +37,7 @@
     int IH, IW, IWp, CIN, OH, OW, units_x, units_y, relu1;
     int stream, shares; float* ks_ws; int* ks_cnt;
     long long* dbg;
-    long long* stat_acc; const long long* acc1; long long* acc1_zero; const float* gamma1; const float* beta1; float eps1; int count1;
+    long long* stat_acc; StatAcc acc1;
     int COUT, groups;
 };
 
@@ -99,30 +100,8 @@
         const int nwg = gridDim.x, q = nwg >> 3, r = nwg & 7, xcd = blockIdx.x & 7, idx = blockIdx.x >> 3;
         lb = (xcd < r ? xcd * (q + 1) : r * (q + 1) + (xcd - r) * q) + idx;
     }
-    if (MODE == 1 && p.acc1 != nullptr) {
-        for (int i = t; i < CIN; i += NT) {
-            long long w0 = 0, w1 = 0, w2 = 0, w3 = 0;
-#pragma unroll
-            for (int cp = 0; cp < STAT_COPIES; ++cp) {
-                const longlong2* a = reinterpret_cast<const longlong2*>(p.acc1 + ((size_t)cp * CIN + i) * 4);
-                const longlong2 lo = a[0], hi = a[1];
-                w0 += lo.x; w1 += lo.y; w2 += hi.x; w3 += hi.y;
-            }
-            const double s1 = ((double)w1 * 4294967296.0 + (double)w0) * (1.0 / 1099511627776.0);
-            const double s2 = ((double)w3 * 4294967296.0 + (double)w2) * (1.0 / 1099511627776.0);
-            const double mean = s1 / (double)p.count1;
-            double var = s2 / (double)p.count1 - mean * mean;
-            var = var > 0.0 ? var : 0.0;
-            const double sc = stat_acc_poisoned(w1, w3) ? (double)NAN : (double)p.gamma1[i] / sqrt(var + (double)p.eps1);
-            aff[i] = (float)sc; aff[CIN + i] = (float)((double)p.beta1[i] - mean * sc);
-            if (blockIdx.x == 0) {
-#pragma unroll
-                for (int cp = 0; cp < STAT_COPIES; ++cp) {
-                    longlong2* z = reinterpret_cast<longlong2*>(p.acc1_zero + ((size_t)cp * CIN + i) * 4);
-                    z[0] = longlong2{0, 0}; z[1] = longlong2{0, 0};
-                }
-            }
-        }
+    if (MODE == 1 && p.acc1.acc != nullptr) {
+        stat_acc_table<NT>(p.acc1, CIN, aff, aff + CIN);
     } else if (AFF) for (int i = t; i < CIN; i += NT) { aff[i] = p.scale1[i]; aff[CIN + i] = p.shift1[i]; }
     const float lo1 = (MODE == 1 && p.relu1) ? 0.f : -INFINITY;
 
@@ -445,14 +424,9 @@
         if (p.partials != nullptr) {
             m2 += __shfl_xor(m2, 16); m2 += __shfl_xor(m2, 32);
             if (p.stat_acc != nullptr) {
-                const double nd = (double)nv, mud = (double)mu;
-                const double v = (g & 2) ? (double)m2 + nd * mud * mud : nd * mud;
-                const double tt = v * 1099511627776.0;
-                const double hi = floor(tt * (1.0 / 4294967296.0));
-                const bool fin = fabs(tt) < 9.0e18;
-                const long long word = !fin ? ((g & 1) ? STAT_NONFINITE : 0ll) : (g & 1) ? (long long)hi : (long long)(tt - hi * 4294967296.0);
-                long long* const dst = p.stat_acc + ((size_t)(blockIdx.x & (STAT_COPIES - 1)) * (WIDE ? p.COUT : 128) + cb) * 4 + g;
-                __hip_atomic_fetch_add(dst, word, __ATOMIC_RELAXED, __HIP_MEMORY_SCOPE_AGENT);
+                bool fin;
+                const long long word = stat_acc_word(g, nv, mu, m2, &fin);
+                stat_acc_commit(p.stat_acc, WIDE ? p.COUT : 128, cb, g, word, fin);
             } else if (g == 0) p.partials[(size_t)u * (WIDE ? p.COUT : 128) + cb] = make_float2(mu, m2);
         }
         if (p.partials != nullptr && p.stat_acc == nullptr && t == 0 && grp == 0) p.counts[u] = nv;
@@ -570,9 +544,9 @@
     a.skip = c.join_skip; a.zout = c.join_out; a.OWp = c.OWp > 0 ? c.OWp : c.OW;
     a.ks_ws = c.ks_ws; a.ks_cnt = c.ks_cnt; a.stream = 0; a.shares = 1;
     a.COUT = c.COUT; a.groups = c.COUT / 128;
-    a.stat_acc = c.stat_acc; a.acc1 = c.pre.acc1; a.acc1_zero = c.pre.acc1_zero; a.gamma1 = c.pre.gamma1; a.beta1 = c.pre.beta1; a.eps1 = c.pre.eps1; a.count1 = c.pre.count1;
+    a.stat_acc = c.stat_acc; a.acc1 = c.pre.acc;
     if (c.stat_acc != nullptr && a.partials == nullptr) a.partials = reinterpret_cast<float2*>(c.stat_acc);
-    FAV_REQUIRE(c.pre.acc1 == nullptr || (c.join_skip == nullptr && c.pre.stages == 1 && c.pre.count1 > 0), "winograd F(4x4) conv: accumulator-form InstanceNorm on an unsupported input");
+    FAV_REQUIRE(c.pre.acc.acc == nullptr || (c.join_skip == nullptr && c.pre.stages == 1 && c.pre.acc.count > 0), "winograd F(4x4) conv: accumulator-form InstanceNorm on an unsupported input");
     if (c.join_skip != nullptr) {
         FAV_REQUIRE(c.join_out != nullptr && c.pre.stages == 1 && c.pre.relu1 == 0, "winograd F(4x4) conv: a pending residual join needs its output tensor and exactly one pending normalisation");
         FAV_REQUIRE(a.groups == 1, "winograd F(4x4) conv: a pending residual join is formed by 128-filter layers only");
diff --git a/fast-artistic-videos_amd/csrc/net.cpp b/fast-artistic-videos_amd/csrc/net.cpp
--- a/fast-artistic-videos_amd/csrc/net.cpp
+++ b/fast-artistic-videos_amd/csrc/net.cpp
@@ -27,7 +27,8 @@
     int cinp = 0, coutp = 0, kpad = 0;
 };
 struct DevIN { float* gamma = nullptr; float* beta = nullptr; float* scale = nullptr; float* shift = nullptr;
-               long long* acc = nullptr; size_t acc_bytes = 0; };
+               long long* acc = nullptr; size_t acc_bytes = 0;
+               int parity = 0; };
 
 struct Act {
     float* data = nullptr;
@@ -152,6 +153,25 @@
     case CK_S2HALO:  return launch_conv3s2(tuning().side_sk == 2 ? cs : cg, counts, st);
     }
     set_error("internal: unknown convolution kernel %d", (int)k); return FAV_EINVAL;
+}
+
+Affine plain_stages(const Affine& a)
+{
+    Affine r = a;
+    if (a.acc.acc != nullptr) {
+        if (a.stages >= 2) { r.scale2 = a.acc.scale_out; r.shift2 = a.acc.shift_out; } else { r.scale1 = a.acc.scale_out; r.shift1 = a.acc.shift_out; }
+        r.acc = StatAcc();
+    }
+    return r;
+}
+bool conv_takes_acc(ConvKernel k, int stages, int cinp, int coutp, int ksz, int pad, int ups, int IH, int IW)
+{
+    if (stages == 1) return k == CK_WINO4 || k == CK_S2W || (k == CK_UP2 && conv3_up2_takes_acc(coutp));
+    return stages == 2 && k == CK_FOLD && conv_fold_takes_acc(cinp, ksz, pad, ups, IH, IW);
+}
+bool conv_gives_acc(ConvKernel k, int coutp)
+{
+    return k == CK_WINO4 || (k == CK_FIRST2D && coutp == 32) || (k == CK_S2W && coutp <= 128) || (k == CK_UP2 && conv3_up2_takes_acc(coutp));
 }
 
 int append_stage(Affine& a, const float* scale, const float* shift, int relu)
@@ -250,7 +270,6 @@
     unsigned* sk_err_host = nullptr; unsigned* sk_err_dev = nullptr;
     bool shared_device = false;
     int precision = 0;
-    int acc_parity = 0;
     bool acc_dirty = false;
     bool branch_tail_acc_ok = false;
     int reserve_cus = 0;
@@ -280,7 +299,8 @@
     int timed_conv(const ConvLaunch& c, int conv_index, const Layer& L, ConvKernel kernel, int* counts);
     int run(std::vector<Layer>& ls, Act& cur, bool top, float* out_planar, float* out_raw);
     bool res_block_is_winograd(const Layer& R, size_t first_conv) const;
-    bool acc_stats_ok(const std::vector<Layer>& ls, size_t li) const;
+    bool acc_consumer_ok(const std::vector<Layer>& ls, size_t j, int stages, int ups, bool top, int H, int W) const;
+    void take_acc(DevIN& din, int C, Act& a);
     int forward_padded(const float* in8, int H, int W, float* out_planar, float* out_raw, hipStream_t stream);
     int forward_padded_unordered(const float* in8, int H, int W, float* out_planar, float* out_raw, hipStream_t stream);
     void out_size(int H, int W, int* Ho, int* Wo) const;
@@ -462,7 +482,7 @@
 
 int fav_net::timed_conv(const ConvLaunch& c, int conv_index, const Layer& L, ConvKernel kernel, int* counts)
 {
-    if (c.pre.acc1 != nullptr && kernel != CK_WINO4) { set_error("internal: accumulator-form InstanceNorm in front of a kernel that cannot take it"); return FAV_EINVAL; }
+    if (c.pre.acc.acc != nullptr && (!conv_takes_acc(kernel, c.pre.stages, c.CIN, c.COUTp, c.KH, c.pad, c.ups, c.IH, c.IW) || c.join_skip != nullptr)) { set_error("internal: accumulator-form InstanceNorm in front of a kernel that cannot take it"); return FAV_EINVAL; }
     ConvLaunch cs = c;
     cs.reserve_cus = reserve_cus;
     cs.no_sk = shared_device ? 1 : 0;
@@ -496,13 +516,31 @@
     return n;
 }
 
-bool fav_net::acc_stats_ok(const std::vector<Layer>& ls, size_t li) const
-{
-    if (tuning().no_acc_stats) return false;
-    if (li + 3 >= ls.size() || ls[li + 1].type != L_IN || ls[li + 2].type != L_RELU || ls[li + 3].type != L_CONV) return false;
+bool fav_net::acc_consumer_ok(const std::vector<Layer>& ls, size_t j, int stages, int ups, bool top, int H, int W) const
+{
+    if (tuning().no_acc_stats || precision != 0) return false;
+    bool relu = false;
+    if (j < ls.size() && ls[j].type == L_RELU) { relu = true; ++j; }
+    if (j < ls.size() && ls[j].type == L_UP && ls[j].scale == 2 && ups == 0) { ups = 1; ++j; }
+    if (j == ls.size()) return !top && !relu && ups == 0 && stages == 1 && branch_tail_acc_ok;
+    const Layer& N = ls[j];
+    if (N.type == L_IN) return stages == 1;
     if (conv_cursor >= convs.size()) return false;
-    const Layer& c2 = ls[li + 3]; const DevConvW& d2 = convs[conv_cursor];
-    return select_conv(c2, d2, 1, 0, precision, false, 0, 0, tuning()) == CK_WINO4;
+    const DevConvW& d = convs[conv_cursor];
+    if (N.type == L_RES)
+        return stages == 1 && ups == 0 && !N.block.empty() && N.block[0].type == L_CONV &&
+               select_conv(N.block[0], d, 1, 0, precision, false, 0, 0, tuning()) == CK_WINO4;
+    if (N.type != L_CONV) return false;
+    bool has_tanh = false; float mul = 1.f;
+    const bool is_final = top && only_tail(ls, j + 1, has_tanh, mul) && has_tanh && N.cout == 3;
+    const int IH = H << ups, IW = W << ups;
+    const ConvKernel k = select_conv(N, d, stages, ups, precision, is_final, IH, IW, tuning());
+    return conv_takes_acc(k, stages, d.cinp, d.coutp, N.k, N.pad, ups, IH, IW);
+}
+void fav_net::take_acc(DevIN& din, int C, Act& a)
+{
+    din.parity ^= 1;
+    a.acc = din.acc + (size_t)din.parity * stat_acc_words(C); a.acc_other = din.acc + (size_t)(din.parity ^ 1) * stat_acc_words(C);
 }
 
 bool fav_net::res_block_is_winograd(const Layer& R, size_t first_conv) const
@@ -529,7 +567,7 @@
             if (L.pad_mode == 0 && (std::max(L.pl, L.pr) >= cur.W() || std::max(L.pt, L.pb) >= cur.H())) { set_error("network: reflection padding %d %d %d %d of a %dx%d tensor", L.pl, L.pr, L.pt, L.pb, cur.W(), cur.H()); return FAV_EINVAL; }
             Act nxt;
             nxt.Hp = cur.H() + L.pt + L.pb; nxt.Wp = cur.W() + L.pl + L.pr; nxt.C = cur.C; nxt.pre = cur.pre;
-            if (nxt.pre.acc1 != nullptr) { set_error("internal: accumulator-form InstanceNorm in front of a padding layer"); return FAV_EINVAL; }
+            if (nxt.pre.acc.acc != nullptr) { set_error("internal: accumulator-form InstanceNorm in front of a padding layer"); return FAV_EINVAL; }
             int rc = alloc((size_t)nxt.Hp * nxt.Wp * nxt.C * sizeof(float), &nxt.data); if (rc) return rc;
             rc = launch_pad_nhwc(cur.data, cur.Hp, cur.Wp, cur.P(), cur.C, cur.ups, nxt.data, L.pl, L.pr, L.pt, L.pb, L.pad_mode, st); if (rc) return rc;
             cur = nxt;
@@ -576,11 +614,10 @@
             const bool want_stats = li + 1 < ls.size() && ls[li + 1].type == L_IN;
             const ConvFacts facts = conv_facts(kernel, c.OH, c.OW, d.coutp, precision, cur.join_skip != nullptr);
             nxt.mblocks = facts.tiles; nxt.ppitch = d.coutp;
-            const bool acc = kernel == CK_WINO4 && want_stats && !pitched_out && cur.join_skip == nullptr &&
-                             (acc_stats_ok(ls, li) || (branch_tail_acc_ok && !top && li + 2 == ls.size() && !tuning().no_acc_stats && precision == 0));
+            const bool acc = want_stats && conv_gives_acc(kernel, d.coutp) && !pitched_out && cur.join_skip == nullptr && d.coutp == L.cout &&
+                             acc_consumer_ok(ls, li + 2, 1, 0, top, c.OH, c.OW);
             if (acc) {
-                DevIN& din = ins[in_cursor];
-                nxt.acc = din.acc + (size_t)acc_parity * stat_acc_words(L.cout); nxt.acc_other = din.acc + (size_t)(acc_parity ^ 1) * stat_acc_words(L.cout);
+                take_acc(ins[in_cursor], L.cout, nxt);
                 c.stat_acc = nxt.acc;
             }
             if (want_stats && !acc) { rc = alloc((size_t)nxt.mblocks * d.coutp * 2 * sizeof(float), &nxt.partials); if (rc) return rc; }
@@ -603,7 +640,8 @@
             if (cur.data == nullptr || C != cur.C) { set_error("network: misplaced InstanceNormalization"); return FAV_EUNSUPPORTED; }
             if (cur.acc != nullptr && cur.pre.stages == 0) {
                 cur.pre = Affine();
-                cur.pre.acc1 = cur.acc; cur.pre.acc1_zero = cur.acc_other; cur.pre.gamma1 = d.gamma; cur.pre.beta1 = d.beta; cur.pre.eps1 = L.eps; cur.pre.count1 = M;
+                cur.pre.acc.acc = cur.acc; cur.pre.acc.zero = cur.acc_other; cur.pre.acc.gamma = d.gamma; cur.pre.acc.beta = d.beta; cur.pre.acc.eps = L.eps; cur.pre.acc.count = M;
+                cur.pre.acc.scale_out = d.scale; cur.pre.acc.shift_out = d.shift;
                 cur.pre.relu1 = 0; cur.pre.stages = 1;
             } else if (cur.partials != nullptr && cur.pre.stages == 0) {
                 int rc = launch_in_finalize(cur.partials, cur.counts, cur.mblocks, M, CONV_BM, C, cur.ppitch, d.gamma, d.beta, L.eps,
@@ -611,13 +649,21 @@
                 if (rc) return rc;
                 rc = append_stage(cur.pre, d.scale, d.shift, 0); if (rc) return rc;
             } else {
-                Affine normalised = cur.pre;
+                Affine normalised = plain_stages(cur.pre);
                 int rc = append_stage(normalised, d.scale, d.shift, 0); if (rc) return rc;
-                float* part = nullptr;
-                const int mb = (M + 127) / 128;
-                rc = alloc((size_t)mb * C * 2 * sizeof(float), &part); if (rc) return rc;
-                rc = launch_stats(cur.data, M, C, cur.pre, part, st); if (rc) return rc;
-                rc = launch_in_finalize(part, nullptr, mb, M, 128, C, C, d.gamma, d.beta, L.eps, d.scale, d.shift, st); if (rc) return rc;
+                if (C <= 256 && acc_consumer_ok(ls, li + 1, normalised.stages, cur.ups, top, cur.Hp, cur.Wp)) {
+                    Act own; take_acc(ins[in_cursor - 1], C, own);
+                    rc = launch_stats(cur.data, M, C, cur.pre, nullptr, st, own.acc); if (rc) return rc;
+                    if (normalised.stages >= 2) { normalised.scale2 = nullptr; normalised.shift2 = nullptr; } else { normalised.scale1 = nullptr; normalised.shift1 = nullptr; }
+                    normalised.acc.acc = own.acc; normalised.acc.zero = own.acc_other; normalised.acc.gamma = d.gamma; normalised.acc.beta = d.beta; normalised.acc.eps = L.eps;
+                    normalised.acc.count = M; normalised.acc.scale_out = d.scale; normalised.acc.shift_out = d.shift;
+                } else {
+                    float* part = nullptr;
+                    const int mb = (M + 127) / 128;
+                    rc = alloc((size_t)mb * C * 2 * sizeof(float), &part); if (rc) return rc;
+                    rc = launch_stats(cur.data, M, C, cur.pre, part, st); if (rc) return rc;
+                    rc = launch_in_finalize(part, nullptr, mb, M, 128, C, C, d.gamma, d.beta, L.eps, d.scale, d.shift, st); if (rc) return rc;
+                }
                 cur.pre = normalised;
             }
             cur.partials = nullptr; cur.counts = nullptr; cur.acc = nullptr; cur.acc_other = nullptr;
@@ -643,6 +689,7 @@
         case L_RES: {
             if (cur.ups != 0) { set_error("network: residual block directly after an upsampling is unsupported"); return FAV_EUNSUPPORTED; }
             Act skip = cur;
+            skip.pre = plain_stages(cur.pre);
             Act br = cur;
             br.partials = nullptr;
             int rc;
@@ -660,7 +707,7 @@
             size_t nx = li + 1;
             if (nx < ls.size() && ls[nx].type == L_UP && ls[nx].scale == 2) ++nx;
             const bool join_stats = nx < ls.size() && ls[nx].type == L_IN;
-            branch_tail_acc_ok = !lazy_out && !join_stats;
+            branch_tail_acc_ok = !lazy_out;
             rc = run(L.block, br, false, nullptr, nullptr);
             lazy.active = false; branch_tail_acc_ok = false;
             if (rc) return rc;
@@ -677,13 +724,15 @@
             }
             Act z; z.Hp = br.Hp; z.Wp = br.Wp; z.C = br.C;
             rc = alloc((size_t)z.Hp * z.Wp * z.C * sizeof(float), &z.data); if (rc) return rc;
-            if (join_stats) {
+            const bool z_acc = join_stats && z.C <= 256 && acc_consumer_ok(ls, nx + 1, 1, nx > li + 1 ? 1 : 0, top, z.Hp, z.Wp);
+            if (z_acc) take_acc(ins[in_cursor], z.C, z);
+            else if (join_stats) {
                 z.mblocks = res_add_stat_blocks(z.Hp, z.Wp); z.ppitch = z.C;
                 rc = alloc((size_t)z.mblocks * z.C * 2 * sizeof(float), &z.partials); if (rc) return rc;
                 float* cp = nullptr; rc = alloc((size_t)z.mblocks * sizeof(int), &cp); if (rc) return rc; z.counts = reinterpret_cast<int*>(cp);
             }
             rc = launch_res_add(br.data, br.pre.scale1, br.pre.shift1, skip.data, skip.Hp, skip.Wp, L.shave, skip.pre, z.C,
-                                z.data, z.partials, z.counts, st, skip.P(), &br.pre);
+                                z.data, z.partials, z.counts, st, skip.P(), &br.pre, z.acc);
             if (rc) return rc;
             cur = z;
             break;
@@ -771,7 +820,6 @@
         for (DevIN& i : ins) if (i.acc) FAV_HIP(hipMemsetAsync(i.acc, 0, i.acc_bytes, stream));
         acc_dirty = false;
     }
-    if (precision == 0 && !tuning().no_acc_stats && !tuning().no_wino) acc_parity ^= 1;
     Act cur;
     cur.data = const_cast<float*>(in8); cur.Hp = H + 2 * pad; cur.Wp = W + 2 * pad; cur.C = 8;
     const int rc = run(exec, cur, true, out_planar, out_raw);
diff --git a/fast-artistic-videos_amd/csrc/stat_acc.h b/fast-artistic-videos_amd/csrc/stat_acc.h
--- /dev/null
+++ b/fast-artistic-videos_amd/csrc/stat_acc.h
@@ -0,0 +1,71 @@
+#pragma once
+#include "fav_internal.h"
+
+namespace fav {
+
+__device__ __forceinline__ long long stat_acc_word(int which, int n, float mean, float m2, bool* fin)
+{
+    const double nd = (double)n, mud = (double)mean;
+    const double v = (which & 2) ? (double)m2 + nd * mud * mud : nd * mud;
+    const double tt = v * 1099511627776.0;
+    const double hi = floor(tt * (1.0 / 4294967296.0));
+    *fin = fabs(tt) < STAT_TILE_LIMIT;
+    return !*fin ? 0ll : (which & 1) ? (long long)hi : (long long)(tt - hi * 4294967296.0);
+}
+__device__ __forceinline__ void stat_acc_commit(long long* acc, int C, int c, int which, long long word, bool fin)
+{
+    long long* const dst = acc + ((size_t)(blockIdx.x & (STAT_COPIES - 1)) * C + c) * 4 + which;
+    if (fin) __hip_atomic_fetch_add(dst, word, __ATOMIC_RELAXED, __HIP_MEMORY_SCOPE_AGENT);
+    else if (which & 1) __hip_atomic_exchange(dst, STAT_NONFINITE, __ATOMIC_RELAXED, __HIP_MEMORY_SCOPE_AGENT);
+}
+
+struct StatAccRun {
+    long long w[4] = {0, 0, 0, 0};
+    bool fin = true;
+    __device__ __forceinline__ void add(int n, float mean, float m2)
+    {
+#pragma unroll
+        for (int k = 0; k < 4; ++k) { bool f; w[k] += stat_acc_word(k, n, mean, m2, &f); fin = fin && f; }
+    }
+    __device__ __forceinline__ void flush(long long* acc, int C, int c) const
+    {
+        const bool ok = fin && w[1] < STAT_RUN_LIMIT && w[1] > -STAT_RUN_LIMIT && w[3] < STAT_RUN_LIMIT;
+#pragma unroll
+        for (int k = 0; k < 4; ++k) stat_acc_commit(acc, C, c, k, w[k], ok);
+    }
+};
+
+__device__ __forceinline__ void stat_acc_affine(const StatAcc& a, int C, int c, bool zero, float* scale, float* shift)
+{
+    long long w0 = 0, w1 = 0, w2 = 0, w3 = 0;
+    bool bad = false;
+#pragma unroll
+    for (int cp = 0; cp < STAT_COPIES; ++cp) {
+        const longlong2* q = reinterpret_cast<const longlong2*>(a.acc + ((size_t)cp * C + c) * 4);
+        const longlong2 lo = q[0], hi = q[1];
+        bad = bad || stat_acc_poisoned(lo.y, hi.y);
+        w0 += lo.x; w1 += lo.y; w2 += hi.x; w3 += hi.y;
+    }
+    const double s1 = ((double)w1 * 4294967296.0 + (double)w0) * (1.0 / 1099511627776.0);
+    const double s2 = ((double)w3 * 4294967296.0 + (double)w2) * (1.0 / 1099511627776.0);
+    const double mean = s1 / (double)a.count;
+    double var = s2 / (double)a.count - mean * mean;
+    var = var > 0.0 ? var : 0.0;
+    const double sc = (bad || stat_acc_poisoned(w1, w3)) ? (double)NAN : (double)a.gamma[c] / sqrt(var + (double)a.eps);
+    *scale = (float)sc; *shift = (float)((double)a.beta[c] - mean * sc);
+    if (zero) {
+#pragma unroll
+        for (int cp = 0; cp < STAT_COPIES; ++cp) {
+            longlong2* z = reinterpret_cast<longlong2*>(a.zero + ((size_t)cp * C + c) * 4);
+            z[0] = longlong2{0, 0}; z[1] = longlong2{0, 0};
+        }
+        if (a.scale_out != nullptr) { a.scale_out[c] = *scale; a.shift_out[c] = *shift; }
+    }
+}
+template <int NT>
+__device__ __forceinline__ void stat_acc_table(const StatAcc& a, int C, float* sc, float* sh)
+{
+    for (int i = threadIdx.x; i < C; i += NT) stat_acc_affine(a, C, i, blockIdx.x == 0, sc + i, sh + i);
+}
+
+}
```
